# apple/ml-4m

Hardware: AMD Instinct MI355X
Metric: multimodal tokens/sec (4M-B train step, whole job) (higher is better)
Workload: dtype bf16; 1 GPU; 4M-B mod7 (fm_base_12e_12d_swiglu_nobias, 360.8M params, 8 input / 7 target modalities) masked-modeling train step, 224^2 token grids, 128 input + 128 target tokens/sample, AdamW; model=fm_base_12e_12d_swiglu_nobias, per_gpu_batch=256, global_batch=256, seq_len=256, parallelism=dp1

## Files before the change

include/fourm_hip.h:

```cpp
#ifndef FOURM_HIP_H
#define FOURM_HIP_H
#include <stdint.h>

#ifdef __cplusplus
extern "C" {
#endif

#define FM_ABI_VERSION 11
int fm_abi_version(void);
const char* fm_last_error(void);

enum fm_epilogue {
    FM_EPI_BF16 = 0,
    FM_EPI_GELU = 1,
    FM_EPI_RESIDUAL = 2,
    FM_EPI_SWIGLU = 3,
    FM_EPI_F32 = 4,
    FM_EPI_TANH = 5,
    FM_EPI_SWIGLU_BWD = 6,
    FM_EPI_GELU_BWD = 7,
    FM_EPI_QUICK_GELU = 8,
    FM_EPI_RELU = 9,
    FM_EPI_RELU_BWD = 10
};

typedef struct fm_gemm_group {
    const void* W;
    void* out;
    int32_t N, K, ldw, pad_;
} fm_gemm_group;

typedef struct fm_gemm_nt_args {
    const void* W; const void* W2; const void* X;
    void* out; void* out2; const void* res; const void* bias; const void* bias2;
    int32_t M, N, K, ldw, ldx, ldo, ldo2, ldr, Hp, epilogue;
    const fm_gemm_group* groups; const int32_t* tile_group; int32_t max_N;
    int32_t fixed_tiling;
    const int32_t* m_dev; const int32_t* row0_dev;
    void* splitk_ws; int64_t splitk_ws_bytes;
    int32_t conv_C, conv_H, conv_W, conv_Ho, conv_Wo, conv_stride, conv_up, conv_pad_;
} fm_gemm_nt_args;
int fm_gemm_nt(const fm_gemm_nt_args* args, void* stream);
void fm_set_gemm_nt_config(int cfg);
int fm_get_gemm_nt_config(void);
void fm_set_reserved_cus(int n);
int fm_get_reserved_cus(void);

typedef struct fm_gemm_tn_args {
    const void* A; const void* B; void* out;
    int32_t R, N, K, lda, ldb, ldo, a_cols, b_cols, splits, force_tr;
    const fm_gemm_group* groups; const int32_t* seg_start; const int32_t* seg_count;
    int32_t n_groups, max_N, max_R, pad_;
} fm_gemm_tn_args;
int fm_gemm_tn(const fm_gemm_tn_args* args, void* stream);
#define FM_TN_MAX_JOBS 16
typedef struct fm_gemm_tn_job {
    const void* A; const void* B; void* out;
    int32_t R, N, K, lda, ldb, ldo, a_cols, b_cols;
} fm_gemm_tn_job;
int fm_gemm_tn_multi(const fm_gemm_tn_job* jobs, int n_jobs, void* stream);
void fm_set_gemm_tn_config(int cfg);
int fm_get_gemm_tn_config(void);
void fm_set_tn_transpose_read(int on);
int fm_get_tn_transpose_read(void);

int fm_layernorm_fwd(const void* x, int ldx, const void* w, const void* b, void* y, int ldy, int y_is_f32,
                     void* mean, void* rstd, const int32_t* row_map, int R, int D, float eps, void* stream);
int fm_layernorm_fwd_res(const void* x, int ldx, const void* delta, int ldd, void* x_out, int ldxo, const void* w, const void* b,
                         void* y, int ldy, int y_is_f32, void* mean, void* rstd, const int32_t* row_map, int R, int D, float eps,
                         void* stream);
int fm_layernorm_bwd(const void* dy, int lddy, const int32_t* dy_row_map, const void* x, int ldx, const void* w,
                     const void* mean, const void* rstd, const void* dres, void* dx, int lddx, void* dx_bf16,
                     int lddxbf, void* dw, void* db, int R, int D, void* stream);
int fm_layernorm_bwd_h(const void* dy, int lddy, const void* h, int ldh, const void* x, int ldx, const void* w,
                       const void* mean, const void* rstd, const void* dres, void* dx, int lddx, void* dx_bf16,
                       int lddxbf, void* dw, int R, int D, void* stream);

int fm_headnorm_fwd(const void* x, int ldx, const void* w, const void* b, void* y, int ldy, void* stats, int R, int H, float eps,
                    void* stream);
int fm_headnorm_bwd(const void* dy, int lddy, const void* x, int ldx, const void* w, const void* stats, void* dx, int lddx, void* dw,
                    void* db, int R, int H, void* stream);

enum fm_mask_kind {
    FM_MASK_NONE = 0,
    FM_MASK_KEYPAD = 1,
    FM_MASK_DECODER = 2,
    FM_MASK_DENSE = 3
};
typedef struct fm_attn_args {
    const void* Q; const void* K; const void* V; void* O;
    void* stat_m; void* stat_l;
    int32_t ldq, ldk, ldv, ldo;
    int32_t B, H, Nq, Nk, head_dim, mask_kind;
    float scale; int32_t causal;
    const void* kpad; const int32_t* cs; const int16_t* modq; const int16_t* modk; const void* dense;
    const void* dO; void* dQ; void* dK; void* dV;
    int32_t lddo, lddq, lddk, lddv;
    int32_t force_tr;
    int32_t kv_batch_rows;
    int32_t zero_attn;
} fm_attn_args;
int fm_attn_fwd(const fm_attn_args* args, void* stream);
int fm_attn_bwd(const fm_attn_args* args, void* stream);
void fm_set_attn_transpose_read(int on);
int fm_get_attn_transpose_read(void);

#define FM_ATTN_DECODE_MAX_NK 8192
typedef struct fm_attn_decode_args {
    const void* q; void* k; const void* v; void* o;
    const void* q_w; const void* q_b; const void* k_w; const void* k_b;
    const void* kpad;
    int32_t ldq, ldk, ldv, ldo;
    int32_t B, H, Nk, kv_batch_rows, k_new_row, is_f32, zero_attn, pad_;
    float scale, eps;
} fm_attn_decode_args;
int fm_attn_decode(const fm_attn_decode_args* args, void* stream);

#define FM_MAX_MODS 24
enum fm_mod_kind {
    FM_KIND_TOK = 0,
    FM_KIND_PATCH = 1,
    FM_KIND_SEQ = 2,
    FM_KIND_SEQ_EMB = 3
};
typedef struct fm_mod_desc {
    const void* ids;
    const void* mask;
    const void* dam;
    const void* table;
    const void* pos;
    const void* mod_emb;
    const void* proj_bias;
    int32_t L;
    int32_t kind, ids_are_i64, mod_id;
    int32_t max_len;
    int32_t shifted;
    int32_t mask_stride, id_stride;
    int32_t patch, channels, grid_w, orig_dim;
    int32_t head_index;
    int32_t pad_;
} fm_mod_desc;
// ... 267 lines not shown
```

ml-4m_amd/csrc/gemm.hip:

```cpp
#include <type_traits>
#include <cstdlib>
#include <algorithm>
#include "common.h"
#include "fourm_hip.h"
#include "gemm_args.h"

namespace {
using namespace fmk;

constexpr int BK = 64;

__device__ __attribute__((aligned(16))) const uint32_t g_zero16[4] = {0u, 0u, 0u, 0u};

template <int TW, int TX, int WW, int WX, int KB, int STAGES, int EPI, bool GROUPED, bool PP = false, bool PERSIST = false, bool CONV = false>
__global__ __launch_bounds__(WW * WX * 64) void gemm_nt_kernel(NTArgs a) {
    constexpr int NWAVES = WW * WX;
    constexpr int RB = KB * 2;
    constexpr int CPR = RB / 16;
    constexpr int RPP = 1024 / RB;
    constexpr int SWSH = (RB == 128) ? 1 : 2;
    constexpr int LOADS = (TW + TX) / (RPP * NWAVES);
    constexpr int FW = TW / WW / 32, FX = TX / WX / 32;
    constexpr int STAGE = (TW + TX) * RB;
    static_assert(TW % (RPP * NWAVES) == 0 && TX % (RPP * NWAVES) == 0, "tile rows must split evenly over the DMA pieces");
// ... 633 lines not shown
#pragma unroll
                for (int i = 0; i < 2; ++i)
#pragma unroll
                    for (int j = 0; j < 2; ++j)
                        acc[i][j] = __builtin_amdgcn_mfma_f32_32x32x16_bf16(af[kk][i].v, bfr[kk][j].v, acc[i][j], 0, 0, 0);
                if (lead && more) stage_part(t_begin + it + 2, nbuf, kk, KS);
            }
            __builtin_amdgcn_s_setprio(0);
            if (lead) { if (more) wait_vmcnt<LOADS>(); else wait_vmcnt<0>(); }
            __builtin_amdgcn_sched_barrier(0);
            if (lead || it + 1 < NT_) block_barrier();
            buf = buf + 1 == STAGES ? 0 : buf + 1;
        }
    } else {
    int buf = 0;
    for (int it = 0; it < NT_; ++it) {
        const int younger = NT_ - 1 - it;
        if (STAGES >= 4 && younger >= 2) wait_vmcnt<2 * LOADS>();
        else if (STAGES >= 3 && younger >= 1) wait_vmcnt<LOADS>();
        else wait_vmcnt<0>();
        block_barrier();
        if (it + STAGES - 1 < NT_) stage(t_begin + it + STAGES - 1, (buf + STAGES - 1) % STAGES);
        const char* at = smem + buf * STAGE;
        const char* bt = at + KB * RBA;
        if constexpr (TR) {
            bf16x8_t af[2][2], bfr[2][2];
            auto load = [&](int kk, int par) {
                const int rA = kk * 16 + fhi * 8, rB = rA + 4;
#pragma unroll
                for (int i = 0; i < 2; ++i)
                    af[par][i] = lds_col_frag_tr_async([&](int r, int c) { return tn_addr<RBA>(at, r, c); }, rA, rB, wa * 64 + i * 32);
#pragma unroll
                for (int j = 0; j < 2; ++j)
                    bfr[par][j] = lds_col_frag_tr_async([&](int r, int c) { return tn_addr<RBB>(bt, r, c); }, rA, rB, wb * 64 + j * 32);
            };
            load(0, 0);
#pragma unroll
            for (int kk = 0; kk < KB / 16; ++kk) {
                if (kk + 1 < KB / 16) { load(kk + 1, (kk + 1) & 1); wait_lgkmcnt<8>(); }
                else wait_lgkmcnt<0>();
                __builtin_amdgcn_sched_barrier(0);
#pragma unroll
                for (int i = 0; i < 2; ++i)
#pragma unroll
                    for (int j = 0; j < 2; ++j)
                        acc[i][j] = __builtin_amdgcn_mfma_f32_32x32x16_bf16(af[kk & 1][i], bfr[kk & 1][j], acc[i][j], 0, 0, 0);
            }
        } else {
#pragma unroll
            for (int kk = 0; kk < KB / 16; ++kk) {
                const int rA = kk * 16 + fhi * 8, rB = rA + 4;
                bf16x8_t af[2], bfr[2];
#pragma unroll
                for (int i = 0; i < 2; ++i)
                    af[i] = lds_col_frag<false>([&](int r, int c) { return tn_addr<RBA>(at, r, c); }, rA, rB, wa * 64 + i * 32);
#pragma unroll
                for (int j = 0; j < 2; ++j)
                    bfr[j] = lds_col_frag<false>([&](int r, int c) { return tn_addr<RBB>(bt, r, c); }, rA, rB, wb * 64 + j * 32);
#pragma unroll
                for (int i = 0; i < 2; ++i)
#pragma unroll
                    for (int j = 0; j < 2; ++j)
                        acc[i][j] = __builtin_amdgcn_mfma_f32_32x32x16_bf16(af[i], bfr[j], acc[i][j], 0, 0, 0);
            }
        }
        buf = buf + 1 == STAGES ? 0 : buf + 1;
    }
    }
#pragma unroll
    for (int j = 0; j < 2; ++j) {
        const int k = k0 + wb * 64 + j * 32 + (lane & 31);
        if (k >= a.K) continue;
#pragma unroll
        for (int i = 0; i < 2; ++i)
#pragma unroll
            for (int r = 0; r < 16; ++r) {
                const int n = n0 + wa * 64 + i * 32 + (r & 3) + 8 * (r >> 2) + 4 * fhi;
                if (n < N) unsafeAtomicAdd(out + (size_t)n * a.ldo + k, acc[i][j][r]);
            }
    }
}


template <bool MASKED, int TA = 128, int KB = 64, bool LS = false>
__global__ __launch_bounds__(512) void gemm_tn_multi_kernel(TNMultiArgs a) {
    constexpr int TB = 256, WB = 4, STAGES = LS ? 2 : 3, NWAVES = 8;
    constexpr int FWA = TA / 2 / 32;
    constexpr int RBA = TA * 2, RBB = TB * 2;
    constexpr int PA = KB * RBA / 1024, PB = KB * RBB / 1024;
    constexpr int LOADS = (PA + PB) / NWAVES;
    constexpr int STAGE = KB * (RBA + RBB);
    constexpr int KS = KB / 16;
    extern __shared__ __attribute__((aligned(16))) char smem[];
    const int lane = threadIdx.x & 63;
    const int wave = __builtin_amdgcn_readfirstlane(threadIdx.x >> 6);
    const int wa = wave / WB, wb = wave % WB;
    const bool lead = wa == 0;
    const int fhi = lane >> 5;
    const bf16_t* zsrc = (const bf16_t*)g_zero16;
    const int G = gridDim.x;
    const int w = (blockIdx.x % 8) * (G / 8) + blockIdx.x / 8;

    const int li = lane & 15;
    const int frow0 = fhi * 8 + (li >> 2), fcol = ((lane >> 4) & 1) * 16 + (li & 3) * 4;
    const uint32_t smem_lds = (uint32_t)(uintptr_t)(__attribute__((address_space(3))) const char*)smem;
    uint32_t baseA[FWA], baseB[2];
#pragma unroll
    for (int i = 0; i < FWA; ++i) baseA[i] = (uint32_t)tn_off<RBA>(frow0, wa * (TA / 2) + i * 32 + fcol);
#pragma unroll
    for (int i = 0; i < 2; ++i) baseB[i] = (uint32_t)tn_off<RBB>(frow0, wb * 64 + i * 32 + fcol) + KB * RBA;

    auto run = [&](int tile, int t_begin, int t_end) {
        if (t_begin >= t_end) return;
        int j = 0;
        while (j + 1 < a.n_jobs && tile >= a.job[j + 1].tile_start) ++j;
        const TNJob& jb = a.job[j];
        const int local = tile - jb.tile_start;
        const int n0 = (local / jb.n_tiles_b) * TA, k0 = (local % jb.n_tiles_b) * TB;
        const bf16_t* A = jb.A; const bf16_t* B = jb.B;
        const int lda = jb.lda, ldb = jb.ldb, a_cols = jb.a_cols, b_cols = jb.b_cols, r_lim = jb.R;

#if defined(__HIP_DEVICE_COMPILE__)
        if constexpr (LS) {
            static_assert(!LS || (TA == 256 && KB == 64), "lock-step form: 256 x 256 tiles, K-step 64");
            constexpr int NPA = PA / NWAVES, NPB = PB / NWAVES, NP = NPA + NPB;
            const __amdgpu_buffer_rsrc_t rs_a = __builtin_amdgcn_make_buffer_rsrc(const_cast<bf16_t*>(A), 0, (int)min((size_t)r_lim * lda * 2, (size_t)0x7fffffff), 0x00020000);
            const __amdgpu_buffer_rsrc_t rs_b = __builtin_amdgcn_make_buffer_rsrc(const_cast<bf16_t*>(B), 0, (int)min((size_t)r_lim * ldb * 2, (size_t)0x7fffffff), 0x00020000);
            uint32_t offp[NP];
#pragma unroll
            for (int q = 0; q < NP; ++q) {
                const bool isa = q < NPA;
                const int piece = (isa ? q : q - NPA) * NWAVES + wave;
                const int row = piece * 2 + lane / 32;
                const int lc = (lane % 32) ^ ((row & 3) << 2);
                int c = (isa ? n0 : k0) + lc * 8;
                const int cols = isa ? a_cols : b_cols;
                c = c <= cols - 8 ? c : cols - 8;
                offp[q] = (uint32_t)row * (uint32_t)(isa ? lda : ldb) * 2u + (uint32_t)c * 2u;
            }
            auto dma = [&](int t, int buf, int q) __attribute__((always_inline)) {
                char* base = smem + buf * STAGE;
                if (q < NPA) __builtin_amdgcn_raw_ptr_buffer_load_lds(rs_a, LDS_PTR(base + (q * NWAVES + wave) * 1024), 16, offp[q], t * (KB * lda * 2), 0, 0);
                else __builtin_amdgcn_raw_ptr_buffer_load_lds(rs_b, LDS_PTR(base + KB * RBA + ((q - NPA) * NWAVES + wave) * 1024), 16, offp[q], t * (KB * ldb * 2), 0, 0);
            };
            f32x16_t acc[FWA][2];
#pragma unroll
            for (int i = 0; i < FWA; ++i)
#pragma unroll
                for (int jj = 0; jj < 2; ++jj)
#pragma unroll
                    for (int r = 0; r < 16; ++r) acc[i][jj][r] = 0.f;
            const int NT_ = t_end - t_begin;
#pragma unroll
            for (int q = 0; q < NP; ++q) dma(t_begin, 0, q);
            if (NT_ > 1) {
#pragma unroll
                for (int q = 0; q < NP; ++q) dma(t_begin + 1, 1, q);
                wait_vmcnt<NP>();
            } else wait_vmcnt<0>();
            block_barrier();
            union Frag { bf16x8_t v; s16x4_t h[2]; };
            Frag af[2][FWA], bfr[2][2];
            auto rd = [&](uint32_t st, auto kk_c, auto f_c, auto h_c, auto par_c) __attribute__((always_inline)) {
                constexpr int kk = decltype(kk_c)::value, f = decltype(f_c)::value, h = decltype(h_c)::value, PAR = decltype(par_c)::value;
                if constexpr (f < FWA) af[PAR][f].h[h] = tr_read<kk * 16 * RBA + h * 4 * RBA>(st + baseA[f]);
                else bfr[PAR][f - FWA].h[h] = tr_read<kk * 16 * RBB + h * 4 * RBB>(st + baseB[f - FWA]);
            };
            constexpr int NF = FWA + 2, NMF = FWA * 2;
            static_assert(!LS || NMF == 8, "k-step of the lock-step form: 8 MFMAs");
            using I0 = std::integral_constant<int, 0>; using I1 = std::integral_constant<int, 1>; using I2 = std::integral_constant<int, 2>;
            using I3 = std::integral_constant<int, 3>; using I4 = std::integral_constant<int, 4>; using I5 = std::integral_constant<int, 5>;
            auto k_step = [&](uint32_t st_next, auto kn_c, auto par_c, int t_dma, int buf_dma, auto d0_c, auto dn_c) __attribute__((always_inline)) {
                constexpr int PAR = decltype(par_c)::value, d0 = decltype(d0_c)::value, dn = decltype(dn_c)::value;
                wait_lgkmcnt<0>();
                __builtin_amdgcn_sched_barrier(0);
                auto one = [&](auto m_c) __attribute__((always_inline)) {
                    constexpr int m = decltype(m_c)::value;
                    constexpr int i = m / 2, jj = m % 2;
                    acc[i][jj] = __builtin_amdgcn_mfma_f32_32x32x16_bf16(af[PAR][i].v, bfr[PAR][jj].v, acc[i][jj], 0, 0, 0);
                    __builtin_amdgcn_sched_barrier(0);
                    if constexpr (m < NF) {
                        rd(st_next, kn_c, std::integral_constant<int, (m < NF ? m : 0)>{}, I0{}, std::integral_constant<int, PAR ^ 1>{});
                        rd(st_next, kn_c, std::integral_constant<int, (m < NF ? m : 0)>{}, I1{}, std::integral_constant<int, PAR ^ 1>{});
                    }
                    if constexpr (m < dn) { if (t_dma >= 0) dma(t_dma, buf_dma, d0 + m); }
                    __builtin_amdgcn_sched_barrier(0);
                };
                one(I0{}); one(I1{}); one(I2{}); one(I3{}); one(I4{}); one(I5{}); one(std::integral_constant<int, 6>{}); one(std::integral_constant<int, 7>{});
            };
            {
                const uint32_t st0 = smem_lds;
                rd(st0, I0{}, I0{}, I0{}, I0{}); rd(st0, I0{}, I0{}, I1{}, I0{}); rd(st0, I0{}, I1{}, I0{}, I0{}); rd(st0, I0{}, I1{}, I1{}, I0{});
                rd(st0, I0{}, I2{}, I0{}, I0{}); rd(st0, I0{}, I2{}, I1{}, I0{}); rd(st0, I0{}, I3{}, I0{}, I0{}); rd(st0, I0{}, I3{}, I1{}, I0{});
                rd(st0, I0{}, I4{}, I0{}, I0{}); rd(st0, I0{}, I4{}, I1{}, I0{}); rd(st0, I0{}, I5{}, I0{}, I0{}); rd(st0, I0{}, I5{}, I1{}, I0{});
            }
            int buf = 0;
            using NA = std::integral_constant<int, NPA>; using NB = std::integral_constant<int, NPB>;
            for (int it = 0; it < NT_; ++it) {
                const uint32_t st = smem_lds + buf * STAGE, stn = smem_lds + (buf ^ 1) * STAGE;
                const bool next = it + 1 < NT_, more = it + 2 < NT_;
                k_step(st, I1{}, I0{}, (it > 0 && next) ? t_begin + it + 1 : -1, buf ^ 1, NA{}, NB{});
                k_step(st, I2{}, I1{}, 0, 0, I0{}, I0{});
                k_step(st, I3{}, I0{}, 0, 0, I0{}, I0{});
// ... 53 lines not shown
        auto stage_part = [&](int t, int buf, int part, int nparts) {
#pragma unroll
            for (int q = 0; q < NP; ++q)
                if (q >= part * NP / nparts && q < (part + 1) * NP / nparts) stage_piece(t, buf, q);
        };

        f32x16_t acc[FWA][2];
#pragma unroll
        for (int i = 0; i < FWA; ++i)
#pragma unroll
            for (int jj = 0; jj < 2; ++jj)
#pragma unroll
                for (int r = 0; r < 16; ++r) acc[i][jj][r] = 0.f;

        const int NT_ = t_end - t_begin;
#pragma unroll
        for (int p = 0; p < STAGES - 1; ++p)
            if (p < NT_) stage(t_begin + p, p);
        if (NT_ > 1) wait_vmcnt<LOADS>(); else wait_vmcnt<0>();
        block_barrier();
        if (!lead) block_barrier();
        int buf = 0;
        for (int it = 0; it < NT_; ++it) {
            const bool more = it + 2 < NT_;
            const int nbuf = buf >= 1 ? buf - 1 : 2;
            const uint32_t st = smem_lds + buf * STAGE;
            union Frag { bf16x8_t v; s16x4_t h[2]; };
            Frag af[KS][FWA], bfr[KS][2];
            auto read_k = [&](auto kk_c) {
                constexpr int kk = decltype(kk_c)::value;
#pragma unroll
                for (int i = 0; i < FWA; ++i) {
                    af[kk][i].h[0] = tr_read<kk * 16 * RBA>(st + baseA[i]);
                    af[kk][i].h[1] = tr_read<kk * 16 * RBA + 4 * RBA>(st + baseA[i]);
                }
#pragma unroll
                for (int jj = 0; jj < 2; ++jj) {
                    bfr[kk][jj].h[0] = tr_read<kk * 16 * RBB>(st + baseB[jj]);
                    bfr[kk][jj].h[1] = tr_read<kk * 16 * RBB + 4 * RBB>(st + baseB[jj]);
                }
            };
            read_k(std::integral_constant<int, 0>{});
            read_k(std::integral_constant<int, 1>{});
            if constexpr (KS > 2) read_k(std::integral_constant<int, 2>{});
            if constexpr (KS > 3) read_k(std::integral_constant<int, 3>{});
            if (!lead) {
                if (more) { stage(t_begin + it + 2, nbuf); wait_vmcnt<LOADS>(); } else wait_vmcnt<0>();
            }
            wait_lgkmcnt<0>();
            block_barrier();
            __builtin_amdgcn_sched_barrier(0);
            __builtin_amdgcn_s_setprio(1);
#pragma unroll
            for (int kk = 0; kk < KS; ++kk) {
#pragma unroll
                for (int i = 0; i < FWA; ++i)
#pragma unroll
                    for (int jj = 0; jj < 2; ++jj)
                        acc[i][jj] = __builtin_amdgcn_mfma_f32_32x32x16_bf16(af[kk][i].v, bfr[kk][jj].v, acc[i][jj], 0, 0, 0);
                if (lead && more) stage_part(t_begin + it + 2, nbuf, kk, KS);
            }
            __builtin_amdgcn_s_setprio(0);
            if (lead) { if (more) wait_vmcnt<LOADS>(); else wait_vmcnt<0>(); }
            __builtin_amdgcn_sched_barrier(0);
            if (lead || it + 1 < NT_) block_barrier();
            buf = buf + 1 == STAGES ? 0 : buf + 1;
        }
        float* out = jb.out;
        const int N = jb.N, K = jb.K, ldo = jb.ldo;
        if (a.lab & 1) return;
#pragma unroll
        for (int jj = 0; jj < 2; ++jj) {
            const int k = k0 + wb * 64 + jj * 32 + (lane & 31);
            if (k >= K) continue;
#pragma unroll
            for (int i = 0; i < FWA; ++i)
#pragma unroll
                for (int r = 0; r < 16; ++r) {
                    const int n = n0 + wa * (TA / 2) + i * 32 + (r & 3) + 8 * (r >> 2) + 4 * fhi;
                    if (n < N) unsafeAtomicAdd(out + (size_t)n * ldo + k, acc[i][jj][r]);
                }
        }
    };
    tn_multi_walk(a, w, G, run);
}

int g_nt_config = 9, g_nt_prio = 1;
int g_lab[16] = {0, 0, [] { const char* e = getenv("FOURM_NT3"); return e ? atoi(e) : 3; }(), [] { const char* e = getenv("FOURM_NT3_LAB"); return e ? atoi(e) : 0; }(),
                 [] { const char* e = getenv("FOURM_NT4"); return e ? atoi(e) : 1; }(),
                 [] { const char* e = getenv("FOURM_TN4"); return e ? atoi(e) : 0; }(), 0, 0, 0,
                 [] { const char* e = getenv("FOURM_NT_SMALL"); return e ? atoi(e) : 1; }(),
                 [] { const char* e = getenv("FOURM_CONV_K32"); return e ? atoi(e) : 1; }()};
int g_nt_swiglu = 12;
int g_nt_auto[2] = {11, 10};

int g_reserved_cus = [] { const char* e = getenv("FOURM_RESERVED_CUS"); return e ? atoi(e) : 0; }();
static int n_compute_units() {
    static int n = [] {
        int dev = 0, cus = 0;
        if (hipGetDevice(&dev) != hipSuccess || hipDeviceGetAttribute(&cus, hipDeviceAttributeMultiprocessorCount, dev) != hipSuccess || cus <= 0) cus = 256;
        return cus;
    }();
    const int avail = n - g_reserved_cus;
    return avail >= 64 ? avail / 8 * 8 : n;
}

}
int fm_grid_cus() { return n_compute_units(); }
namespace {

template <int TW, int TX, int WW, int WX, int KB, int STAGES, int EPI, bool GROUPED, bool PP = false, bool PERSIST = false, bool CONV = false>
int launch_nt_cfg(NTArgs a, int max_n, hipStream_t s) {
    constexpr int NPT = (EPI == EPI_SWIGLU) ? TW / 2 : TW;
    a.n_tiles_w = (max_n + NPT - 1) / NPT;
    a.n_tiles_x = (a.M + TX - 1) / TX;
    int grid = a.n_tiles_w * a.n_tiles_x;
    if (GROUPED) {
        const int gw_max = TW > 128 ? 8 : 16;
        a.group_w = a.n_tiles_w < gw_max ? a.n_tiles_w : gw_max;
        const int chunks = ((a.n_tiles_w + a.group_w - 1) / a.group_w) * ((a.n_tiles_x + 3) / 4);
        grid = (chunks + 7) / 8 * 8 * a.group_w * 4;
    }
    const size_t lds = (size_t)STAGES * (TW + TX) * KB * 2;
    if (PERSIST) {
        const int slots = n_compute_units() * (int)(160 * 1024 / lds) / 8 * 8;
        if (grid > slots) grid = slots;
    }
    auto k = gemm_nt_kernel<TW, TX, WW, WX, KB, STAGES, EPI, GROUPED, PP, PERSIST, CONV>;
    static bool once = (hipFuncSetAttribute((const void*)k, hipFuncAttributeMaxDynamicSharedMemorySize, (int)lds), true);
    (void)once;
    hipLaunchKernelGGL(k, dim3(grid, a.split_k > 1 ? a.split_k : 1), dim3(WW * WX * 64), lds, s, a);
    FM_CHECK_LAUNCH("fm_gemm_nt");
    return 0;
}

__global__ __launch_bounds__(256) void splitk_reduce_kernel(const float* __restrict__ ws, int S, long long stride, int M, int N4, int ldp, const float* __restrict__ bias,
                                                            bf16_t* __restrict__ out, int ldo) {
    const long long total = (long long)M * N4;
    for (long long e = (long long)blockIdx.x * 256 + threadIdx.x; e < total; e += (long long)gridDim.x * 256) {
        const int m = (int)(e / N4), n = (int)(e % N4) * 4;
        float4 acc = *(const float4*)(ws + (size_t)m * ldp + n);
        for (int z = 1; z < S; ++z) {
            const float4 t = *(const float4*)(ws + (size_t)z * stride + (size_t)m * ldp + n);
            acc.x += t.x; acc.y += t.y; acc.z += t.z; acc.w += t.w;
        }
        if (bias) { const float4 b = *(const float4*)(bias + n); acc.x += bfround(b.x); acc.y += bfround(b.y); acc.z += bfround(b.z); acc.w += bfround(b.w); }
        *(uint2*)(out + (size_t)m * ldo + n) = make_uint2(pack2bf(acc.x, acc.y), pack2bf(acc.z, acc.w));
    }
}

template <int EPI, bool GROUPED>
int launch_nt(const NTArgs& a, int max_n, hipStream_t s) {
    if constexpr (GROUPED) {
        static_assert(FM_SEG_ROWS == 256, "the grouped configurations use a 256-row X tile");
        if constexpr (EPI == EPI_BF16) {
            static const int heads_cfg_k = [] { const char* e = getenv("FOURM_HEADS_NT_CFG"); return e ? atoi(e) : 0; }();
            if (a.K >= 1536 && heads_cfg_k == 3) return launch_nt_cfg<256, 256, 2, 4, 32, 3, EPI, true, true>(a, max_n, s);
            if (a.K >= 1536 && heads_cfg_k == 4) return launch_nt_cfg<256, 256, 2, 4, 64, 2, EPI, true>(a, max_n, s);
        }
        if (a.K >= 1536) return launch_nt_cfg<128, 256, 2, 4, 64, 3, EPI, true, true>(a, max_n, s);
        if constexpr (EPI == EPI_BF16) {
            static const int heads_cfg = [] { const char* e = getenv("FOURM_HEADS_NT_CFG"); return e ? atoi(e) : 0; }();
            if (heads_cfg == 1) return launch_nt_cfg<256, 256, 2, 4, 32, 3, EPI, true, true>(a, max_n, s);
            if (heads_cfg == 2) return launch_nt_cfg<128, 256, 2, 4, 32, 3, EPI, true, true>(a, max_n, s);
        }
        return launch_nt_cfg<128, 256, 2, 4, 32, 3, EPI, true>(a, max_n, s);
    }
    if (a.M <= 128 || a.fixed_tiling) return launch_nt_cfg<128, 128, 2, 2, 32, 3, EPI, GROUPED>(a, max_n, s);
    if constexpr (!GROUPED) {
        int cfg = g_nt_config;
        if (cfg == 9) {
            cfg = EPI == EPI_SWIGLU ? g_nt_swiglu : g_nt_auto[(a.K >= 1536 || EPI == EPI_RES || EPI == EPI_SWIGLU_BWD || EPI == EPI_GELU_BWD) ? 1 : 0];
            const long t256 = (long)((max_n + 255) / 256) * ((a.M + 255) / 256);
            if (cfg == g_nt_auto[0] && g_nt_auto[0] == 11 && max_n % 256 == 0 && t256 % n_compute_units() == 0) cfg = 12;
        }
        switch (cfg) {
            case 0: return launch_nt_cfg<128, 128, 2, 2, 64, 3, EPI, false>(a, max_n, s);
            case 1: return launch_nt_cfg<128, 256, 2, 4, 64, 3, EPI, false>(a, max_n, s);
            case 3: return launch_nt_cfg<256, 256, 2, 4, 32, 3, EPI, false, true>(a, max_n, s);
            case 4: return launch_nt_cfg<256, 256, 2, 4, 32, 3, EPI, false>(a, max_n, s);
            case 5: return launch_nt_cfg<256, 256, 2, 4, 64, 2, EPI, false>(a, max_n, s);
            case 6: return launch_nt_cfg<128, 128, 2, 2, 32, 3, EPI, false>(a, max_n, s);
            case 7: return launch_nt_cfg<128, 256, 2, 4, 64, 3, EPI, false, true>(a, max_n, s);
            case 8: return launch_nt_cfg<128, 256, 2, 4, 32, 3, EPI, false, true>(a, max_n, s);
            case 10: return launch_nt_cfg<128, 256, 2, 4, 64, 3, EPI, false, true, true>(a, max_n, s);
            case 11: return launch_nt_cfg<128, 256, 2, 4, 32, 3, EPI, false, true, true>(a, max_n, s);
            case 12: return launch_nt_cfg<256, 256, 2, 4, 32, 3, EPI, false, true, true>(a, max_n, s);
            case 13: if constexpr (EPI == EPI_BF16) return launch_nt_cfg<256, 256, 2, 2, 64, 2, EPI, false>(a, max_n, s); else break;
            case 14: if constexpr (EPI == EPI_BF16) return launch_nt_cfg<256, 256, 2, 2, 32, 3, EPI, false>(a, max_n, s); else break;
            default: return launch_nt_cfg<128, 256, 2, 4, 32, 3, EPI, false>(a, max_n, s);
        }
    }
    return -1;
}

}

extern "C" int fm_gemm_nt(const fm_gemm_nt_args* p, void* stream) {
    FM_CHECK_ARG(p && p->X && p->out, "fm_gemm_nt: null pointer");
    const bool grouped = p->groups != nullptr;
    FM_CHECK_ARG(grouped || p->W, "fm_gemm_nt: W is null");
    FM_CHECK_ARG(p->M > 0 && (grouped || (p->N > 0 && p->K > 0)), "fm_gemm_nt: bad shape M=%d N=%d K=%d", p->M, p->N, p->K);
    FM_CHECK_ARG(grouped || p->K % BK == 0, "fm_gemm_nt: K=%d must be a multiple of %d (zero padded)", p->K, BK);
    FM_CHECK_ARG(p->ldx % 8 == 0 && (grouped || p->ldw % 8 == 0), "fm_gemm_nt: leading dims must be multiples of 8");
    FM_CHECK_ARG(grouped || p->epilogue == FM_EPI_SWIGLU || p->ldo >= (p->N + 3) / 4 * 4, "fm_gemm_nt: ldo=%d too small for N=%d", p->ldo, p->N);
    FM_CHECK_ARG(!p->bias || (((uintptr_t)p->bias) & 15) == 0, "fm_gemm_nt: bias must be 16-byte aligned");
    FM_CHECK_ARG(p->ldo % 4 == 0, "fm_gemm_nt: ldo must be a multiple of 4");
    NTArgs a{};
    a.W = (const bf16_t*)p->W; a.W2 = (const bf16_t*)p->W2; a.X = (const bf16_t*)p->X;
    a.out = p->out; a.out2 = p->out2; a.res = (const float*)p->res; a.bias = (const float*)p->bias; a.bias2 = (const float*)p->bias2;
    a.M = p->M; a.N = p->N; a.K = p->K; a.ldw = p->ldw; a.ldx = p->ldx; a.ldo = p->ldo; a.ldo2 = p->ldo2; a.ldr = p->ldr; a.Hp = p->Hp;
    a.groups = p->groups; a.tile_group = p->tile_group;
    a.prio = g_nt_prio;
    a.dephase_groups = g_lab[0]; a.dephase_step = g_lab[1]; a.lab = g_lab[3];
    hipStream_t s = (hipStream_t)stream;
    a.m_dev = p->m_dev; a.row0_dev = p->row0_dev;
    const bool fixed = p->fixed_tiling != 0;
    FM_CHECK_ARG(!fixed || (!grouped && !p->m_dev && !p->row0_dev && p->conv_C == 0), "fm_gemm_nt: fixed_tiling is for dense launches (no groups, device-side rows or conv_*)");
    a.fixed_tiling = fixed ? 1 : 0;
    FM_CHECK_ARG(!(p->epilogue == FM_EPI_RELU || p->epilogue == FM_EPI_RELU_BWD) || (p->conv_C > 0 && !grouped && !p->m_dev && !p->row0_dev),
                 "fm_gemm_nt: FM_EPI_RELU / FM_EPI_RELU_BWD belong to the implicit convolution (conv_*), not to dense launches");
    if (p->m_dev || p->row0_dev) {
        FM_CHECK_ARG(p->m_dev && p->row0_dev && !grouped, "fm_gemm_nt: m_dev and row0_dev go together (dense launches only)");
        const int r = fm_launch_nt3(a, p->epilogue, g_lab[2] ? g_lab[2] : 3, s);
        if (r < 0) { fm_set_error("fm_gemm_nt (nt3, device-side rows): launch failed"); return -2; }
        if (r > 0) return 0;
        fm_set_error("fm_gemm_nt: a device-side row range needs FM_EPI_BF16 without bias, N %% 8 == 0, K %% 64 == 0, ldo %% 64 == 0 and a 128-byte aligned out "
                     "(N=%d K=%d ldo=%d epilogue=%d)", p->N, p->K, p->ldo, p->epilogue);
        return -1;
    }
    const int max_n = grouped ? p->max_N : p->N;
    if (!grouped && p->M <= 32 && p->conv_C == 0 && !fixed) {
        const int r = fm_launch_nt_skinny(a, p->epilogue, s);
        if (r < 0) { fm_set_error("fm_gemm_nt (skinny): launch failed"); return -2; }
        if (r > 0) return 0;
    }
    a.conv_C = p->conv_C; a.conv_H = p->conv_H; a.conv_W = p->conv_W; a.conv_Ho = p->conv_Ho; a.conv_Wo = p->conv_Wo; a.conv_stride = p->conv_stride; a.conv_up = p->conv_up;
    if (p->conv_C > 0) {
        const bool relu_bwd = p->epilogue == FM_EPI_RELU_BWD;
        FM_CHECK_ARG(!grouped && !p->m_dev && !p->out2 && (relu_bwd || !p->res) &&
                     (p->epilogue == FM_EPI_BF16 || p->epilogue == FM_EPI_F32 || p->epilogue == FM_EPI_RELU || relu_bwd),
                     "fm_gemm_nt (conv): dense FM_EPI_BF16 / FM_EPI_F32 / FM_EPI_RELU / FM_EPI_RELU_BWD only, no second output, res with FM_EPI_RELU_BWD only");
        FM_CHECK_ARG(!relu_bwd || (p->res && !p->bias && p->ldr % 4 == 0 && p->ldr >= (p->N + 3) / 4 * 4 && (((uintptr_t)p->res | (uintptr_t)p->out) & 7) == 0),
                     "fm_gemm_nt (conv): FM_EPI_RELU_BWD needs res = the saved bf16 activation (ldr %% 4 == 0, ldr >= roundup4(N), 8-byte aligned res / out) and no bias");
        FM_CHECK_ARG(p->conv_C % 64 == 0 && p->K == 9 * p->conv_C && (p->conv_stride == 1 || p->conv_stride == 2) && (p->conv_up == 0 || p->conv_up == 1) &&
                     p->conv_H > 0 && p->conv_W > 0 && p->conv_Ho > 0 && p->conv_Wo > 0 && p->M % (p->conv_Ho * p->conv_Wo) == 0,
                     "fm_gemm_nt (conv): C=%d K=%d stride=%d up=%d grid %dx%d -> %dx%d M=%d", p->conv_C, p->K, p->conv_stride, p->conv_up, p->conv_H, p->conv_W, p->conv_Ho, p->conv_Wo, p->M);
        FM_CHECK_ARG(p->conv_Ho == (p->conv_H + 2 - 3) / p->conv_stride + 1 && p->conv_Wo == (p->conv_W + 2 - 3) / p->conv_stride + 1, "fm_gemm_nt (conv): output grid does not match the input grid");
        if (p->epilogue == FM_EPI_F32) return launch_nt_cfg<128, 128, 2, 2, 64, 3, EPI_F32, false, false, false, true>(a, max_n, s);
        if (p->epilogue == FM_EPI_RELU) {
            if (g_lab[10]) return launch_nt_cfg<128, 128, 2, 2, 32, 3, EPI_RELU, false, false, false, true>(a, max_n, s);
            return launch_nt_cfg<128, 128, 2, 2, 64, 3, EPI_RELU, false, false, false, true>(a, max_n, s);
        }
        if (relu_bwd) {
            if (g_lab[10]) return launch_nt_cfg<128, 128, 2, 2, 32, 3, EPI_RELU_BWD, false, false, false, true>(a, max_n, s);
            return launch_nt_cfg<128, 128, 2, 2, 64, 3, EPI_RELU_BWD, false, false, false, true>(a, max_n, s);
        }
        const int cus = n_compute_units();
        const long t128 = (long)((p->M + 127) / 128) * ((p->N + 127) / 128);
        const int kt = p->K / 64;
        const long ldp = (p->N + 3) / 4 * 4;
        int S = 1;
        if (g_lab[9] && p->splitk_ws && t128 * 2 <= cus && p->N % 4 == 0 && (((uintptr_t)p->splitk_ws) & 15) == 0 && (((uintptr_t)p->out) & 7) == 0)
            S = (int)std::min<long>({cus / t128, (long)kt / 4, 16L, (long)(p->splitk_ws_bytes / ((long long)p->M * ldp * 4))});
        if (S >= 2) {
            const int ks = (kt + S - 1) / S * 64;
            S = (p->K + ks - 1) / ks;
            NTArgs b = a;
            b.out = p->splitk_ws; b.ldo = (int)ldp; b.bias = nullptr;
            b.split_k = S; b.k_slice = ks; b.split_stride = (long long)p->M * ldp;
            const int r = launch_nt_cfg<128, 128, 2, 2, 64, 3, EPI_F32, false, false, false, true>(b, max_n, s);
            if (r != 0) return r;
            const long long quads = (long long)p->M * (ldp / 4);
            const int rgrid = (int)std::min<long long>((quads + 255) / 256, 2048);
            hipLaunchKernelGGL(splitk_reduce_kernel, dim3(rgrid), dim3(256), 0, s, (const float*)p->splitk_ws, S, b.split_stride, p->M, (int)(ldp / 4), (int)ldp,
                               (const float*)p->bias, (bf16_t*)p->out, p->ldo);
            FM_CHECK_LAUNCH("fm_gemm_nt (conv, split-K reduction)");
            return 0;
        }
// ... 72 lines not shown
    }
    fm_set_error("fm_gemm_nt: unknown epilogue %d", p->epilogue);
    return -1;
}

extern int g_nt_flat;
extern "C" void fm_set_gemm_nt_config(int cfg) {
    g_nt_config = cfg & 0xff; g_nt_prio = (cfg >> 8) & 1;
    g_nt_flat = (cfg >> 29) & 1;
    if ((cfg >> 16) & 0xff) { g_nt_auto[0] = (cfg >> 16) & 0xf; g_nt_auto[1] = (cfg >> 20) & 0xf; }
    if ((cfg >> 24) & 0xf) g_nt_swiglu = (cfg >> 24) & 0xf;
}
extern "C" int fm_get_gemm_nt_config(void) { return g_nt_config; }
extern "C" void fm_lab_set(int key, int value) { if (key >= 0 && key < 16) g_lab[key] = value; }
extern "C" void fm_set_reserved_cus(int n) { g_reserved_cus = n < 0 ? 0 : n; }
extern "C" int fm_get_reserved_cus(void) { return g_reserved_cus; }
static int g_tn_config = [] { const char* e = getenv("FOURM_TN_CONFIG"); return e ? atoi(e) : 1; }();
extern "C" void fm_set_gemm_tn_config(int cfg) { g_tn_config = cfg; }
extern "C" int fm_get_gemm_tn_config(void) { return g_tn_config; }
static int g_tn_use_tr = 1;
extern "C" void fm_set_tn_transpose_read(int on) { g_tn_use_tr = on; }
extern "C" int fm_get_tn_transpose_read(void) { return g_tn_use_tr; }

extern "C" int fm_gemm_tn(const fm_gemm_tn_args* p, void* stream) {
    FM_CHECK_ARG(p && p->A && p->B, "fm_gemm_tn: null pointer");
    const bool grouped = p->groups != nullptr;
    FM_CHECK_ARG(grouped || p->out, "fm_gemm_tn: out is null");
    FM_CHECK_ARG(p->K > 0 && (grouped || (p->N > 0 && p->R > 0)), "fm_gemm_tn: bad shape");
    FM_CHECK_ARG(p->lda % 8 == 0 && p->ldb % 8 == 0, "fm_gemm_tn: leading dims must be multiples of 8");
    TNArgs a{};
    a.A = (const bf16_t*)p->A; a.B = (const bf16_t*)p->B; a.out = (float*)p->out;
    a.R = p->R; a.N = p->N; a.K = p->K; a.lda = p->lda; a.ldb = p->ldb; a.ldo = p->ldo;
    a.a_cols = p->a_cols > 0 ? p->a_cols : p->lda; a.b_cols = p->b_cols > 0 ? p->b_cols : p->ldb;
    FM_CHECK_ARG(a.a_cols >= 8 && a.b_cols >= 8, "fm_gemm_tn: operands need at least 8 readable columns");
    a.groups = p->groups; a.seg_start = p->seg_start; a.seg_count = p->seg_count;
    const int max_n = grouped ? p->max_N : p->N;
    constexpr int TN_TA = 128, TN_TB = 256, TN_STAGES = 3;
    const bool pp = (g_tn_config == 1 || g_tn_config == 3 || g_tn_config == 4) && !grouped && p->force_tr != 0;
    const int kb = pp ? 64 : 32, slots = (pp ? 1 : 2) * n_compute_units();
    a.n_tiles_a = (max_n + TN_TA - 1) / TN_TA; a.n_tiles_b = (p->K + TN_TB - 1) / TN_TB;
    int splits = p->splits;
    if (splits <= 0) {
        const int tiles = a.n_tiles_a * a.n_tiles_b;
        const int nt = grouped ? (p->max_R + kb - 1) / kb : (p->R + kb - 1) / kb;
        splits = tiles >= slots ? 1 : slots / tiles;
        while (splits > 1 && nt / splits < 8) --splits;
        if (splits > 64) splits = 64;
        if (nt < 16) splits = 1;
    }
    a.splits = splits;
    const size_t lds = (size_t)TN_STAGES * kb * (TN_TA + TN_TB) * 2;
    const int total_items = a.n_tiles_a * a.n_tiles_b * splits;
    const int deal = grouped ? 8 * 4 * a.n_tiles_b : 8;
    dim3 grid((total_items + deal - 1) / deal * deal, 1, grouped ? p->n_groups : 1);
    hipStream_t s = (hipStream_t)stream;
    const bool masked = grouped || p->R % kb != 0;
#define LAUNCH_TN(TR, G, KBV, PPV)                                                                  \
    if (masked) LAUNCH_TN2(TR, G, KBV, PPV, true) else LAUNCH_TN2(TR, G, KBV, PPV, false)
#define LAUNCH_TN2(TR, G, KBV, PPV, MK)                                                             \
    {                                                                                               \
        auto k = gemm_tn_kernel<TR, G, TN_TA, TN_TB, 2, 4, KBV, TN_STAGES, PPV, MK>;                \
        static bool once = (hipFuncSetAttribute((const void*)k, hipFuncAttributeMaxDynamicSharedMemorySize, (int)lds), true); \
        (void)once;                                                                                 \
        hipLaunchKernelGGL(k, grid, dim3(512), lds, s, a);                                          \
    }
    const int tr = p->force_tr >= 0 ? p->force_tr : g_tn_use_tr;
    if (pp) { if (grouped) { LAUNCH_TN(true, true, 64, true); } else { LAUNCH_TN(true, false, 64, true); } }
    else if (tr) { if (grouped) { LAUNCH_TN(true, true, 32, false); } else { LAUNCH_TN(true, false, 32, false); } }
    else { if (grouped) { LAUNCH_TN(false, true, 32, false); } else { LAUNCH_TN(false, false, 32, false); } }
#undef LAUNCH_TN
#undef LAUNCH_TN2
    FM_CHECK_LAUNCH("fm_gemm_tn");
    return 0;
}

extern "C" int fm_gemm_tn_multi(const fm_gemm_tn_job* jobs, int n_jobs, void* stream) {
    FM_CHECK_ARG(jobs && n_jobs > 0 && n_jobs <= FM_TN_MAX_JOBS, "fm_gemm_tn_multi: 1..FM_TN_MAX_JOBS jobs");
    TNMultiArgs a{};
    bool masked = false;
    int tiles = 0;
    long long units = 0;
    static const bool small_env = [] { const char* e = getenv("FOURM_TN_MULTI_TILE"); return e && atoi(e) == 128; }();
    const bool big = !(small_env || g_tn_config == 3);
    bool t4 = big && g_lab[5] != 0 && (g_tn_config == 1 || g_tn_config == 4);
    if (t4) {
        double useful = 0, padded = 0;
        for (int i = 0; i < n_jobs && t4; ++i) {
            const fm_gemm_tn_job& p = jobs[i];
            const int ac = p.a_cols > 0 ? p.a_cols : p.lda, bc = p.b_cols > 0 ? p.b_cols : p.ldb;
            t4 = p.R % 64 == 0 && p.R >= 256 && p.N % 128 == 0 && p.K % 128 == 0 && ac >= 128 && bc >= 128 && ac % 8 == 0 && bc % 8 == 0 &&
                 (((uintptr_t)p.A | (uintptr_t)p.B) & 15) == 0 && ((size_t)p.R * p.lda + ac) * 2 < 0x7fffffffull && ((size_t)p.R * p.ldb + bc) * 2 < 0x7fffffffull;
            useful += (double)p.N * p.K * p.R;
            padded += (double)((p.N + 255) / 256 * 256) * ((p.K + 383) / 384 * 384) * p.R;
        }
        t4 = t4 && useful >= 0.92 * padded;
    }
    const bool ls = big && (g_tn_config == 4 || t4);
    const int ta = big ? 256 : 128, kb = (big && !ls) ? 32 : 64, tb = t4 ? 384 : 256;
    for (int i = 0; i < n_jobs; ++i) {
        const fm_gemm_tn_job& p = jobs[i];
        FM_CHECK_ARG(p.A && p.B && p.out, "fm_gemm_tn_multi: null pointer");
        FM_CHECK_ARG(p.K > 0 && p.N > 0 && p.R > 0, "fm_gemm_tn_multi: bad shape");
        FM_CHECK_ARG(p.lda % 8 == 0 && p.ldb % 8 == 0, "fm_gemm_tn_multi: leading dims must be multiples of 8");
        TNJob& j = a.job[i];
        j.A = (const bf16_t*)p.A; j.B = (const bf16_t*)p.B; j.out = (float*)p.out;
        j.R = p.R; j.N = p.N; j.K = p.K; j.lda = p.lda; j.ldb = p.ldb; j.ldo = p.ldo;
        j.a_cols = p.a_cols > 0 ? p.a_cols : p.lda; j.b_cols = p.b_cols > 0 ? p.b_cols : p.ldb;
        FM_CHECK_ARG(j.a_cols >= 8 && j.b_cols >= 8, "fm_gemm_tn_multi: operands need at least 8 readable columns");
        j.n_tiles_b = (p.K + tb - 1) / tb;
        j.tiles = ((p.N + ta - 1) / ta) * j.n_tiles_b;
        j.tile_start = tiles;
        j.kt = (p.R + kb - 1) / kb;
        tiles += j.tiles;
        units += (long long)j.tiles * j.kt;
        masked = masked || p.R % kb != 0;
    }
    a.n_jobs = n_jobs; a.tiles = tiles; a.lab = g_lab[6];
    int grid = n_compute_units();
    if (units / 8 < grid) grid = (int)((units / 8 + 7) / 8 * 8);
    if (grid < 8) grid = 8;
    {
        const int rem = tiles % grid, ntail = grid - rem;
        a.tail_rr = rem >= ntail;
        double c = ls ? (a.tail_rr ? 12.0 : 64.0) : big ? (a.tail_rr ? 24.0 : 128.0) : 8.0;
        if (t4 && g_lab[7] > 0) c = g_lab[7];
        double cb = ls ? 16.0 : 32.0;
        if (t4 && g_lab[8] > 0) cb = g_lab[8];
        static const bool band_off = [] { const char* e = getenv("FOURM_TN_BANDS"); return e && atoi(e) == 0; }();
        a.banded = !a.tail_rr && rem > 0 && ntail > rem && !band_off;
        static const bool hybrid_off = [] { const char* e = getenv("FOURM_TN_HYBRID"); return e && atoi(e) == 0; }();
        a.hybrid = a.tail_rr && rem > ntail && ntail > 0 && !hybrid_off;
        for (int i = 0; i < n_jobs; ++i) {
            TNJob& j = a.job[i];
            j.lb = 0;
            if (rem == 0) { j.q = j.kt; continue; }
            if (a.banded) {
                const double rw = (double)rem / (ntail - rem);
                double q = (rw * j.kt + rw * cb) / (1.0 + 2.0 * rw);
                if (q < 0) q = 0;
                if (2 * q > j.kt) q = j.kt / 2;
                j.q = j.lb = (int)q;
                continue;
            }
            if (a.hybrid) {
                const double r = (double)rem / ntail;
                j.q = (int)((j.kt * r + c) / (1.0 + r));
            } else if (a.tail_rr) {
                const int n = (rem + ntail - 1) / ntail;
                double left = (j.kt - (n - 1) * c) / (n + 1.0);
                j.q = j.kt - (left > 0 ? (int)left : 0);
            } else {
                const double r = (double)rem / ntail;
                j.q = (int)((j.kt * r + r * c) / (1.0 + r));
            }
            if (j.q > j.kt) j.q = j.kt;
            if (j.q < 0) j.q = 0;
        }
    }
    hipStream_t s = (hipStream_t)stream;
#define LAUNCH_TNM(MK, TAV, KBV, ...)                                                                                         \
    {                                                                                                                         \
        constexpr bool lsv = sizeof(#__VA_ARGS__) > 1;                                                                        \
        constexpr size_t lds = (size_t)(lsv ? 2 : 3) * KBV * (TAV + 256) * 2;                                                 \
        auto k = gemm_tn_multi_kernel<MK, TAV, KBV, lsv>;                                                                     \
        static bool once = (hipFuncSetAttribute((const void*)k, hipFuncAttributeMaxDynamicSharedMemorySize, (int)lds), true); \
        (void)once;                                                                                                           \
        hipLaunchKernelGGL(k, dim3(grid), dim3(512), lds, s, a);                                                              \
    }
    if (t4) fm_launch_tn4_multi(a, grid, s);
    else if (ls) LAUNCH_TNM(false, 256, 64, ls)
    else if (big) { if (masked) LAUNCH_TNM(true, 256, 32) else LAUNCH_TNM(false, 256, 32) }
    else { if (masked) LAUNCH_TNM(true, 128, 64) else LAUNCH_TNM(false, 128, 64) }
#undef LAUNCH_TNM
    FM_CHECK_LAUNCH("fm_gemm_tn_multi");
    return 0;
}
```

ml-4m_amd/csrc/gemm_args.h:

```cpp
#pragma once
#include "common.h"
#include "fourm_hip.h"

namespace fmk {

enum { EPI_BF16 = FM_EPI_BF16, EPI_GELU = FM_EPI_GELU, EPI_RES = FM_EPI_RESIDUAL, EPI_SWIGLU = FM_EPI_SWIGLU,
       EPI_F32 = FM_EPI_F32, EPI_TANH = FM_EPI_TANH, EPI_SWIGLU_BWD = FM_EPI_SWIGLU_BWD, EPI_GELU_BWD = FM_EPI_GELU_BWD, EPI_QGELU = FM_EPI_QUICK_GELU,
       EPI_RELU = FM_EPI_RELU, EPI_RELU_BWD = FM_EPI_RELU_BWD };

struct NTArgs {
    const bf16_t* W; const bf16_t* W2; const bf16_t* X;
    void* out; void* out2; const float* res; const float* bias; const float* bias2;
    int M, N, K, ldw, ldx, ldo, ldo2, ldr, Hp;
    const fm_gemm_group* groups; const int* tile_group;
    const int* m_dev; const int* row0_dev;
    int n_tiles_w, n_tiles_x;
    int group_w;
    int prio;
    int dephase_groups, dephase_step;
    int reverse;
    int conv_C, conv_H, conv_W, conv_Ho, conv_Wo, conv_stride, conv_up;
    int split_k, k_slice; long long split_stride;
    int fixed_tiling;
    int lab;
};

__device__ __forceinline__ float gelu_f(float x) { return 0.5f * x * (1.0f + erf_fast(x * 0.70710678118654752f)); }
__device__ __forceinline__ float quick_gelu_f(float x) { return x * __builtin_amdgcn_rcpf(1.0f + __expf(-1.702f * x)); }
template <int EPI> constexpr bool is_gelu_like = EPI == EPI_GELU || EPI == EPI_QGELU;
template <int EPI> __device__ __forceinline__ float gelu_like_f(float x) { if constexpr (EPI == EPI_QGELU) return quick_gelu_f(x); else return gelu_f(x); }
__device__ __forceinline__ float silu_f(float x) { return x * __builtin_amdgcn_rcpf(1.0f + __expf(-x)); }


struct TNJob {
    const bf16_t* A; const bf16_t* B; float* out;
    int R, N, K, lda, ldb, ldo, a_cols, b_cols;
    int n_tiles_b, tiles, tile_start, kt;
    int q;
    int lb;
};
struct TNMultiArgs {
    TNJob job[FM_TN_MAX_JOBS];
    int n_jobs, tiles, tail_rr, banded;
    int hybrid;
    int lab;
};


template <typename Run>
__device__ __forceinline__ void tn_multi_walk(const TNMultiArgs& a, int w, int G, Run&& run) {
    auto job_of = [&](int tile) {
        int j = 0;
        while (j + 1 < a.n_jobs && tile >= a.job[j + 1].tile_start) ++j;
        return j;
    };

    const int full = a.tiles / G, T0 = full * G, rem = a.tiles - T0, ntail = G - rem;
    auto q_of = [&](int j) { return a.job[j].q; };
    const int nband = a.hybrid ? 0 : (a.banded ? rem : 0), nwalk = ntail - nband;
    const int walk_T0 = a.hybrid ? T0 + ntail : T0;
    auto q2_of = [&](int j) { return a.job[j].q + ((a.banded && !a.hybrid) ? a.job[j].lb : 0); };
    long long u0 = 0, u1 = 0;
    if (rem > 0 && w >= rem + nband && (!a.tail_rr || a.hybrid)) {
        long long Lsum = 0;
        for (int j = 0; j < a.n_jobs; ++j) {
            const int lo = max(a.job[j].tile_start, walk_T0), hi = a.job[j].tile_start + a.job[j].tiles;
            if (hi > lo) Lsum += (long long)(hi - lo) * (a.job[j].kt - q2_of(j));
        }
        u0 = Lsum * (w - rem - nband) / nwalk; u1 = Lsum * (w - rem - nband + 1) / nwalk;
    }
    int phase = 0, f = 0, tj = 0, ci = -1;
    long long P = 0;
    for (;;) {
        int tile = 0, t0 = 0, t1 = 0;
        bool have = false;
        if (phase == 0) {
            if (f < full) { tile = f * G + w; t1 = a.job[job_of(tile)].kt; ++f; have = true; }
            else { phase = rem == 0 ? 3 : (w < rem ? 1 : ((!a.tail_rr && w < rem + nband) ? 4 : 2)); f = 0; }
        } else if (phase == 1) {
            tile = T0 + w; t1 = q_of(job_of(tile)); phase = 3; have = true;
        } else if (phase == 4) {
            tile = T0 + (w - rem); const int j = job_of(tile); t0 = q_of(j); t1 = t0 + a.job[j].lb; phase = 3; have = true;
        } else if (phase == 2 && a.tail_rr && !(a.hybrid && f > 0)) {
            const int sgm = (w - rem) + f * ntail;
            if (sgm >= rem) phase = 3;
            else { tile = T0 + sgm; const int j = job_of(tile); t0 = q_of(j); t1 = a.job[j].kt; ++f; have = true; }
        } else if (phase == 2) {
            if (tj >= a.n_jobs) phase = 3;
            else {
                const int lo = max(a.job[tj].tile_start, walk_T0), hi = a.job[tj].tile_start + a.job[tj].tiles;
                const int q = q2_of(tj), left = a.job[tj].kt - q;
                bool advance = true;
                if (hi > lo && left > 0) {
                    const long long Pn = P + (long long)(hi - lo) * left;
                    if (u1 > P && u0 < Pn) {
                        const long long s0 = max(u0, P) - P, s1 = min(u1, Pn) - P;
                        if (ci < 0) ci = (int)(s0 / left);
                        const long long base = (long long)ci * left;
                        if (base < s1) {
                            tile = lo + ci; t0 = q + (int)(max(s0, base) - base); t1 = q + (int)(min(s1, base + left) - base);
                            ++ci; have = true; advance = false;
                        }
                    }
                    if (advance) P = Pn;
                }
                if (advance) { ++tj; ci = -1; }
            }
        } else break;
        if (have) run(tile, t0, t1);
    }
}

}

int fm_launch_nt_flat(const fmk::NTArgs& a, int epilogue, hipStream_t s);
int fm_launch_nt3(const fmk::NTArgs& a, int epilogue, int mode, hipStream_t s);
int fm_launch_nt4(const fmk::NTArgs& a, int epilogue, int mode, hipStream_t s);
int fm_launch_nt_skinny(const fmk::NTArgs& a, int epilogue, hipStream_t s);
int fm_grid_cus();
int fm_launch_tn4_multi(const fmk::TNMultiArgs& a, int grid, hipStream_t s);
```

ml-4m_amd/csrc/gemm_nt3.hip:

```cpp
#include <type_traits>
#include "common.h"
#include "fourm_hip.h"
#include "gemm_args.h"

namespace {
using namespace fmk;

typedef __attribute__((ext_vector_type(4))) unsigned int u32x4_t;
typedef __attribute__((ext_vector_type(4))) float f32x4v_t;

__device__ __forceinline__ __amdgpu_buffer_rsrc_t rsrc_of(const void* base) {
    return __builtin_amdgcn_make_buffer_rsrc(const_cast<void*>(base), 0, 0x7fffffff, 0x00020000);
}
constexpr uint32_t OOB = 0x80000000u;

template <int TW, int EPI, bool SPLIT = false, bool STG = false, bool BIAS = false, bool DEVM = false>
__global__ __launch_bounds__(512) void gemm_nt3_kernel(NTArgs a) {
#if defined(__HIP_DEVICE_COMPILE__)
    if constexpr (DEVM) {
        static_assert(EPI == EPI_BF16, "device-side row ranges: bf16 outputs only");
        const int m = (a.m_dev[0] + 255) & ~255;
        const size_t r0 = (size_t)a.row0_dev[0];
        a.M = m; a.n_tiles_x = m >> 8;
        a.X += r0 * a.ldx;
        a.out = (char*)a.out + r0 * a.ldo * 2;
        if (a.n_tiles_w * a.n_tiles_x <= (int)blockIdx.x) return;
    }
    constexpr int TX = 256, KB = 64, WW = 2, WX = 4, NWAVES = 8, KS = 4;
    constexpr int RB = 128, CPR = 8, RPP = 8;
    constexpr int FW = TW / WW / 32, FX = TX / WX / 32;
    constexpr int PW = TW / (RPP * NWAVES), PX = TX / (RPP * NWAVES), LOADS = PW + PX;
    constexpr int STAGE = (TW + TX) * RB;
    constexpr int NPT = (EPI == EPI_SWIGLU) ? TW / 2 : TW;
    constexpr int NMF = FW * FX;
    constexpr int NST = (EPI == EPI_BF16 || is_gelu_like<EPI>) ? FW * FX * 2 : EPI == EPI_SWIGLU ? FX * (FW / 2) * 2 * 3 : EPI == EPI_SWIGLU_BWD ? 60 : FW * FX * 4;
    static_assert(TW % (RPP * NWAVES) == 0, "tile rows must split evenly over the DMA pieces");
    static_assert(EPI != EPI_SWIGLU || FW % 2 == 0, "SwiGLU needs (g,u) fragment pairs per wave");
    extern __shared__ __attribute__((aligned(16))) char smem[];

    const int lane = threadIdx.x & 63;
    const int wave = __builtin_amdgcn_readfirstlane(threadIdx.x >> 6);
    const int ww = wave / WX, wx = wave % WX;
    const int frow = lane & 31, fhi = lane >> 5;
    const int fswz = (frow >> 1) & (CPR - 1);

    const int total = a.n_tiles_w * a.n_tiles_x;
    if (a.dephase_groups > 1) {
        const int ph = ((int)blockIdx.x / 8) % a.dephase_groups;
        for (int i = 0; i < ph * a.dephase_step; ++i) __builtin_amdgcn_s_sleep(32);
    }
    const int n_my = (total - (int)blockIdx.x + (int)gridDim.x - 1) / (int)gridDim.x;
    const int KT = a.K / KB;
    const int G = n_my * KT;
    const int N = a.N;

    uint32_t woff[PW], xoff[PX];
    __amdgpu_buffer_rsrc_t rs_w = rsrc_of(a.W), rs_w2 = rsrc_of(a.W2 ? a.W2 : a.W), rs_x = rsrc_of(a.X);
    (void)rs_w2;
    const int gw = a.group_w;
    const bool grouped_order = gw > 0 && total % 8 == 0 && a.n_tiles_x % 8 == 0 && a.n_tiles_w % gw == 0;
    auto tile_origin = [&](int j, int& n0, int& m0) {
        int tile = xcd_remap((int)blockIdx.x + j * (int)gridDim.x, total);
        if (a.reverse) tile = total - 1 - tile;
        int tw = tile % a.n_tiles_w, tx = tile / a.n_tiles_w;
        if (grouped_order) {
            const int per_xcd = total / 8, xr = a.n_tiles_x / 8;
            const int xcd = tile / per_xcd, l = tile % per_xcd;
            const int grp = l / (xr * gw), rem = l % (xr * gw);
            tx = xcd * xr + rem / gw; tw = grp * gw + rem % gw;
        }
        n0 = tw * NPT; m0 = tx * TX;
    };
    auto set_sources = [&](int j) __attribute__((always_inline)) {
        int n0, m0;
        tile_origin(j, n0, m0);
        rs_w = rsrc_of(a.W + (size_t)n0 * a.ldw);
        if constexpr (EPI == EPI_SWIGLU) rs_w2 = rsrc_of(a.W2 + (size_t)n0 * a.ldw);
        rs_x = rsrc_of(a.X + (size_t)m0 * a.ldx);
#pragma unroll
        for (int p = 0; p < PW; ++p) {
            const int t = (p * NWAVES + wave) * RPP + lane / CPR;
            const int lc = (lane % CPR) ^ ((t >> 1) & (CPR - 1));
            int r;
            if constexpr (EPI == EPI_SWIGLU) r = (t >> 6) * 32 + (t & 31);
            else r = t;
            r = n0 + r < N ? r : N - 1 - n0;
            woff[p] = (uint32_t)r * (uint32_t)a.ldw * 2u + (uint32_t)lc * 16u;
        }
#pragma unroll
        for (int p = 0; p < PX; ++p) {
            const int t = (p * NWAVES + wave) * RPP + lane / CPR;
            const int lc = (lane % CPR) ^ ((t >> 1) & (CPR - 1));
            const int r = m0 + t < a.M ? t : a.M - 1 - m0;
            xoff[p] = (uint32_t)r * (uint32_t)a.ldx * 2u + (uint32_t)lc * 16u;
        }
    };
    int s_kt = 0, s_j = 0, s_buf = 0;
    auto stage_piece = [&](int q) __attribute__((always_inline)) {
        const int soff = s_kt * (KB * 2);
        if (q < PW) {
            const int pi = q < PW ? q : 0;
            const int t0 = (pi * NWAVES + wave) * RPP;
            if (EPI == EPI_SWIGLU && ((t0 >> 5) & 1))
                __builtin_amdgcn_raw_ptr_buffer_load_lds(rs_w2, LDS_PTR(smem + s_buf * STAGE + (pi * NWAVES + wave) * 1024), 16, woff[pi], soff, 0, 0);
            else
                __builtin_amdgcn_raw_ptr_buffer_load_lds(rs_w, LDS_PTR(smem + s_buf * STAGE + (pi * NWAVES + wave) * 1024), 16, woff[pi], soff, 0, 0);
        } else {
            const int pi = q >= PW ? q - PW : 0;
            __builtin_amdgcn_raw_ptr_buffer_load_lds(rs_x, LDS_PTR(smem + s_buf * STAGE + TW * RB + (pi * NWAVES + wave) * 1024), 16, xoff[pi], soff, 0, 0);
        }
    };
    auto stage_advance = [&]() __attribute__((always_inline)) {
        ++s_kt; s_buf ^= 1;
        if (s_kt == KT) { s_kt = 0; ++s_j; if (s_j < n_my) set_sources(s_j); }
    };

    f32x16_t acc[FW][FX];
#pragma unroll
    for (int i = 0; i < FW; ++i)
#pragma unroll
        for (int j = 0; j < FX; ++j)
#pragma unroll
            for (int r = 0; r < 16; ++r) acc[i][j][r] = 0.f;

    auto finish_tile = [&](int j_done) __attribute__((always_inline)) {
        int n0, m0;
        tile_origin(j_done, n0, m0);
        if constexpr ((EPI == EPI_BF16 || is_gelu_like<EPI>) && STG) {
            const __amdgpu_buffer_rsrc_t rs_out = rsrc_of((const char*)a.out + (size_t)m0 * a.ldo * 2);
            const __amdgpu_buffer_rsrc_t rs_pre = rsrc_of((const char*)(a.out2 ? a.out2 : a.out) + (size_t)m0 * (a.out2 ? a.ldo2 : a.ldo) * 2);
            (void)rs_pre;
            constexpr int CW = (TW / WW) / 8;
            constexpr int RCH = CW == 16 ? 8 : 12, ROWB = RCH * 16, NRND = CW / RCH, SPR = 32 * RCH / 64;
            char* sc = smem + 2 * STAGE + wave * (32 * ROWB);
            constexpr int NWHICH = is_gelu_like<EPI> ? 2 : 1;
#pragma unroll
            for (int j = 0; j < FX; ++j)
#pragma unroll
                for (int rnd = 0; rnd < NRND; ++rnd)
#pragma unroll
                for (int which = 0; which < NWHICH; ++which) {
                    if (is_gelu_like<EPI> && which == 0 && !a.out2) continue;
#pragma unroll
                    for (int ii = 0; ii < RCH / 4; ++ii)
#pragma unroll
                        for (int g = 0; g < 4; ++g) {
                            const int i = rnd * (RCH / 4) + ii, ch = ii * 4 + g;
                            float v[4] = {acc[i][j][4 * g], acc[i][j][4 * g + 1], acc[i][j][4 * g + 2], acc[i][j][4 * g + 3]};
                            if constexpr (BIAS) {
                                const int cb = n0 + ww * (TW / WW) + i * 32 + 8 * g + 4 * fhi;
                                if (cb < N) {
                                    const float4 t = *(const float4*)(a.bias + cb);
                                    v[0] += bfround(t.x); v[1] += bfround(t.y); v[2] += bfround(t.z); v[3] += bfround(t.w);
                                }
                            }
                            if (is_gelu_like<EPI> && which == 1) {
#pragma unroll
                                for (int e = 0; e < 4; ++e) v[e] = gelu_like_f<EPI>(bfround(v[e]));
                            }
                            const uint2 pv = make_uint2(pack2bf(v[0], v[1]), pack2bf(v[2], v[3]));
                            int pos;
                            if constexpr (RCH == 8) pos = ch ^ (frow & 7);
                            else { pos = ch + (frow & 7); pos = pos >= 12 ? pos - 12 : pos; }
                            *(uint2*)(sc + frow * ROWB + pos * 16 + fhi * 8) = pv;
                        }
                    wait_lgkmcnt<0>();
                    __builtin_amdgcn_sched_barrier(0);
                    u32x4_t rv[SPR];
                    int rr[SPR], cc[SPR];
#pragma unroll
                    for (int q = 0; q < SPR; ++q) {
                        const int t = q * 64 + lane;
                        rr[q] = t / RCH; cc[q] = t % RCH;
                        int pos;
                        if constexpr (RCH == 8) pos = cc[q] ^ (rr[q] & 7);
                        else { pos = cc[q] + (rr[q] & 7); pos = pos >= 12 ? pos - 12 : pos; }
                        rv[q] = *(const u32x4_t*)(sc + rr[q] * ROWB + pos * 16);
                    }
                    wait_lgkmcnt<0>();
                    __builtin_amdgcn_sched_barrier(0);
#pragma unroll
                    for (int q = 0; q < SPR; ++q) {
                        const int rl = wx * (TX / WX) + j * 32 + rr[q];
                        const int c = n0 + ww * (TW / WW) + rnd * (RCH * 8) + cc[q] * 8;
                        if (is_gelu_like<EPI> && which == 0) {
                            const uint32_t so = ((m0 + rl < a.M && c < N) ? 0u : OOB) | ((uint32_t)(rl * a.ldo2) * 2u + (uint32_t)c * 2u);
                            __builtin_amdgcn_raw_buffer_store_b128(rv[q], rs_pre, so, 0, 0);
                        } else {
                            const uint32_t so = ((m0 + rl < a.M && c < N) ? 0u : OOB) | ((uint32_t)(rl * a.ldo) * 2u + (uint32_t)c * 2u);
                            __builtin_amdgcn_raw_buffer_store_b128(rv[q], rs_out, so, 0, 0);
                        }
                    }
                }
        } else if constexpr (EPI == EPI_BF16) {
            const __amdgpu_buffer_rsrc_t rs_out = rsrc_of((const char*)a.out + (size_t)m0 * a.ldo * 2);
            const int c0 = n0 + ww * (TW / WW) + 8 * fhi;
#pragma unroll
            for (int j = 0; j < FX; ++j) {
                const int rl = wx * (TX / WX) + j * 32 + frow;
                const uint32_t rowoff = (m0 + rl < a.M ? 0u : OOB) | ((uint32_t)(rl * a.ldo) * 2u);
#pragma unroll
                for (int i = 0; i < FW; ++i)
#pragma unroll
                    for (int gp = 0; gp < 2; ++gp) {
                        const int g = 2 * gp;
                        const uint2 p0 = make_uint2(pack2bf(acc[i][j][4 * g], acc[i][j][4 * g + 1]), pack2bf(acc[i][j][4 * g + 2], acc[i][j][4 * g + 3]));
                        const uint2 p1 = make_uint2(pack2bf(acc[i][j][4 * g + 4], acc[i][j][4 * g + 5]), pack2bf(acc[i][j][4 * g + 6], acc[i][j][4 * g + 7]));
                        const auto x = __builtin_amdgcn_permlane32_swap(p0.x, p1.x, false, false);
                        const auto y = __builtin_amdgcn_permlane32_swap(p0.y, p1.y, false, false);
                        const u32x4_t v = {x[0], y[0], x[1], y[1]};
                        const int c = c0 + i * 32 + 16 * gp;
                        const uint32_t so = (c < N ? rowoff : OOB) + (uint32_t)c * 2u;
                        if (a.lab & 32) __builtin_amdgcn_raw_buffer_store_b128(v, rs_out, so, 0, 2);
                        else if (a.lab & 64) __builtin_amdgcn_raw_buffer_store_b128(v, rs_out, so, 0, 17);
                        else if (a.lab & 128) __builtin_amdgcn_raw_buffer_store_b128(v, rs_out, so, 0, 3);
                        else __builtin_amdgcn_raw_buffer_store_b128(v, rs_out, so, 0, 0);
                    }
            }
        } else if constexpr (EPI == EPI_RES) {
            const __amdgpu_buffer_rsrc_t rs_out = rsrc_of((const char*)a.out + (size_t)m0 * a.ldo * 4);
            const __amdgpu_buffer_rsrc_t rs_res = rsrc_of((const char*)a.res + (size_t)m0 * a.ldr * 4);
            const int c0 = n0 + ww * (TW / WW) + 4 * fhi;
            f32x4v_t rv[2][4];
            auto req = [&](int f, int par) __attribute__((always_inline)) {
                const int j = f / FW, i = f % FW;
                const int rl = wx * (TX / WX) + j * 32 + frow;
                const uint32_t rowoff = (m0 + rl < a.M ? 0u : OOB) | ((uint32_t)(rl * a.ldr) * 4u);
#pragma unroll
                for (int g = 0; g < 4; ++g) {
                    const int c = c0 + i * 32 + 8 * g;
                    rv[par][g] = __builtin_bit_cast(f32x4v_t, __builtin_amdgcn_raw_buffer_load_b128(rs_res, (c < N ? rowoff : OOB) + (uint32_t)c * 4u, 0, 0));
                }
            };
            req(0, 0);
#pragma unroll
            for (int f = 0; f < FW * FX; ++f) {
                if (f + 1 < FW * FX) req(f + 1, (f + 1) & 1);
                const int j = f / FW, i = f % FW;
                const int rl = wx * (TX / WX) + j * 32 + frow;
                const uint32_t rowoff = (m0 + rl < a.M ? 0u : OOB) | ((uint32_t)(rl * a.ldo) * 4u);
#pragma unroll
                for (int g = 0; g < 4; ++g) {
                    const int c = c0 + i * 32 + 8 * g;
                    f32x4v_t o = rv[f & 1][g];
#pragma unroll
                    for (int e = 0; e < 4; ++e) o[e] += bfround(acc[i][j][4 * g + e]);
                    __builtin_amdgcn_raw_buffer_store_b128(__builtin_bit_cast(u32x4_t, o), rs_out, (c < N ? rowoff : OOB) + (uint32_t)c * 4u, 0, 0);
                }
            }
        } else if constexpr (EPI == EPI_SWIGLU_BWD) {
            const __amdgpu_buffer_rsrc_t rs_out = rsrc_of((const char*)a.out + (size_t)m0 * a.ldo * 2);
            const __amdgpu_buffer_rsrc_t rs_gu = rsrc_of((const char*)a.res + (size_t)m0 * a.ldr * 2);
            const int c0 = n0 + ww * (TW / WW) + 8 * fhi;
            u32x4_t sv[2][2];
            constexpr int NU = FW * FX * 2;
            auto src_off = [&](int unit, int ld) __attribute__((always_inline)) {
                const int f = unit / 2, gp = unit % 2, j = f / FW, i = f % FW;
                const int rl = wx * (TX / WX) + j * 32 + frow;
                const int c = c0 + i * 32 + 16 * gp;
                return ((m0 + rl < a.M && c < N) ? 0u : OOB) | ((uint32_t)(rl * ld) * 2u + (uint32_t)c * 2u);
            };
            auto req = [&](int unit, int par) __attribute__((always_inline)) {
                const uint32_t off = src_off(unit, a.ldr);
                sv[par][0] = __builtin_amdgcn_raw_buffer_load_b128(rs_gu, off, 0, 0);
                sv[par][1] = __builtin_amdgcn_raw_buffer_load_b128(rs_gu, off + (uint32_t)a.Hp * 2u, 0, 0);
            };
            req(0, 0);
#pragma unroll
            for (int unit = 0; unit < NU; ++unit) {
                if (unit + 1 < NU) req(unit + 1, (unit + 1) & 1);
                const int f = unit / 2, gp = unit % 2, j = f / FW, i = f % FW;
                uint2 g2[2], u2[2], dg2[2], du2[2];
                {
                    const u32x4_t tg = sv[unit & 1][0], tu = sv[unit & 1][1];
                    const auto gx = __builtin_amdgcn_permlane32_swap(tg[0], tg[2], false, false);
                    const auto gy = __builtin_amdgcn_permlane32_swap(tg[1], tg[3], false, false);
                    const auto ux = __builtin_amdgcn_permlane32_swap(tu[0], tu[2], false, false);
                    const auto uy = __builtin_amdgcn_permlane32_swap(tu[1], tu[3], false, false);
                    g2[0] = make_uint2(gx[0], gy[0]); g2[1] = make_uint2(gx[1], gy[1]);
                    u2[0] = make_uint2(ux[0], uy[0]); u2[1] = make_uint2(ux[1], uy[1]);
                }
#pragma unroll
                for (int u = 0; u < 2; ++u) {
                    const int g = 2 * gp + u;
                    float xv[4], uv[4], r1[4], r2[4];
                    unpack_bf4(g2[u], xv); unpack_bf4(u2[u], uv);
#pragma unroll
                    for (int e = 0; e < 4; ++e) {
                        const float d = bfround(acc[i][j][4 * g + e]);
                        const float sg = 1.0f / (1.0f + __expf(-xv[e]));
                        const float sl = bfround(xv[e] * sg);
                        const float ds = bfround(d * uv[e]);
                        r2[e] = d * sl;
                        r1[e] = ds * (sg * (1.0f + xv[e] * (1.0f - sg)));
                    }
                    dg2[u] = make_uint2(pack2bf(r1[0], r1[1]), pack2bf(r1[2], r1[3]));
                    du2[u] = make_uint2(pack2bf(r2[0], r2[1]), pack2bf(r2[2], r2[3]));
                }
                const auto ax = __builtin_amdgcn_permlane32_swap(dg2[0].x, dg2[1].x, false, false);
                const auto ay = __builtin_amdgcn_permlane32_swap(dg2[0].y, dg2[1].y, false, false);
                const auto bx = __builtin_amdgcn_permlane32_swap(du2[0].x, du2[1].x, false, false);
                const auto by = __builtin_amdgcn_permlane32_swap(du2[0].y, du2[1].y, false, false);
                const u32x4_t vg = {ax[0], ay[0], ax[1], ay[1]}, vu = {bx[0], by[0], bx[1], by[1]};
                const uint32_t off = src_off(unit, a.ldo);
                __builtin_amdgcn_raw_buffer_store_b128(vg, rs_out, off, 0, 0);
                __builtin_amdgcn_raw_buffer_store_b128(vu, rs_out, off + (uint32_t)a.Hp * 2u, 0, 0);
            }
        } else if constexpr (EPI == EPI_SWIGLU && STG) {
            const __amdgpu_buffer_rsrc_t rs_out = rsrc_of((const char*)a.out + (size_t)m0 * a.ldo * 2);
            const __amdgpu_buffer_rsrc_t rs_out2 = rsrc_of((const char*)(a.out2 ? a.out2 : a.out) + (size_t)m0 * (a.out2 ? a.ldo2 : a.ldo) * 2);
            char* sc = smem + 2 * STAGE + wave * 4096;
            const int hw0 = n0 + (ww * (TW / WW) / 64) * 32;
#pragma unroll
            for (int j = 0; j < FX; ++j) {
                uint2 qg[FW / 2][4], qu[FW / 2][4];
#pragma unroll
                for (int ip = 0; ip < FW / 2; ++ip)
#pragma unroll
                    for (int g = 0; g < 4; ++g) {
                        qg[ip][g] = make_uint2(pack2bf(acc[2 * ip][j][4 * g], acc[2 * ip][j][4 * g + 1]), pack2bf(acc[2 * ip][j][4 * g + 2], acc[2 * ip][j][4 * g + 3]));
                        qu[ip][g] = make_uint2(pack2bf(acc[2 * ip + 1][j][4 * g], acc[2 * ip + 1][j][4 * g + 1]), pack2bf(acc[2 * ip + 1][j][4 * g + 2], acc[2 * ip + 1][j][4 * g + 3]));
                        asm volatile("" : "+v"(qg[ip][g].x), "+v"(qg[ip][g].y), "+v"(qu[ip][g].x), "+v"(qu[ip][g].y));
                    }
#pragma unroll
                for (int which = 0; which < 3; ++which) {
                    if (which < 2 && !a.out2) continue;
#pragma unroll
                    for (int ip = 0; ip < FW / 2; ++ip)
#pragma unroll
                        for (int g = 0; g < 4; ++g) {
                            uint2 pv = which == 0 ? qg[ip][g] : qu[ip][g];
                            if (which == 2) {
                                float gv[4], uv[4];
                                unpack_bf4(qg[ip][g], gv); unpack_bf4(qu[ip][g], uv);
                                pv = make_uint2(pack2bf(bfround(silu_f(gv[0])) * uv[0], bfround(silu_f(gv[1])) * uv[1]),
                                                pack2bf(bfround(silu_f(gv[2])) * uv[2], bfround(silu_f(gv[3])) * uv[3]));
                            }
                            const int ch = ip * 4 + g;
                            *(uint2*)(sc + frow * 128 + ((ch ^ (frow & 7)) * 16) + fhi * 8) = pv;
                        }
                    wait_lgkmcnt<0>();
                    __builtin_amdgcn_sched_barrier(0);
                    u32x4_t rv[4];
#pragma unroll
                    for (int q = 0; q < 4; ++q) {
                        const int r = q * 8 + (lane >> 3), c = lane & 7;
                        rv[q] = *(const u32x4_t*)(sc + r * 128 + ((c ^ (r & 7)) * 16));
                    }
                    wait_lgkmcnt<0>();
                    __builtin_amdgcn_sched_barrier(0);
#pragma unroll
                    for (int q = 0; q < 4; ++q) {
                        const int rl = wx * (TX / WX) + j * 32 + q * 8 + (lane >> 3);
                        const int h = hw0 + (lane & 7) * 8;
                        const uint32_t ok = (m0 + rl < a.M && h < N) ? 0u : OOB;
                        if (which == 2) __builtin_amdgcn_raw_buffer_store_b128(rv[q], rs_out, ok | ((uint32_t)(rl * a.ldo) * 2u + (uint32_t)h * 2u), 0, 0);
                        else if (a.lab & 32) __builtin_amdgcn_raw_buffer_store_b128(rv[q], rs_out2, ok | ((uint32_t)(rl * a.ldo2) * 2u + (uint32_t)(h + (which == 1 ? a.Hp : 0)) * 2u), 0, 0);
                        else if (a.lab & 64) __builtin_amdgcn_raw_buffer_store_b128(rv[q], rs_out2, ok | ((uint32_t)(rl * a.ldo2) * 2u + (uint32_t)(h + (which == 1 ? a.Hp : 0)) * 2u), 0, 17);
                        else if (a.lab & 128) __builtin_amdgcn_raw_buffer_store_b128(rv[q], rs_out2, ok | ((uint32_t)(rl * a.ldo2) * 2u + (uint32_t)(h + (which == 1 ? a.Hp : 0)) * 2u), 0, 3);
                        else __builtin_amdgcn_raw_buffer_store_b128(rv[q], rs_out2, ok | ((uint32_t)(rl * a.ldo2) * 2u + (uint32_t)(h + (which == 1 ? a.Hp : 0)) * 2u), 0, 2);
                    }
                }
            }
        } else if constexpr (EPI == EPI_SWIGLU) {
            const __amdgpu_buffer_rsrc_t rs_out = rsrc_of((const char*)a.out + (size_t)m0 * a.ldo * 2);
            const __amdgpu_buffer_rsrc_t rs_out2 = rsrc_of((const char*)(a.out2 ? a.out2 : a.out) + (size_t)m0 * (a.out2 ? a.ldo2 : a.ldo) * 2);
            const int h0 = n0 + (ww * (TW / WW) / 64) * 32 + 8 * fhi;
#pragma unroll
            for (int j = 0; j < FX; ++j) {
                const int rl = wx * (TX / WX) + j * 32 + frow;
                const uint32_t ok = m0 + rl < a.M ? 0u : OOB;
                const uint32_t ro = ok | ((uint32_t)(rl * a.ldo) * 2u), ro2 = ok | ((uint32_t)(rl * a.ldo2) * 2u);
                u32x4_t pg[FW / 2][2], pu[FW / 2][2], pa[FW / 2][2];
#pragma unroll
                for (int ip = 0; ip < FW / 2; ++ip)
#pragma unroll
                    for (int gp = 0; gp < 2; ++gp) {
                        uint2 qg[2], qu[2], qa[2];
#pragma unroll
                        for (int u = 0; u < 2; ++u) {
                            const int g = 2 * gp + u;
                            float gv[4], uv[4], av[4];
#pragma unroll
                            for (int e = 0; e < 4; ++e) {
                                gv[e] = bfround(acc[2 * ip][j][4 * g + e]);
                                uv[e] = bfround(acc[2 * ip + 1][j][4 * g + e]);
                                av[e] = bfround(silu_f(gv[e])) * uv[e];
                            }
                            qg[u] = make_uint2(pack2bf(gv[0], gv[1]), pack2bf(gv[2], gv[3]));
                            qu[u] = make_uint2(pack2bf(uv[0], uv[1]), pack2bf(uv[2], uv[3]));
                            qa[u] = make_uint2(pack2bf(av[0], av[1]), pack2bf(av[2], av[3]));
                        }
                        auto swz = [&](const uint2 (&p)[2]) {
                            const auto x = __builtin_amdgcn_permlane32_swap(p[0].x, p[1].x, false, false);
                            const auto y = __builtin_amdgcn_permlane32_swap(p[0].y, p[1].y, false, false);
                            const u32x4_t v = {x[0], y[0], x[1], y[1]};
                            return v;
                        };
                        pg[ip][gp] = swz(qg); pu[ip][gp] = swz(qu); pa[ip][gp] = swz(qa);
                    }
#pragma unroll
                for (int which = 0; which < 3; ++which)
#pragma unroll
                    for (int ip = 0; ip < FW / 2; ++ip)
#pragma unroll
                        for (int gp = 0; gp < 2; ++gp) {
                            const int h = h0 + ip * 32 + 16 * gp;
                            const uint32_t col = (uint32_t)h * 2u;
                            if (which == 2) __builtin_amdgcn_raw_buffer_store_b128(pa[ip][gp], rs_out, (h < N ? ro : OOB) + col, 0, 0);
                            else __builtin_amdgcn_raw_buffer_store_b128(which == 0 ? pg[ip][gp] : pu[ip][gp], rs_out2,
                                                                        ((h < N && a.out2) ? ro2 : OOB) + col + (which == 1 ? (uint32_t)a.Hp * 2u : 0u), 0, 0);
                        }
            }
        }
#pragma unroll
        for (int i = 0; i < FW; ++i)
#pragma unroll
            for (int j = 0; j < FX; ++j)
#pragma unroll
                for (int r = 0; r < 16; ++r) acc[i][j][r] = 0.f;
    };

    set_sources(0);
#pragma unroll
    for (int q = 0; q < LOADS; ++q) stage_piece(q);
    stage_advance();
    if (G > 1) {
#pragma unroll
        for (int q = 0; q < LOADS; ++q) stage_piece(q);
        stage_advance();
        wait_vmcnt<LOADS>();
    } else wait_vmcnt<0>();
    block_barrier();

    bf16x8_t wf[2][FW], xf[2][FX];
    auto read_frags = [&](int buf, int kk, int par) __attribute__((always_inline)) {
        const char* wt = smem + buf * STAGE + (ww * (TW / WW) + frow) * RB;
        const char* xt = smem + buf * STAGE + TW * RB + (wx * (TX / WX) + frow) * RB;
        const int off = ((kk * 2 + fhi) ^ fswz) * 16;
#pragma unroll
        for (int i = 0; i < FW; ++i) wf[par][i] = *(const bf16x8_t*)(wt + i * 32 * RB + off);
#pragma unroll
        for (int j = 0; j < FX; ++j) xf[par][j] = *(const bf16x8_t*)(xt + j * 32 * RB + off);
    };
    auto mfmas = [&](int par) __attribute__((always_inline)) {
#pragma unroll
        for (int i = 0; i < FW; ++i)
#pragma unroll
            for (int j = 0; j < FX; ++j)
                acc[i][j] = __builtin_amdgcn_mfma_f32_32x32x16_bf16(wf[par][i], xf[par][j], acc[i][j], 0, 0, 0);
    };
    read_frags(0, 0, 0);

    int buf = 0, c_kt = 0, c_j = 0;
// ... 8 lines not shown
#pragma unroll
                for (int q = 0; q < PW; ++q) stage_piece(q);
            }
            mfmas(kk & 1);
#pragma unroll
            for (int q = 0; q < FW + FX; ++q) {
                __builtin_amdgcn_sched_group_barrier(0x008, 1, 0);
                __builtin_amdgcn_sched_group_barrier(0x100, 1, 0);
                if (HALF && kk == 0 && q < PW) __builtin_amdgcn_sched_group_barrier(0x020, 1, 0);
            }
            __builtin_amdgcn_sched_barrier(0);
            if (HALF && kk == 0) stage_advance();
        }
        if constexpr (NEXT) {
            if (!(a.lab & 1)) { if (stores_behind && !SPLIT) wait_vmcnt<NST>(); else wait_vmcnt<0>(); }
        }
        wait_lgkmcnt<0>();
        block_barrier();
        __builtin_amdgcn_sched_barrier(0);
        if constexpr (NEXT) read_frags(buf ^ 1, 0, 0);
        constexpr int NOW = SPLIT ? PX : LOADS;
        if constexpr (MORE) {
            if (!(a.lab & 2)) {
#pragma unroll
                for (int q = SPLIT ? PW : 0; q < LOADS; ++q) stage_piece(q);
            }
        }
        mfmas(1);
        constexpr int RD = NEXT ? FW + FX : 0, RSTEPS = (RD + 1) / 2;
#pragma unroll
        for (int q = 0; q < RSTEPS; ++q) {
            __builtin_amdgcn_sched_group_barrier(0x008, 1, 0);
            __builtin_amdgcn_sched_group_barrier(0x100, 2, 0);
        }
        if constexpr (MORE) {
            constexpr int LEFT = NMF - RSTEPS - 1;
            constexpr int PER = (NOW + LEFT - 1) / LEFT;
#pragma unroll
            for (int q = 0; q < LEFT; ++q) {
                __builtin_amdgcn_sched_group_barrier(0x008, 1, 0);
                __builtin_amdgcn_sched_group_barrier(0x020, PER, 0);
            }
        }
        __builtin_amdgcn_sched_barrier(0);
        if constexpr (MORE && !SPLIT) stage_advance();
        buf ^= 1;
        stores_behind = false;
        if (++c_kt == KT) {
            if (!(a.lab & 4)) finish_tile(c_j);
            c_kt = 0; ++c_j; stores_behind = true;
        }
    };
    using T = std::true_type; using F = std::false_type;
    if (G > 2) k_tile(T{}, T{}, T{}); else k_tile(T{}, T{}, F{});
    for (int g = 1; g + 2 < G; ++g) k_tile(F{}, T{}, T{});
    if (G > 2) k_tile(F{}, T{}, F{});
    k_tile(F{}, F{}, F{});
#endif
}

template <int TW, int EPI, bool SPLIT = false, bool STG = false, bool BIAS = false, bool DEVM = false>
int launch_nt3(NTArgs a, hipStream_t s) {
    constexpr int NPT = (EPI == EPI_SWIGLU) ? TW / 2 : TW;
    a.n_tiles_w = (a.N + NPT - 1) / NPT;
    a.n_tiles_x = (a.M + 255) / 256;
    a.group_w = (a.lab >> 12) & 15;
    if (a.group_w == 0 && EPI == EPI_SWIGLU && STG) a.group_w = 4;
    if (a.group_w == 15) a.group_w = 0;
    int grid = a.n_tiles_w * a.n_tiles_x;
    const int cus = fm_grid_cus();
    if (grid > cus || DEVM) grid = cus;
    a.reverse = (a.lab & 2048) ? 0 : 1;
    const size_t lds = (size_t)2 * (TW + 256) * 128 + (STG ? (TW == 256 ? 32768 : 49152) : 0);
    auto k = gemm_nt3_kernel<TW, EPI, SPLIT, STG, BIAS, DEVM>;
    static bool once = (hipFuncSetAttribute((const void*)k, hipFuncAttributeMaxDynamicSharedMemorySize, (int)lds), true);
    (void)once;
    hipLaunchKernelGGL(k, dim3(grid), dim3(512), lds, s, a);
    if (hipGetLastError() != hipSuccess) return -2;
    return 1;
}

}

int fm_launch_nt3(const fmk::NTArgs& a, int epilogue, int mode, hipStream_t s) {
    using namespace fmk;
    if (!mode || a.groups || a.bias2) return 0;
    if (a.m_dev) {
        if (!a.row0_dev || epilogue != FM_EPI_BF16 || a.bias || a.K % 64 != 0 || a.K < 128 || a.N % 8 != 0 || a.ldo % 64 != 0 ||
            (((uintptr_t)a.out) & 127) != 0 || (a.lab & (16 | 1024)))
            return 0;
        if ((size_t)256 * (size_t)a.ldo * 4 >= 0x7fffffffull || (size_t)256 * (size_t)a.ldx * 2 >= 0x7fffffffull || (size_t)256 * (size_t)a.ldw * 2 >= 0x7fffffffull) return 0;
        return (a.N % 192 == 0 && a.N % 256 != 0) ? launch_nt3<192, EPI_BF16, true, true, false, true>(a, s) : launch_nt3<256, EPI_BF16, true, true, false, true>(a, s);
    }
    if (a.bias && !(epilogue == FM_EPI_BF16 || epilogue == FM_EPI_GELU || epilogue == FM_EPI_QUICK_GELU)) return 0;
    if (a.bias && ((((uintptr_t)a.bias) & 15) != 0 || (a.lab & (16 | 1024)))) return 0;
    if (a.M < 2048 || a.K % 64 != 0 || a.K < 128 || a.N % 8 != 0) return 0;
    if ((size_t)256 * (size_t)a.ldo * 4 >= 0x7fffffffull || (size_t)256 * (size_t)a.ldx * 2 >= 0x7fffffffull || (size_t)256 * (size_t)a.ldw * 2 >= 0x7fffffffull) return 0;
    const bool al16 = (((uintptr_t)a.out | (uintptr_t)a.out2 | (uintptr_t)a.res) & 15) == 0;
    if (!al16) return 0;
    const int cus = fm_grid_cus();
    const long xt = (a.M + 255) / 256;
    const long t256 = (long)((a.N + 255) / 256) * xt, t192 = (long)((a.N + 191) / 192) * xt;
    const bool fits192 = a.N % 192 == 0;
    const long c256 = (t256 + cus - 1) / cus * 256, c192 = (t192 + cus - 1) / cus * 192;
    const bool use192 = mode == 2 ? fits192 : mode == 3 ? (fits192 && c192 < c256) : false;
    if (epilogue == FM_EPI_GELU) {
        if (!(a.lab & 131072)) return 0;
        if (a.ldo % 64 != 0 || (((uintptr_t)a.out) & 127) != 0 || (a.out2 && (a.ldo2 % 64 != 0 || (((uintptr_t)a.out2) & 127) != 0)) || (a.lab & (16 | 1024))) return 0;
        if (a.bias) return use192 ? launch_nt3<192, EPI_GELU, true, true, true>(a, s) : launch_nt3<256, EPI_GELU, true, true, true>(a, s);
        return use192 ? launch_nt3<192, EPI_GELU, true, true, false>(a, s) : launch_nt3<256, EPI_GELU, true, true, false>(a, s);
    }
    if (epilogue == FM_EPI_QUICK_GELU) {
        if (!(a.lab & 131072)) return 0;
        if (a.ldo % 64 != 0 || (((uintptr_t)a.out) & 127) != 0 || (a.out2 && (a.ldo2 % 64 != 0 || (((uintptr_t)a.out2) & 127) != 0)) || (a.lab & (16 | 1024))) return 0;
        if (a.bias) return use192 ? launch_nt3<192, EPI_QGELU, true, true, true>(a, s) : launch_nt3<256, EPI_QGELU, true, true, true>(a, s);
        return use192 ? launch_nt3<192, EPI_QGELU, true, true, false>(a, s) : launch_nt3<256, EPI_QGELU, true, true, false>(a, s);
    }
    if (epilogue == FM_EPI_BF16) {
        if (a.ldo % 8 != 0) return 0;
        if (a.bias) {
            if (a.ldo % 64 != 0 || (((uintptr_t)a.out) & 127) != 0) return 0;
            return use192 ? launch_nt3<192, EPI_BF16, true, true, true>(a, s) : launch_nt3<256, EPI_BF16, true, true, true>(a, s);
        }
        if (!(a.lab & 1024) && !(a.lab & 16) && a.ldo % 64 == 0 && (((uintptr_t)a.out) & 127) == 0)
            return use192 ? launch_nt3<192, EPI_BF16, true, true>(a, s) : launch_nt3<256, EPI_BF16, true, true>(a, s);
        if (!(a.lab & 16)) return use192 ? launch_nt3<192, EPI_BF16, true>(a, s) : launch_nt3<256, EPI_BF16, true>(a, s);
        return use192 ? launch_nt3<192, EPI_BF16>(a, s) : launch_nt3<256, EPI_BF16>(a, s);
    }
    if (epilogue == FM_EPI_RESIDUAL) {
        if (!(a.lab & 256)) return 0;
        if (a.ldo % 4 != 0 || a.ldr % 4 != 0 || !a.res) return 0;
        if (!(a.lab & 16)) return use192 ? launch_nt3<192, EPI_RES, true>(a, s) : launch_nt3<256, EPI_RES, true>(a, s);
        return use192 ? launch_nt3<192, EPI_RES>(a, s) : launch_nt3<256, EPI_RES>(a, s);
    }
    if (epilogue == FM_EPI_SWIGLU_BWD) {
        if (a.N % 16 != 0 || a.Hp % 8 != 0 || a.ldo % 8 != 0 || a.ldr % 8 != 0 || !a.res || a.Hp < a.N) return 0;
        if ((size_t)256 * (size_t)a.ldr * 2 >= 0x7fffffffull) return 0;
        return launch_nt3<256, EPI_SWIGLU_BWD, true>(a, s);
    }
    if (epilogue == FM_EPI_SWIGLU) {
        if (a.N % 64 != 0 || a.Hp % 8 != 0 || a.ldo % 8 != 0 || (a.out2 && a.ldo2 % 8 != 0) || !a.W2) return 0;
        if (!(a.lab & 1024) && !(a.lab & 16) && a.ldo % 64 == 0 && (!a.out2 || a.ldo2 % 64 == 0) && a.Hp % 64 == 0 && a.N % 64 == 0)
            return launch_nt3<256, EPI_SWIGLU, true, true>(a, s);
        if (!(a.lab & 16)) return launch_nt3<256, EPI_SWIGLU, true>(a, s);
        return launch_nt3<256, EPI_SWIGLU>(a, s);
    }
    return 0;
}
```

ml-4m_amd/fourm/hip/_lib.py:

```python
import ctypes as C
import os

FM_MAX_MODS = 24
_LIB_PATH = os.environ.get("FOURM_HIP_LIB") or os.path.join(os.path.dirname(os.path.dirname(os.path.abspath(__file__))), "_lib", "libfourm_hip.so")


class FourmHipUnavailable(ImportError):
    pass


def _load():
    if not os.path.exists(_LIB_PATH):
        raise FourmHipUnavailable(
            f"{_LIB_PATH} is missing - build the gfx950 kernels first: python ml-4m_amd/build_ext.py "
            "(the 4M hot path has no fallback implementation)")
    return C.CDLL(_LIB_PATH)


lib = _load()
lib.fm_last_error.restype = C.c_char_p
lib.fm_abi_version.restype = C.c_int
ABI_VERSION = 11
if lib.fm_abi_version() != ABI_VERSION:
    raise FourmHipUnavailable(f"libfourm_hip.so ABI {lib.fm_abi_version()} != expected {ABI_VERSION}; rebuild")

vp, i32, i64, f32 = C.c_void_p, C.c_int32, C.c_int64, C.c_float

EPI_BF16, EPI_GELU, EPI_RESIDUAL, EPI_SWIGLU, EPI_F32, EPI_TANH, EPI_SWIGLU_BWD, EPI_GELU_BWD, EPI_QUICK_GELU = 0, 1, 2, 3, 4, 5, 6, 7, 8
EPI_RELU, EPI_RELU_BWD = 9, 10
MASK_NONE, MASK_KEYPAD, MASK_DECODER, MASK_DENSE = 0, 1, 2, 3
KIND_TOK, KIND_PATCH, KIND_SEQ, KIND_SEQ_EMB = 0, 1, 2, 3
LOSS_MOD, LOSS_TOKEN = 0, 1


class GemmGroup(C.Structure):
    _fields_ = [("W", vp), ("out", vp), ("N", i32), ("K", i32), ("ldw", i32), ("pad_", i32)]


class GemmNTArgs(C.Structure):
    _fields_ = [("W", vp), ("W2", vp), ("X", vp), ("out", vp), ("out2", vp), ("res", vp), ("bias", vp), ("bias2", vp),
                ("M", i32), ("N", i32), ("K", i32), ("ldw", i32), ("ldx", i32), ("ldo", i32), ("ldo2", i32), ("ldr", i32),
                ("Hp", i32), ("epilogue", i32), ("groups", vp), ("tile_group", vp), ("max_N", i32), ("fixed_tiling", i32),
                ("m_dev", vp), ("row0_dev", vp), ("splitk_ws", vp), ("splitk_ws_bytes", i64),
                ("conv_C", i32), ("conv_H", i32), ("conv_W", i32), ("conv_Ho", i32), ("conv_Wo", i32), ("conv_stride", i32), ("conv_up", i32), ("conv_pad_", i32)]


class GemmTNArgs(C.Structure):
    _fields_ = [("A", vp), ("B", vp), ("out", vp), ("R", i32), ("N", i32), ("K", i32), ("lda", i32), ("ldb", i32),
                ("ldo", i32), ("a_cols", i32), ("b_cols", i32), ("splits", i32), ("force_tr", i32), ("groups", vp),
                ("seg_start", vp), ("seg_count", vp), ("n_groups", i32), ("max_N", i32), ("max_R", i32), ("pad_", i32)]


class GemmTNJob(C.Structure):
    _fields_ = [("A", vp), ("B", vp), ("out", vp), ("R", i32), ("N", i32), ("K", i32), ("lda", i32), ("ldb", i32),
                ("ldo", i32), ("a_cols", i32), ("b_cols", i32)]


TN_MAX_JOBS = 16


class AttnArgs(C.Structure):
    _fields_ = [("Q", vp), ("K", vp), ("V", vp), ("O", vp), ("stat_m", vp), ("stat_l", vp),
                ("ldq", i32), ("ldk", i32), ("ldv", i32), ("ldo", i32),
                ("B", i32), ("H", i32), ("Nq", i32), ("Nk", i32), ("head_dim", i32), ("mask_kind", i32),
                ("scale", f32), ("causal", i32),
                ("kpad", vp), ("cs", vp), ("modq", vp), ("modk", vp), ("dense", vp),
                ("dO", vp), ("dQ", vp), ("dK", vp), ("dV", vp),
                ("lddo", i32), ("lddq", i32), ("lddk", i32), ("lddv", i32), ("force_tr", i32), ("kv_batch_rows", i32), ("zero_attn", i32)]


class AttnDecodeArgs(C.Structure):
    _fields_ = [("q", vp), ("k", vp), ("v", vp), ("o", vp), ("q_w", vp), ("q_b", vp), ("k_w", vp), ("k_b", vp), ("kpad", vp),
                ("ldq", i32), ("ldk", i32), ("ldv", i32), ("ldo", i32),
                ("B", i32), ("H", i32), ("Nk", i32), ("kv_batch_rows", i32), ("k_new_row", i32), ("is_f32", i32), ("zero_attn", i32), ("pad_", i32),
                ("scale", f32), ("eps", f32)]


class ModDesc(C.Structure):
    _fields_ = [("ids", vp), ("mask", vp), ("dam", vp), ("table", vp), ("pos", vp), ("mod_emb", vp), ("proj_bias", vp),
                ("L", i32), ("kind", i32), ("ids_are_i64", i32), ("mod_id", i32), ("max_len", i32), ("shifted", i32),
                ("mask_stride", i32), ("id_stride", i32), ("patch", i32), ("channels", i32), ("grid_w", i32),
                ("orig_dim", i32), ("head_index", i32), ("pad_", i32)]


class ShadowDesc(C.Structure):
    _fields_ = [("src", vp), ("dst", vp), ("ld_src", i32), ("ld_dst", i32), ("rows", i32), ("cols", i32),
                ("transpose", i32), ("tile_start", i32), ("col_scale", vp), ("dst_f32", i32), ("reserved", i32)]


FOLD_MAX_JOBS = 48


class FoldGradJob(C.Structure):
    _fields_ = [("dWp", vp), ("W", vp), ("gamma", vp), ("gW", vp), ("ggamma", vp), ("rows", i32), ("cols", i32), ("ld_dwp", i32), ("reserved", i32)]


class GemmF32Args(C.Structure):
    _fields_ = [("X", vp), ("W", vp), ("W2", vp), ("out", vp), ("out2", vp), ("res", vp), ("bias", vp), ("bias2", vp),
                ("sxm", i64), ("sxk", i64), ("swn", i64), ("swk", i64),
                ("M", i32), ("N", i32), ("K", i32), ("ldo", i32), ("ldo2", i32), ("ldr", i32), ("Hp", i32), ("epilogue", i32),
                ("accumulate", i32), ("max_N", i32), ("seg_rows", i32), ("n_groups", i32),
                ("groups", vp), ("tile_group", vp), ("seg_start", vp), ("seg_count", vp)]


class SpanMaskArgs(C.Structure):
    _fields_ = [("ids", vp), ("len", vp), ("unit", vp), ("noise", vp), ("keep_prob", vp), ("r_choice", vp), ("input_budget", vp), ("target_budget", vp),
                ("sentinel_ids", vp), ("emb", vp), ("emb_out", vp), ("src", vp), ("tensor", vp), ("input_mask", vp), ("target_mask", vp),
                ("decoder_attention_mask", vp), ("tries", vp),
                ("B", i32), ("ld_ids", i32), ("T", i32), ("ld_noise", i32), ("n_sentinels", i32), ("max_tokens", i32), ("vocab_offset", i32), ("pad_id", i32),
                ("emb_rows", i32), ("emb_dim", i32)]


class AdamWJob(C.Structure):
    _fields_ = [("p", vp), ("g", vp), ("m", vp), ("v", vp), ("dst_plain", vp), ("dst_t", vp),
                ("rows", i32), ("cols", i32), ("ld_plain", i32), ("ld_t", i32), ("tile_start", i32), ("pad_", i32)]


class SelectDesc(C.Structure):
    _fields_ = [("mods", ModDesc * FM_MAX_MODS),
                ("n_mods", i32), ("batch", i32), ("dim", i32), ("n_keep", i32), ("n_reg", i32), ("total_len", i32),
                ("is_decoder", i32), ("raw", i32),
                ("reg_tokens", vp), ("mask_token", vp),
                ("tokens", vp), ("emb", vp), ("x0", vp), ("out_mask", vp), ("out_mod", vp), ("slot_mod", vp),
                ("slot_src", vp), ("slot_pos", vp), ("target_ids", vp), ("out_cs", vp), ("out_mod_pre", vp),
                ("out_mod_index", vp), ("patch_rows", vp), ("seqemb_rows", vp), ("patch_ld", i32), ("seqemb_ld", i32),
                ("rows_f32", i32), ("pad2_", i32)]


class EmbedBwdMod(C.Structure):
    _fields_ = [("d_table", vp), ("d_pos", vp), ("d_mod_emb", vp), ("d_proj_bias", vp),
                ("kind", i32), ("has_padding_idx", i32), ("padding_idx", i32), ("pad_", i32)]


class EmbedBwdDesc(C.Structure):
    _fields_ = [("mods", EmbedBwdMod * FM_MAX_MODS), ("dx", vp), ("slot_mod", vp), ("slot_src", vp), ("slot_pos", vp),
                ("d_mask_token", vp), ("d_reg_tokens", vp),
                ("n_mods", i32), ("batch", i32), ("dim", i32), ("Nt", i32), ("lddx", i32), ("is_decoder", i32)]


class EmaJob(C.Structure):
    _fields_ = [("ema", vp), ("model", vp), ("n", i64), ("first_chunk", i64)]


def _sig(name, *argtypes):
    fn = getattr(lib, name)
    fn.argtypes = list(argtypes)
    fn.restype = C.c_int
    return fn


P = C.POINTER
gemm_nt = _sig("fm_gemm_nt", P(GemmNTArgs), vp)
gemm_tn = _sig("fm_gemm_tn", P(GemmTNArgs), vp)
gemm_tn_multi = _sig("fm_gemm_tn_multi", P(GemmTNJob), C.c_int, vp)
layernorm_fwd = _sig("fm_layernorm_fwd", vp, i32, vp, vp, vp, i32, i32, vp, vp, vp, i32, i32, f32, vp)
layernorm_fwd_res = _sig("fm_layernorm_fwd_res", vp, i32, vp, i32, vp, i32, vp, vp, vp, i32, i32, vp, vp, vp, i32, i32, f32, vp)
layernorm_bwd = _sig("fm_layernorm_bwd", vp, i32, vp, vp, i32, vp, vp, vp, vp, vp, i32, vp, i32, vp, vp, i32, i32, vp)
layernorm_bwd_h = _sig("fm_layernorm_bwd_h", vp, i32, vp, i32, vp, i32, vp, vp, vp, vp, vp, i32, vp, i32, vp, i32, i32, vp)
attn_fwd = _sig("fm_attn_fwd", P(AttnArgs), vp)
attn_bwd = _sig("fm_attn_bwd", P(AttnArgs), vp)
attn_decode = _sig("fm_attn_decode", P(AttnDecodeArgs), vp)
ATTN_DECODE_MAX_NK = 8192
select_embed = _sig("fm_select_embed", P(SelectDesc), vp)
embed_bwd = _sig("fm_embed_bwd", P(EmbedBwdDesc), vp)
dense_decoder_mask = _sig("fm_dense_decoder_mask", vp, vp, vp, i32, i32, i32, i32, i32, vp)
segment_rows = _sig("fm_segment_rows", vp, i32, i32, vp, vp, vp, vp, vp, i32, vp)
gather_rows = _sig("fm_gather_rows", vp, i32, vp, vp, i32, i32, i32, vp)
cross_entropy = _sig("fm_cross_entropy", vp, i32, vp, vp, vp, vp, vp, vp, vp, i32, i32, i32, i32, vp, vp, vp, vp, i32, vp)
swiglu_bwd = _sig("fm_swiglu_bwd", vp, i32, vp, i32, vp, i32, i32, i32, i32, vp)
gelu_bwd = _sig("fm_gelu_bwd", vp, i32, vp, i32, vp, i32, i32, i32, i32, vp)
cast_pad = _sig("fm_cast_pad", vp, i32, vp, i32, i32, i32, vp)
transpose_cast_pad = _sig("fm_transpose_cast_pad", vp, i32, vp, i32, i32, i32, i32, vp)
colsum = _sig("fm_colsum", vp, i32, vp, i32, i32, vp)
shadow_refresh = _sig("fm_shadow_refresh", vp, i32, i32, vp)
fold_colscale_grad = _sig("fm_fold_colscale_grad", vp, i32, vp)
headnorm_fwd = _sig("fm_headnorm_fwd", vp, i32, vp, vp, vp, i32, vp, i32, i32, C.c_float, vp)
headnorm_bwd = _sig("fm_headnorm_bwd", vp, i32, vp, i32, vp, vp, vp, i32, vp, vp, i32, i32, vp)
f32_to_bf16 = _sig("fm_f32_to_bf16", vp, vp, i64, vp)
bf16_to_f32_scaled = _sig("fm_bf16_to_f32_scaled", vp, vp, i64, f32, vp)
add_bf16_f32 = _sig("fm_add_bf16_f32", vp, vp, vp, i64, vp)
lib.fm_set_reserved_cus.argtypes = [C.c_int]
lib.fm_get_reserved_cus.restype = C.c_int
lib.fm_get_reserved_cus.argtypes = []
adamw = _sig("fm_adamw", vp, vp, vp, vp, i64, f32, f32, f32, f32, f32, i64, vp, vp, vp, vp)
adamw_shadow = _sig("fm_adamw_shadow", vp, i32, i32, f32, f32, f32, f32, f32, i64, vp, vp, vp, vp)
sumsq = _sig("fm_sumsq", vp, i64, vp, vp)
clip_coef = _sig("fm_clip_coef", vp, f32, vp, vp, vp)
sample_tokens = _sig("fm_sample_tokens", vp, i32, i32, i32, i32, f32, i32, f32, vp, vp, vp, vp)
maskgit_commit = _sig("fm_maskgit_commit", vp, vp, vp, i32, i32, i32, vp, i32, i32, vp, vp, vp, vp)
gemm_f32 = _sig("fm_gemm_f32", P(GemmF32Args), vp)
attn_f32_fwd = _sig("fm_attn_f32_fwd", P(AttnArgs), vp)
attn_f32_bwd = _sig("fm_attn_f32_bwd", P(AttnArgs), vp)
layernorm_bwd_f32 = _sig("fm_layernorm_bwd_f32", vp, i32, vp, vp, i32, vp, vp, vp, vp, vp, i32, vp, i32, vp, vp, i32, i32, vp)
headnorm_f32_fwd = _sig("fm_headnorm_f32_fwd", vp, i32, vp, vp, vp, i32, vp, i32, i32, C.c_float, vp)
headnorm_f32_bwd = _sig("fm_headnorm_f32_bwd", vp, i32, vp, i32, vp, vp, vp, i32, vp, vp, i32, i32, vp)
swiglu_bwd_f32 = _sig("fm_swiglu_bwd_f32", vp, i32, vp, i32, vp, i32, i32, i32, i32, vp)
gelu_bwd_f32 = _sig("fm_gelu_bwd_f32", vp, i32, vp, i32, vp, i32, i32, i32, vp)
colsum_f32 = _sig("fm_colsum_f32", vp, i32, vp, i32, i32, vp)
cross_entropy_f32 = _sig("fm_cross_entropy_f32", vp, i32, vp, vp, vp, vp, vp, vp, vp, i32, i32, i32, i32, vp, vp, vp, vp, i32, vp)
vq_patchify = _sig("fm_vq_patchify", vp, vp, i32, i32, i32, i32, i32, i32, vp)
l2norm_rows = _sig("fm_l2norm_rows", vp, i32, vp, i32, i32, i32, vp)
vq_assign = _sig("fm_vq_assign", vp, i32, vp, vp, i32, i32, i32, i32, i32, vp, vp, i32, vp, vp, vp)
lib.fm_set_tn_transpose_read.argtypes = [C.c_int]
lib.fm_set_gemm_tn_config.argtypes = [C.c_int]
lib.fm_set_attn_transpose_read.argtypes = [C.c_int]

lib.fm_set_gemm_nt_config.argtypes = [C.c_int]
lib.fm_lab_set.argtypes = [C.c_int, C.c_int]
lib.fm_lab_set.restype = None
vq_code_stats = _sig("fm_vq_code_stats", vp, i32, vp, i32, i32, i32, vp, vp, vp)
vq_ema_update = _sig("fm_vq_ema_update", vp, vp, vp, vp, i32, i32, f32, vp)
vq_code_bias = _sig("fm_vq_code_bias", vp, i32, i32, vp, vp)
vq_assign_bias = _sig("fm_vq_assign_bias", vp, i32, vp, vp, vp, i32, i32, i32, i32, i32, vp, vp, i32, vp, vp, vp)
vq_code_stats_raw = _sig("fm_vq_code_stats_raw", vp, i32, vp, i32, i32, i32, vp, vp, vp)
vq_ema_update_euclid = _sig("fm_vq_ema_update_euclid", vp, vp, vp, vp, vp, vp, i32, i32, f32, f32, vp)
vq_unpatchify = _sig("fm_vq_unpatchify", vp, i32, vp, i32, i32, i32, i32, i32, vp)
VQ_WIDE_TILE, CONVNEXT_MAX_C = 128, 4
vq_assign_wide = _sig("fm_vq_assign_wide", vp, i32, vp, vp, i32, i32, i32, i32, vp, vp, i32, vp, vp, vp)
memcodes_assign = _sig("fm_memcodes_assign", vp, i32, vp, vp, i32, i32, i32, i32, i32, vp, vp, i32, vp, vp, vp)
convnext_block = _sig("fm_convnext_block", vp, vp, vp, vp, vp, vp, vp, vp, vp, vp, vp, i32, i32, i32, i32, f32, vp)
vq_latent_grad = _sig("fm_vq_latent_grad", vp, i32, vp, vp, vp, i32, vp, f32, vp, i32, vp, i32, i32, vp)
tanh_bwd_f32 = _sig("fm_tanh_bwd_f32", vp, vp, vp, i32, i32, i32, vp)
embed_rows_f32 = _sig("fm_embed_rows_f32", vp, vp, vp, i32, i32, i32, vp)
vq_patchify_ex = _sig("fm_vq_patchify_ex", vp, vp, vp, vp, vp, vp, i32, i32, i32, i32, i32, i32, vp)
vq_cls_emb_bwd = _sig("fm_vq_cls_emb_bwd", vp, i32, vp, vp, i32, i32, i32, i32, i32, vp)
vq_latent_grad_normalized = _sig("fm_vq_latent_grad_normalized", vp, i32, vp, vp, vp, i32, vp, f32, vp, i32, vp, i32, i32, vp)
scale_rows_bf16 = _sig("fm_scale_rows_bf16", vp, i32, vp, i32, i32, i32, vp)
image_mask = _sig("fm_image_mask", vp, vp, vp, i32, i32, vp, vp, vp, vp)
token_budgets = _sig("fm_token_budgets", vp, vp, vp, vp, vp, vp, vp, i32, i32, i32, i32, vp, vp, vp)
span_mask = _sig("fm_span_mask", P(SpanMaskArgs), vp)
guidance_combine = _sig("fm_guidance_combine", vp, i32, i32, vp, i32, i32, f32, vp, i32, i32, i32, i32, vp)
unpack_image_u8 = _sig("fm_unpack_image_u8", vp, vp, i32, i32, i32, i32, P(C.c_float), P(C.c_float), vp)
unpack_ids_u16 = _sig("fm_unpack_ids_u16", vp, vp, i64, vp)
unpack_mask_bits = _sig("fm_unpack_mask_bits", vp, vp, i32, i32, vp)
decoder_attention_from_target = _sig("fm_decoder_attention_from_target", vp, vp, i32, i32, vp)
split3_bf16 = _sig("fm_split3_bf16", vp, i32, vp, i32, i32, i32, i32, i32, vp)
unet_im2col = _sig("fm_unet_im2col", vp, i32, i32, vp, i32, i32, i32, i32, vp, i32, i32, i32, i32, i32, i32, i32, i32, vp)
groupnorm_nhwc = _sig("fm_groupnorm_nhwc", vp, i32, vp, i32, vp, vp, vp, i32, vp, i32, i32, i32, i32, f32, i32, vp)
add_bf16 = _sig("fm_add_bf16", vp, i32, vp, i32, vp, i32, i64, i32, vp)
silu_f32_to_bf16 = _sig("fm_silu_f32_to_bf16", vp, vp, i64, vp)
timestep_embedding = _sig("fm_timestep_embedding", vp, vp, i32, i32, i32, f32, vp)
unet_attention = _sig("fm_unet_attention", vp, i32, vp, i32, i32, i32, i32, i32, vp)
unet_im2col_f32 = _sig("fm_unet_im2col_f32", vp, i32, i32, vp, i32, i32, i32, i32, vp, i32, i32, i32, i32, i32, i32, i32, i32, vp)
groupnorm_nhwc_f32 = _sig("fm_groupnorm_nhwc_f32", vp, i32, vp, i32, vp, vp, vp, i32, i32, i32, i32, i32, f32, i32, vp)
unet_attention_f32 = _sig("fm_unet_attention_f32", vp, i32, vp, i32, i32, i32, i32, i32, vp)
add_f32 = _sig("fm_add_f32", vp, i32, vp, i32, vp, i32, i64, i32, vp)
silu_f32 = _sig("fm_silu_f32", vp, vp, i64, vp)
timestep_embedding_f32 = _sig("fm_timestep_embedding_f32", vp, vp, i32, i32, i32, f32, vp)
unet_col2im_f32 = _sig("fm_unet_col2im_f32", vp, i32, vp, i32, i32, i32, i32, i32, i32, i32, i32, i32, vp)
groupnorm_nhwc_bwd_f32 = _sig("fm_groupnorm_nhwc_bwd_f32", vp, i32, vp, i32, vp, i32, vp, vp, vp, i32, vp, vp, vp, i32, vp, i32, i32, i32, i32, f32, i32, vp)
unet_attention_bwd_f32 = _sig("fm_unet_attention_bwd_f32", vp, i32, vp, i32, vp, i32, vp, i32, i32, i32, i32, vp)
silu_bwd_f32 = _sig("fm_silu_bwd_f32", vp, vp, vp, i64, vp)
diffusion_x0 = _sig("fm_diffusion_x0", vp, vp, f32, f32, vp, i64, vp)
quantile_abs = _sig("fm_quantile_abs", vp, i32, i64, f32, vp, vp)
diffusion_step = _sig("fm_diffusion_step", vp, vp, f32, f32, vp, vp, vp, f32, f32, f32, f32, vp, vp, i32, i64, vp)
lora_apply = _sig("fm_lora_apply", vp, i32, vp, i64, i64, vp, i64, i64, vp, i32, f32, vp, i32, i32, i32, i32, i32, i32, vp)
lora_grad = _sig("fm_lora_grad", vp, i32, vp, vp, i64, i64, f32, i32, i32, i32, i32, i32, vp)
vit_patch_rows = _sig("fm_vit_patch_rows", vp, vp, i32, i32, i32, i32, i32, i32, i32, vp)
vit_emb_rows = _sig("fm_vit_emb_rows", vp, vp, vp, i32, i32, i32, i32, vp)
vit_colsum = _sig("fm_vit_colsum", vp, i32, vp, i32, i32, vp, i64, vp)
clip_embed_ln = _sig("fm_clip_embed_ln", vp, i32, i32, vp, vp, vp, vp, vp, i32, i32, i32, i32, f32, vp)
FEAT_COSINE, FEAT_L1 = 0, 1
feat_distance = _sig("fm_feat_distance", vp, i32, vp, i32, i32, i32, i32, i32, vp, vp, i32, vp)
quick_gelu_bwd = _sig("fm_quick_gelu_bwd", vp, i32, vp, i32, vp, i32, i32, i32, i32, vp)
quick_gelu_bwd_f32 = _sig("fm_quick_gelu_bwd_f32", vp, i32, vp, i32, vp, i32, i32, i32, vp)
clip_embed_ln_bwd = _sig("fm_clip_embed_ln_bwd", vp, i32, vp, i32, i32, vp, vp, vp, i32, i32, i32, i32, f32, vp)
tap_add = _sig("fm_tap_add", vp, i32, vp, i32, vp, i32, vp, i32, i32, i32, vp)
LPIPS_CHUNK = 64
lpips_stem = _sig("fm_lpips_stem", vp, vp, vp, vp, vp, vp, i32, i32, i32, i32, i32, vp)
lpips_stem_bwd = _sig("fm_lpips_stem_bwd", vp, i32, i32, vp, vp, vp, vp, i32, i32, i32, vp)
maxpool2x2_nhwc = _sig("fm_maxpool2x2_nhwc", vp, i32, vp, i32, i32, i32, i32, i32, i32, vp)
lpips_distance = _sig("fm_lpips_distance", vp, i32, vp, i32, i32, vp, i32, i32, i32, vp, vp, i32, vp, vp)
lpips_tap_bwd = _sig("fm_lpips_tap_bwd", vp, i32, vp, i32, vp, i32, vp, i32, vp, i32, i32, i32, i32, i32, i32, vp)
LOSS_MSE, LOSS_L1, LOSS_SMOOTH_L1, LOSS_CE_INDEX, LOSS_BCE, LOSS_COSINE, LOSS_COSINE_1D = 0, 1, 2, 3, 4, 5, 6
RECONST_CHUNK, EMA_CHUNK, TOKEN_USAGE_MAX_K = 4096, 4096, 1 << 20
reconst_loss_scratch = _sig("fm_reconst_loss_scratch", i32, i32, i32, i64)
reconst_loss = _sig("fm_reconst_loss", vp, vp, i32, i32, i32, i64, vp, vp, vp, vp)
scale_f32 = _sig("fm_scale_f32", vp, vp, i64, vp)
mask_out_samples = _sig("fm_mask_out_samples", vp, vp, f32, vp, i32, i32, i64, vp)
ema_update = _sig("fm_ema_update", vp, i32, i64, f32, f32, vp)
diffusion_pair = _sig("fm_diffusion_pair", vp, vp, vp, vp, vp, i32, vp, vp, i32, i64, vp)
token_usage = _sig("fm_token_usage", vp, i32, i64, i64, i32, vp, vp, vp)
EXPORTS = ["fm_reconst_loss_scratch", "fm_reconst_loss", "fm_scale_f32", "fm_mask_out_samples", "fm_ema_update", "fm_diffusion_pair", "fm_token_usage", "fm_lpips_stem", "fm_lpips_stem_bwd", "fm_maxpool2x2_nhwc", "fm_lpips_distance", "fm_lpips_tap_bwd", "fm_feat_distance", "fm_quick_gelu_bwd", "fm_quick_gelu_bwd_f32", "fm_clip_embed_ln_bwd", "fm_tap_add", "fm_clip_embed_ln", "fm_attn_decode", "fm_vit_patch_rows", "fm_vit_emb_rows", "fm_vit_colsum", "fm_lora_apply", "fm_lora_grad", "fm_vq_assign_wide", "fm_memcodes_assign", "fm_convnext_block", "fm_split3_bf16", "fm_unet_im2col", "fm_groupnorm_nhwc", "fm_add_bf16", "fm_silu_f32_to_bf16", "fm_timestep_embedding", "fm_unet_attention", "fm_diffusion_x0", "fm_quantile_abs",
           "fm_diffusion_step", "fm_unpack_image_u8", "fm_unpack_ids_u16", "fm_unpack_mask_bits", "fm_decoder_attention_from_target", "fm_guidance_combine", "fm_image_mask", "fm_token_budgets", "fm_span_mask", "fm_vq_code_stats", "fm_vq_ema_update", "fm_vq_code_bias", "fm_vq_assign_bias", "fm_vq_code_stats_raw", "fm_vq_ema_update_euclid", "fm_vq_unpatchify", "fm_vq_latent_grad", "fm_tanh_bwd_f32", "fm_embed_rows_f32", "fm_vq_patchify_ex", "fm_vq_cls_emb_bwd", "fm_vq_latent_grad_normalized", "fm_abi_version", "fm_last_error", "fm_gemm_nt", "fm_set_gemm_nt_config", "fm_get_gemm_nt_config", "fm_set_reserved_cus", "fm_get_reserved_cus", "fm_bf16_to_f32_scaled", "fm_add_bf16_f32", "fm_scale_rows_bf16", "fm_gemm_tn", "fm_gemm_tn_multi", "fm_set_gemm_tn_config", "fm_get_gemm_tn_config", "fm_set_tn_transpose_read",
           "fm_get_tn_transpose_read", "fm_layernorm_fwd", "fm_layernorm_fwd_res", "fm_layernorm_bwd", "fm_layernorm_bwd_h", "fm_headnorm_fwd", "fm_headnorm_bwd", "fm_attn_fwd", "fm_attn_bwd",
           "fm_set_attn_transpose_read", "fm_get_attn_transpose_read", "fm_select_embed", "fm_embed_bwd",
           "fm_dense_decoder_mask", "fm_segment_rows", "fm_gather_rows", "fm_cross_entropy", "fm_swiglu_bwd",
           "fm_gelu_bwd", "fm_cast_pad", "fm_transpose_cast_pad", "fm_shadow_refresh", "fm_fold_colscale_grad", "fm_colsum", "fm_f32_to_bf16", "fm_adamw", "fm_adamw_shadow",
           "fm_sumsq", "fm_clip_coef", "fm_vq_patchify", "fm_l2norm_rows", "fm_vq_assign",
           "fm_sample_tokens", "fm_maskgit_commit", "fm_gemm_f32", "fm_attn_f32_fwd", "fm_attn_f32_bwd", "fm_layernorm_bwd_f32", "fm_headnorm_f32_fwd", "fm_headnorm_f32_bwd",
           "fm_swiglu_bwd_f32", "fm_gelu_bwd_f32", "fm_colsum_f32", "fm_cross_entropy_f32", "fm_lab_set",
           "fm_unet_im2col_f32", "fm_groupnorm_nhwc_f32", "fm_unet_attention_f32", "fm_add_f32", "fm_silu_f32", "fm_timestep_embedding_f32",
           "fm_unet_col2im_f32", "fm_groupnorm_nhwc_bwd_f32", "fm_unet_attention_bwd_f32", "fm_silu_bwd_f32"]


def check(rc: int):
    if rc != 0:
        raise RuntimeError(f"libfourm_hip: {lib.fm_last_error().decode()} (rc={rc})")
```

ml-4m_amd/fourm/hip/engine.py:

```python
import math
import os
import random
import weakref
from typing import Dict, List, Optional

import torch
import torch.nn as nn

from . import _lib as L
from . import ops

_WEIGHT_EPOCH = 0
FUSE_ACT_BWD = os.environ.get("FOURM_FUSE_ACT_BWD", "0") == "1"
HEADS_DENSE = os.environ.get("FOURM_HEADS_DENSE", "1") == "1"
HEADS_DENSE_MAX = int(os.environ.get("FOURM_HEADS_DENSE_MAX", "8"))
DEFER_RESIDUAL = os.environ.get("FOURM_DEFER_RESIDUAL", "1") == "1"
HOIST_CTX = os.environ.get("FOURM_HOIST_CTX", "1") == "1"
LN_BWD_FROM_H = os.environ.get("FOURM_LN_BWD_FROM_H", "1") == "1"
DP_RESERVE_ALWAYS = os.environ.get("FOURM_DP_RESERVE_ALWAYS", "0") == "1"


def bump_weight_epoch():
    global _WEIGHT_EPOCH
    _WEIGHT_EPOCH += 1


def ru(x, m):
    return (x + m - 1) // m * m


def is_lora(lin) -> bool:
    return hasattr(lin, "lora_down")


def check_lora_targets(model):
    from fourm.models.lora_utils import MAX_LORA_WIDTH, LoRAWrapper
    ok = set()
    for blk in model.encoder:
        ok |= {id(blk.attn.qkv), id(blk.attn.proj)}
    for blk in getattr(model, "decoder", ()):
        ok |= {id(blk.self_attn.qkv), id(blk.self_attn.proj), id(blk.cross_attn.q), id(blk.cross_attn.kv), id(blk.cross_attn.proj)}
    for name, mod in model.named_modules():
        if not isinstance(mod, LoRAWrapper):
            continue
        if id(mod) not in ok:
            raise NotImplementedError(f"LoRA wrapper at '{name}': the HIP engine adapts the attention Linears of the encoder / decoder blocks only "
                                      "(the MLP's fc1 / fc3 run as one launch whose SwiGLU epilogue consumes the pre-activation; embeddings and "
                                      "heads have no low-rank path)")
        width = mod.lora_down.weight.shape[0]
        if width > MAX_LORA_WIDTH:
            raise NotImplementedError(f"LoRA wrapper at '{name}': rank x packed Linears = {width} exceeds {MAX_LORA_WIDTH}")


class Shadow:
    __slots__ = ("buf", "params", "jobs", "stamp")

    def __init__(self, buf, params, jobs):
        self.buf, self.params, self.jobs, self.stamp = buf, params, jobs, None


class Workspace:

    def __init__(self, device, per_stream: bool = False):
        self.device = device
        self.per_stream = per_stream
        self.bufs: Dict[tuple, torch.Tensor] = {}

    def get(self, name, shape, dtype):
        key = (name, tuple(shape), dtype, torch.cuda.current_stream(self.device).cuda_stream) if self.per_stream else (name, tuple(shape), dtype)
        t = self.bufs.get(key)
        if t is None:
            t = self.bufs[key] = torch.zeros(shape, dtype=dtype, device=self.device)
        return t

    def nbytes(self):
        return sum(t.numel() * t.element_size() for t in self.bufs.values())


def fill_mod_desc(md, d, emb, is_dec: bool, mod_id: int, head_index: int = 0, raw: int = 0, name: str = "modality"):
    kind = emb.kind
    t = d["tensor"]
    B = t.shape[0]
    mask = d["target_mask" if is_dec else "input_mask"]
    mask = mask.reshape(B, -1)
    if mask.dtype != torch.bool:
        mask = mask.bool()
    mask = mask.contiguous()
    keep = [mask]
    md.mask, md.mask_stride = mask.data_ptr(), mask.shape[1]
    md.kind, md.mod_id, md.head_index = kind, mod_id, head_index
    md.pos = emb.pos_emb.data_ptr()
    md.mod_emb = emb.mod_emb.data_ptr()
    md.shifted = 1 if (is_dec and kind == L.KIND_SEQ and raw != 2) else 0
    md.max_len = getattr(emb, "max_length", 0) or 0
    if kind in (L.KIND_TOK, L.KIND_SEQ):
        ids = t.reshape(B, -1)
        if ids.dtype not in (torch.int32, torch.int64):
            ids = ids.long()
# ... 582 lines not shown
        ckpt = save and self.checkpointing
        for i, blk in enumerate(m.encoder):
            if ckpt:
                st["enc_layers"].append(dict(ckpt_in=x))
                x = self.encoder_block_fwd(blk, x, B, N, emask, None, f"enc{i % 2}", defer_out=True, out_name=f"enc{i}.x_out")
                st["enc_layers"][-1]["dp"] = self._last_dp
                continue
            sv = {} if save else None
            x = self.encoder_block_fwd(blk, x, B, N, emask, sv, f"enc{i}" if save else f"enc{i % 2}", defer_out=True)
            if save:
                st["enc_layers"].append(sv)
        R, Rp, D = B * N, x.shape[0], self.D
        sv_top = {} if save else None
        xn = self._ln(m.encoder_norm, x, self._buf(sv_top, "top", "xn", (Rp, D), self.adt), R, sv_top, "en", "top")
        ctx = self._buf(sv_top, "top", "ctx", (Rp, D), torch.float32)
        pc = m.decoder_proj_context
        ops.gemm_nt(xn, self.w(pc.weight), ctx, epilogue=L.EPI_RESIDUAL, res=enc["emb"], bias=pc.bias, M=R, N=D, K=D)
        return x, ctx, emask, sv_top

    def trunk_forward(self, enc, dec, save: bool):
        m = self.model
        B, N, Mt = enc["B"], enc["Nt"], dec["Nt"]
        st = dict(enc_layers=[], dec_layers=[]) if save else None
        x, ctx, emask, sv_top = self.encode_context(enc, st)
        y = dec["x0"]
        smask = self.decoder_mask(dec["cs"], dec["mod_pre"]) if "cs" in dec else dec["sa_mask"]
        ctx_hat, sv_hat = None, None
        if self.hoist_ctx:
            sv_hat = {} if save else None
            ctx_hat = self._ln(self._unit_norm(), ctx, self._buf(sv_hat, "top", "ctx_hat", (ctx.shape[0], self.D), self.adt), B * N, sv_hat, "ch", "top")
        for i, blk in enumerate(m.decoder):
            if save and self.checkpointing:
                st["dec_layers"].append(dict(ckpt_in=y))
                y = self.decoder_block_fwd(blk, y, ctx, B, Mt, N, smask, emask, None, f"dec{i % 2}", defer_out=i + 1 < len(m.decoder),
                                           out_name=f"dec{i}.y_out", ctx_hat=ctx_hat)
                st["dec_layers"][-1]["dp"] = self._last_dp
                continue
            sv = {} if save else None
            y = self.decoder_block_fwd(blk, y, ctx, B, Mt, N, smask, emask, sv, f"dec{i}" if save else f"dec{i % 2}",
                                       defer_out=i + 1 < len(m.decoder), ctx_hat=ctx_hat)
            if save:
                st["dec_layers"].append(sv)
        if save:
            st.update(top=sv_top, x_final=x, y_final=y, ctx=ctx, emask=emask, smask=smask, ctx_hat=ctx_hat, sv_hat=sv_hat)
        return y, st

    def heads_setup(self, dec, y_final, save):
        m = self.model
        heads = dec["heads"]
        nH = len(heads)
        B, Mt, D = dec["B"], dec["Nt"], self.D
        R = B * Mt
        Rp = ops.padded_rows(R, nH)
        ws, dev, i32 = self.ws, self.device, torch.int32
        hs = dict(n=nH, Rp=Rp, heads=heads)
        hs["seg_start"], hs["seg_count"] = ws.get("heads.seg_start", (nH,), i32), ws.get("heads.seg_count", (nH,), i32)
        hs["perm"], hs["r2p"] = ws.get("heads.perm", (Rp,), i32), ws.get("heads.r2p", (R,), i32)
        hs["tile_group"] = ws.get("heads.tile_group", (Rp // ops.SEG,), i32)
        ops.segment_rows(dec["head_of_row"].view(-1), nH, hs["seg_start"], hs["seg_count"], hs["perm"], hs["r2p"], hs["tile_group"])
        sv = {} if save else None
        yp = ws.get("heads.yp", (Rp, D), self.adt)
        with ops._prof("fills"):
            yp.zero_()
        self._ln(m.decoder_norm, y_final, yp, R, sv, "dn", "heads", row_map=hs["r2p"])
        vocabs = [m.decoder_embeddings[h].vocab_size for h in heads]
        hs["vocabs"], hs["maxV"] = vocabs, max(vocabs)
        ldl = ru(hs["maxV"], 64)
        w_fwd = [self.w(m.decoder_embeddings[h].to_logits.weight) for h in heads]
        w_bwd = [self.wt(m.decoder_embeddings[h].to_logits.weight) for h in heads] if save else None
        key = tuple(t.data_ptr() for t in w_fwd) + (tuple(t.data_ptr() for t in w_bwd) if save else ())
        cache = getattr(self, "_head_groups", None)
        if cache is None or cache[0] != key:
            fwd = ops.make_groups([dict(W=t, N=v, K=D, ldw=D) for t, v in zip(w_fwd, vocabs)], dev)
            if self.fp32:
                bwd = ops.make_groups([dict(W=m.decoder_embeddings[h].to_logits.weight, N=D, K=v, ldw=D, transposed=1)
                                       for h, v in zip(heads, vocabs)], dev) if save else None
            else:
                bwd = ops.make_groups([dict(W=t, N=D, K=ru(v, 64), ldw=ru(v, 64)) for t, v in zip(w_bwd, vocabs)], dev) if save else None
            vt = torch.tensor(vocabs, dtype=i32, device=dev)
            self._head_groups = cache = (key, fwd, bwd, vt)
        hs["g_fwd"], hs["g_bwd"], hs["vocab_t"] = cache[1], cache[2], cache[3]
        logits = ws.get("heads.logits", (Rp, ldl), self.adt)
        if HEADS_DENSE and not self.fp32 and nH <= HEADS_DENSE_MAX and ops.heads_dense_ok(w_fwd, vocabs, logits):
            ops.gemm_nt_heads(yp, w_fwd, vocabs, hs["seg_start"], hs["seg_count"], logits, D)
        else:
            ops.gemm_nt_grouped(yp, hs["g_fwd"], hs["tile_group"], logits, hs["maxV"], max_K=D)
        hs.update(yp=yp, logits=logits, sv=sv)
        hs["row_loss"] = ws.get("heads.row_loss", (Rp,), torch.float32)
        hs["row_lse"] = ws.get("heads.row_lse", (Rp,), torch.float32)
        hs["head_loss"] = ws.get("heads.head_loss", (nH,), torch.float32)
        hs["total"] = ws.get("heads.total", (1,), torch.float32)
        return hs

    def loss_forward(self, dec, hs, loss_type):
        lt = L.LOSS_MOD if loss_type in ("mod", "modality") else L.LOSS_TOKEN
        hs["loss_type"] = lt
        ops.cross_entropy(hs["logits"], hs["perm"], hs["tile_group"], dec["target_ids"].view(-1), hs["vocab_t"], hs["seg_start"],
                          hs["seg_count"], hs["n"], hs["maxV"], hs["row_loss"], hs["row_lse"], hs["head_loss"], hs["total"], loss_type=lt)
        return hs["total"], hs["head_loss"]

    def dec_order(self, mod_dict):
        names = [n for n in mod_dict if n in self.model.decoder_embeddings]
        return random.sample(names, len(names))

    def train_forward(self, mod_dict, n_enc, n_dec, loss_type, save=True):
        if loss_type not in ("mod", "modality", "token"):
            raise ValueError("Invalid loss type")
        self.prepare()
        if save:
            self._ensure_flat()
        enc_names = [n for n in mod_dict if n in self.model.encoder_embeddings]
        enc = self.select(mod_dict, n_enc, False, enc_names, "enc.")
        dec = self.select(mod_dict, n_dec, True, self.dec_order(mod_dict), "dec.")
        y, st = self.trunk_forward(enc, dec, save)
        hs = self.heads_setup(dec, y, save)
        total, head_loss = self.loss_forward(dec, hs, loss_type)
        if save:
            self._ctx = dict(enc=enc, dec=dec, st=st, hs=hs)
        return total, head_loss, hs["heads"], hs["seg_count"]

    def _g(self, p):
        return self.grad_view(p) if p.requires_grad else None

    def _dW(self, dy, x, lin, R64, n_cols=None, dy_cols=None):
        g = self._g(lin.weight)
        N = lin.weight.shape[0] if n_cols is None else n_cols
        if g is not None:
            if self._dw_jobs is not None:
                self._dw_jobs.append((dy, x, g.view(g.shape[0], -1), N, lin.weight[0].numel(), R64))
            else:
                ops.gemm_tn(dy, x, g.view(g.shape[0], -1), N=N, K=lin.weight[0].numel(), R=R64)
        if lin.bias is not None and lin.bias.requires_grad:
            ops.colsum(dy, self.grad_view(lin.bias), N, R=R64)

    def _flush_dW(self):
        jobs, self._dw_jobs = self._dw_jobs, None
        if jobs:
            ops.gemm_tn_multi(jobs)

    def _ln_bwd(self, norm, dy, x, sv, key, g, g_bf, R, dres, dy_row_map=None):
        dw = self._g(norm.weight)
        db = self._g(norm.bias) if isinstance(norm.bias, nn.Parameter) else None
        ops.layernorm_bwd(dy, x, norm.weight, sv[key + ".mu"], sv[key + ".rs"], g, dres=dres, dx_bf16=g_bf, dw=dw, db=db,
                          dy_row_map=dy_row_map, R=R, h=sv.get(key + ".h"))

    def _mlp_bwd(self, mlp, sv, g_bf, R, Rp):
        bf, D, Hp, Hd = self.adt, self.D, self.Hp, self.Hd
        R64 = R
        ws = self.ws
        self._dW(g_bf, sv["act"], mlp.fc2, R64)
        dh = ws.get("bwd.dh", (Rp, D), bf)
        fuse = FUSE_ACT_BWD and self.act != "quick_gelu"
        if not fuse:
            da = ws.get("bwd.da", (Rp, Hp), bf)
            padN = not self.fp32 and Hp != Hd
            ops.gemm_nt(g_bf, self.wt(mlp.fc2.weight, padN), da, M=R, N=Hp if padN else Hd, K=D)
        if self.gated:
            dgu = ws.get("bwd.dgu", (Rp, 2 * Hp), bf)
            if fuse:
                ops.gemm_nt(g_bf, self.wt(mlp.fc2.weight), dgu, M=R, N=Hd, K=D, epilogue=L.EPI_SWIGLU_BWD, res=sv["gu"], Hp=Hp)
            else:
                ops.swiglu_bwd(da, sv["gu"], dgu, Hd, Hp, R=R)
            self._dW(dgu[:, :Hp], sv["h2"], mlp.fc1, R64, n_cols=Hd)
            self._dW(dgu[:, Hp:], sv["h2"], mlp.fc3, R64, n_cols=Hd)
            if self.fp32:
                ops.gemm_nt(dgu[:, :Hp], self.wt(mlp.fc1.weight), dh, M=R, N=D, K=Hd)
                ops.gemm_nt(dgu[:, Hp:], self.wt(mlp.fc3.weight), dh, M=R, N=D, K=Hd, epilogue=L.EPI_F32, res=dh)
# ... 81 lines not shown
            ops.attn_bwd(sv["q"], kv[:, :D], kv[:, D:], sv["o2"], do, dq, dkv[:, :D], dkv[:, D:], B, self.H, M, N, self.scale,
                         sv["sm2"], sv["sl2"], zero_attn=getattr(xa, "allow_zero_attn", False), **xa_mask)
        self._dW(dq, sv["hq"], xa.q, Rq)
        dhq = ws.get("bwd.dh", (Rqp, D), bf)
        ops.gemm_nt(dq, self.wt(xa.q.weight), dhq, M=Rq, N=D, K=D)
        self._lora_bwd(xa.q, dq, sv["hq"], dhq, sv.get("lora.q"), Rq)
        g_bf = ws.get("bwd.dec.gbf2", tuple(g_in.shape), g_in.dtype)
        self._ln_bwd(blk.query_norm, dhq, sv["y1"], sv, "nq", g, g_bf, Rq, dres=g)
        if dp:
            ops.scale_rows_bf16(g_bf, dp[0], M, Rq)
        if hoist is None:
            self._dW(dkv, sv["hc"], xa.kv, Rc)
            dhc = ws.get("bwd.dhc", (Rcp, D), bf)
            ops.gemm_nt(dkv, self.wt(xa.kv.weight), dhc, M=Rc, N=D, K=2 * D)
            self._lora_bwd(xa.kv, dkv, sv["hc"], dhc, sv.get("lora.kv"), Rc)
            self._ln_bwd(blk.context_norm, dhc, ctx, sv, "nc", dctx, dctx_bf, Rc, dres=dctx)
        elif xa.kv.weight.requires_grad or blk.context_norm.weight.requires_grad:
            self._dw_jobs.append((dkv, hoist[1], hoist[2], 2 * D, D, Rc))
        dh = self._self_attn_bwd(blk.self_attn, sv, g_bf, B, M, Rq, Rqp, sa_mask)
        self._flush_dW()
        self._ln_bwd(blk.norm1, dh, sv["y_in"], sv, "n1", g, g_in, Rq, dres=g)

    def _embed_bwd(self, sel, dx, dx_extra, is_dec):
        m = self.model
        embs = m.decoder_embeddings if is_dec else m.encoder_embeddings
        d = L.EmbedBwdDesc()
        for i, n in enumerate(sel["names"]):
            e, md = embs[n], d.mods[i]
            md.kind = e.kind
            if e.kind in (L.KIND_TOK, L.KIND_SEQ) and not (is_dec and e.kind == L.KIND_TOK):
                w = e.token_emb.weight
                md.d_table = self.grad_view(w).data_ptr() if w.requires_grad else None
                pad = e.token_emb.padding_idx
                md.has_padding_idx, md.padding_idx = (1, pad) if pad is not None else (0, 0)
            if isinstance(e.pos_emb, nn.Parameter) and e.pos_emb.requires_grad:
                md.d_pos = self.grad_view(e.pos_emb).data_ptr()
            if e.mod_emb.requires_grad:
                md.d_mod_emb = self.grad_view(e.mod_emb).data_ptr()
            if e.kind == L.KIND_SEQ_EMB and e.emb_proj.bias.requires_grad:
                md.d_proj_bias = self.grad_view(e.emb_proj.bias).data_ptr()
        d.dx, d.lddx = dx.data_ptr(), dx.stride(0)
        d.slot_mod, d.slot_src, d.slot_pos = sel["slot_mod"].data_ptr(), sel["slot_src"].data_ptr(), sel["slot_pos"].data_ptr()
        if is_dec and m.mask_token.requires_grad:
            d.d_mask_token = self.grad_view(m.mask_token).data_ptr()
        if not is_dec and m.num_register_tokens and m.register_tokens.requires_grad:
            d.d_reg_tokens = self.grad_view(m.register_tokens).data_ptr()
        d.n_mods, d.batch, d.dim, d.Nt, d.is_decoder = len(sel["names"]), sel["B"], self.D, sel["Nt"], 1 if is_dec else 0
        with ops._prof("embed_bwd"):
            L.check(L.embed_bwd(ops.C.byref(d), ops._stream()))
        if dx_extra is not None:
            d2 = L.EmbedBwdDesc()
            ops.C.memmove(ops.C.byref(d2), ops.C.byref(d), ops.C.sizeof(d))
            for i in range(d.n_mods):
                d2.mods[i].d_table = None
                d2.mods[i].d_proj_bias = None
            d2.d_reg_tokens = None
            d2.dx, d2.lddx = dx_extra.data_ptr(), dx_extra.stride(0)
            with ops._prof("embed_bwd"):
                L.check(L.embed_bwd(ops.C.byref(d2), ops._stream()))

    def train_backward(self, grad_scale: torch.Tensor):
        c = self._ctx
        if c is None:
            raise RuntimeError("train_backward without a preceding training forward")
        self._ctx, self._dw_jobs = None, None
        if self.reducer is not None:
            self.reducer.begin()
            if getattr(self.reducer, "reserved_cus", 0):
                L.lib.fm_set_reserved_cus(int(self.reducer.reserved_cus))
        m, ws = self.model, self.ws
        enc, dec, st, hs = c["enc"], c["dec"], c["st"], c["hs"]
        B, N, Mt, D = enc["B"], enc["Nt"], dec["Nt"], self.D
        bf, f32 = self.adt, torch.float32
        Rq, Rc = B * Mt, B * N
        Rqp, Rcp = st["y_final"].shape[0], st["x_final"].shape[0]
        ops.cross_entropy(hs["logits"], hs["perm"], hs["tile_group"], dec["target_ids"].view(-1), hs["vocab_t"], hs["seg_start"],
                          hs["seg_count"], hs["n"], hs["maxV"], hs["row_loss"], hs["row_lse"], hs["head_loss"], hs["total"],
                          loss_type=hs["loss_type"], grad_scale=grad_scale, write_grad=True)
        dyp = ws.get("bwd.dyp", (hs["Rp"], D), bf)
        ops.gemm_nt_grouped(hs["logits"], hs["g_bwd"], hs["tile_group"], dyp, D, max_K=ru(hs["maxV"], 64))
        heads = [m.decoder_embeddings[h] for h in hs["heads"]]
        if any(h.to_logits.weight.requires_grad for h in heads):
            outs = [self.grad_view(h.to_logits.weight) if h.to_logits.weight.requires_grad else None for h in heads]
            key = tuple(o.data_ptr() if o is not None else 0 for o in outs)
            cache = getattr(self, "_head_tn_groups", None)
            if cache is None or cache[0] != key:
                cache = self._head_tn_groups = (key, ops.make_groups(
                    [dict(out=o, N=(v if o is not None else 0)) for o, v in zip(outs, hs["vocabs"])], self.device))
            tn = cache[1]
            ops.gemm_tn_grouped(hs["logits"], hs["yp"], tn, hs["seg_start"], hs["seg_count"], hs["n"], hs["maxV"], hs["Rp"], D)
        g = ws.get("bwd.g_dec", (Rqp, D), f32)
        g_bf = ws.get("bwd.g_dec_bf", (Rqp, D), bf)
        self._ln_bwd(m.decoder_norm, dyp, st["y_final"], hs["sv"], "dn", g, g_bf, Rq, dres=None, dy_row_map=hs["r2p"])
        self._stage("heads")
        dctx = ws.get("bwd.dctx", (Rcp, D), f32)
        dctx_bf = ws.get("bwd.dctx_bf", (Rcp, D), bf)
        Ld = len(m.decoder)
        ctx_hat = st.get("ctx_hat")
        if ctx_hat is None:
            with ops._prof("fills"):
                dctx.zero_()
        else:
            dkv_all = ws.get("bwd.dkv_all", (Rcp, Ld * 2 * D), bf)
            dwp = ws.get("bwd.dwp", (Ld, 2 * D, D), f32)
            with ops._prof("fills"):
                dwp.zero_()
        for i in reversed(range(Ld)):
            sv = st["dec_layers"][i]
            if "ckpt_in" in sv:
                y_in, dp, sv = sv["ckpt_in"], sv["dp"], {}
                self.decoder_block_fwd(m.decoder[i], y_in, st["ctx"], B, Mt, N, st["smask"], st["emask"], sv, "ckpt", out_name="ckpt.out", dp=dp,
                                       ctx_hat=ctx_hat)
            hoist = None if ctx_hat is None else (dkv_all[:, i * 2 * D:(i + 1) * 2 * D], ctx_hat, dwp[i])
            self.decoder_block_bwd(m.decoder[i], sv, g, g_bf, dctx, dctx_bf, st["ctx"], B, Mt, N, st["smask"], st["emask"], hoist=hoist)
            self._stage(f"dec{i}")
        if ctx_hat is not None and Ld:
            dxh = ws.get("bwd.dhc", (Rcp, D), bf)
            ops.gemm_nt(dkv_all, self.wt_fold_stack(), dxh, M=Rc, N=D, K=Ld * 2 * D)
            self._ln_bwd(self._unit_norm(), dxh, st["ctx"], st["sv_hat"], "ch", dctx, dctx_bf, Rc, dres=None)
            jobs = [(dwp[i], b.cross_attn.kv.weight.detach(), b.context_norm.weight.detach(), self._g(b.cross_attn.kv.weight), self._g(b.context_norm.weight))
                    for i, b in enumerate(m.decoder) if b.cross_attn.kv.weight.requires_grad or b.context_norm.weight.requires_grad]
            if jobs:
                ops.fold_colscale_grad(jobs)
        self._embed_bwd(dec, g, None, True)
        self._stage("dec_emb")
        top = st["top"]
        if len(m.decoder) == 0:
            ops.f32_to_bf16(dctx, dctx_bf)
        self._dW(dctx_bf, top["xn"], m.decoder_proj_context, Rc)
        dxn = ws.get("bwd.dh", (Rcp, D), bf)
        ops.gemm_nt(dctx_bf, self.wt(m.decoder_proj_context.weight), dxn, M=Rc, N=D, K=D)
        ge = ws.get("bwd.g_enc", (Rcp, D), f32)
        ge_bf = ws.get("bwd.g_enc_bf", (Rcp, D), bf)
        self._ln_bwd(m.encoder_norm, dxn, st["x_final"], top, "en", ge, ge_bf, Rc, dres=None)
        self._stage("ctx")
        for i in reversed(range(len(m.encoder))):
            sv = st["enc_layers"][i]
            if "ckpt_in" in sv:
                x_in, dp, sv = sv["ckpt_in"], sv["dp"], {}
                self.encoder_block_fwd(m.encoder[i], x_in, B, N, st["emask"], sv, "ckpt", out_name="ckpt.out", dp=dp)
            self.encoder_block_bwd(m.encoder[i], sv, ge, ge_bf, B, N, st["emask"])
            self._stage(f"enc{i}")
        for n in enc["names"]:
            e = m.encoder_embeddings[n]
            if e.kind == L.KIND_PATCH and e.proj.weight.requires_grad:
                ops.gemm_tn(ge_bf, enc["patch_rows"], self.grad_view(e.proj.weight), N=D, K=e.proj.weight.shape[1], R=Rc)
            elif e.kind == L.KIND_SEQ_EMB and e.emb_proj.weight.requires_grad:
                ops.gemm_tn(ge_bf, enc["seqemb_rows"], self.grad_view(e.emb_proj.weight), N=D, K=e.emb_proj.weight.shape[1], R=Rc)
        self._embed_bwd(enc, ge, dctx, False)
        if self.reducer is not None:
            self.reducer.finish()
            if getattr(self.reducer, "reserved_cus", 0) and not DP_RESERVE_ALWAYS:
                L.lib.fm_set_reserved_cus(0)
```

ml-4m_amd/fourm/hip/ops.py:

```python
import contextlib
import ctypes as C
import threading
from typing import Optional

import torch

from . import _lib as L

_PROFILER = None


def set_profiler(p):
    global _PROFILER
    _PROFILER = p


class _Null:
    def __enter__(self):
        return self

    def __exit__(self, *a):
        return False


# ... 76 lines not shown
        return _gemm_f32(x, w, out, epilogue=epilogue, bias=bias, res=res, w2=w2, bias2=bias2, out2=out2, Hp=Hp, N=N, K=K, M=M)
    a = L.GemmNTArgs()
    a.W, a.W2, a.X, a.out, a.out2 = _p(w), _p(w2), _p(x), _p(out), _p(out2)
    a.res, a.bias, a.bias2 = _p(res), _p(bias), _p(bias2)
    a.M = x.shape[0] if M is None else M
    a.N = w.shape[0] if N is None else N
    a.K = w.shape[1] if K is None else K
    a.ldw, a.ldx, a.ldo = _ld(w), _ld(x), _ld(out)
    a.ldo2 = _ld(out2) if out2 is not None else 0
    a.ldr = _ld(res) if res is not None else 0
    a.Hp, a.epilogue = Hp, epilogue
    if conv is not None:
        a.conv_C, a.conv_H, a.conv_W, a.conv_Ho, a.conv_Wo = conv["C"], conv["H"], conv["W"], conv["Ho"], conv["Wo"]
        a.conv_stride, a.conv_up = conv.get("stride", 1), conv.get("up", 0)
    if conv is None and getattr(_TILING, "fixed", False):
        a.fixed_tiling = 1
    elif epilogue == L.EPI_BF16 and a.M * a.N <= SPLITK_MAX_OUT and a.K >= 512:
        ws = _splitk_ws(x.device)
        a.splitk_ws, a.splitk_ws_bytes = ws.data_ptr(), ws.numel() * 4
    two = 2 if epilogue == L.EPI_SWIGLU else 1
    nbytes = 2.0 * a.K * (a.M + two * a.N) + a.M * a.N * two * out.element_size()
    nbytes += (a.M * a.N * 4.0 if res is not None and epilogue in (L.EPI_RESIDUAL, L.EPI_F32) else 0.0) + (a.M * a.N * 4.0 if out2 is not None else 0.0)
    with _prof(f"gemm_nt/epi{epilogue}", 2.0 * a.M * a.N * a.K * two, nbytes, tag=f"M{a.M} N{a.N} K{a.K}"):
        L.check(L.gemm_nt(C.byref(a), _stream()))
    return out


def _gemm_f32(x, w, out, *, epilogue=L.EPI_BF16, bias=None, res=None, w2=None, bias2=None, out2=None, Hp=0, N=None, K=None, M=None,
              accumulate=False):
    assert w.dtype == torch.float32 and out.dtype == torch.float32 and x.stride(1) == 1 and out.stride(1) == 1
    a = L.GemmF32Args()
    a.X, a.W, a.W2, a.out, a.out2, a.res, a.bias, a.bias2 = _p(x), _p(w), _p(w2), _p(out), _p(out2), _p(res), _p(bias), _p(bias2)
    a.M = x.shape[0] if M is None else M
    a.N = w.shape[0] if N is None else N
    a.K = min(w.shape[1] if K is None else K, w.shape[1])
    a.sxm, a.sxk, a.swn, a.swk = x.stride(0), 1, w.stride(0), w.stride(1)
    if w2 is not None:
        assert w2.stride() == w.stride()
    a.ldo, a.ldo2, a.ldr = out.stride(0), out2.stride(0) if out2 is not None else 0, res.stride(0) if res is not None else 0
    a.Hp, a.epilogue, a.accumulate = Hp, epilogue, 1 if accumulate else 0
    with _prof("gemm_f32", 2.0 * a.M * a.N * a.K * (2 if epilogue == L.EPI_SWIGLU else 1), 4.0 * (a.K * (a.M + a.N) + a.M * a.N), tag=f"M{a.M} N{a.N} K{a.K}"):
        L.check(L.gemm_f32(C.byref(a), _stream()))
    return out


@_timed("heads_gemm_nt (logits, dY)")
def gemm_nt_grouped(x, groups, tile_group, out, max_N, M=None, max_K=0):
    if x.dtype == torch.float32:
        a = L.GemmF32Args()
        a.X, a.out, a.groups, a.tile_group = _p(x), _p(out), _p(groups), _p(tile_group)
        a.M, a.N, a.max_N, a.seg_rows = (x.shape[0] if M is None else M), max_N, max_N, SEG
        a.sxm, a.sxk, a.ldo, a.epilogue = x.stride(0), 1, out.stride(0), L.EPI_BF16
        L.check(L.gemm_f32(C.byref(a), _stream()))
        return out
    a = L.GemmNTArgs()
    a.X, a.out = _p(x), _p(out)
    a.M = x.shape[0] if M is None else M
    a.K = max_K
    a.ldx, a.ldo = _ld(x), _ld(out)
    a.epilogue = L.EPI_BF16
    a.groups, a.tile_group, a.max_N = _p(groups), _p(tile_group), max_N
    L.check(L.gemm_nt(C.byref(a), _stream()))
    return out


def heads_dense_ok(ws, vocabs, out):
    return (out.dtype == torch.bfloat16 and all(v % 8 == 0 for v in vocabs) and all(w.dtype == torch.bfloat16 and w.shape[1] % 64 == 0 for w in ws)
            and _ld(out) % 64 == 0 and out.data_ptr() % 128 == 0)


@_timed("heads_gemm_nt (logits, dY)")
def gemm_nt_heads(x, ws, vocabs, seg_start, seg_count, out, K):
    for h, (w, v) in enumerate(zip(ws, vocabs)):
        a = L.GemmNTArgs()
        a.W, a.X, a.out = _p(w), _p(x), _p(out)
        a.M, a.N, a.K = x.shape[0], v, K
        a.ldw, a.ldx, a.ldo = _ld(w), _ld(x), _ld(out)
        a.epilogue = L.EPI_BF16
        a.m_dev, a.row0_dev = seg_count.data_ptr() + 4 * h, seg_start.data_ptr() + 4 * h
        L.check(L.gemm_nt(C.byref(a), _stream()))
    return out


def gemm_tn(a_mat, b_mat, out, *, N=None, K=None, R=None, splits=0, force_tr=-1, a_cols=0, b_cols=0):
    if a_mat.dtype == torch.float32:
        g = L.GemmF32Args()
        g.X, g.W, g.out = _p(a_mat), _p(b_mat), _p(out)
        g.M = a_mat.shape[1] if N is None else N
        g.N = b_mat.shape[1] if K is None else K
        g.K = a_mat.shape[0] if R is None else R
        g.sxm, g.sxk, g.swn, g.swk = 1, a_mat.stride(0), 1, b_mat.stride(0)
        g.ldo, g.epilogue, g.accumulate = _ld(out), L.EPI_BF16, 1
        L.check(L.gemm_f32(C.byref(g), _stream()))
        return out
    a = L.GemmTNArgs()
    a.A, a.B, a.out = _p(a_mat), _p(b_mat), _p(out)
    a.R = a_mat.shape[0] if R is None else R
    a.N = a_mat.shape[1] if N is None else N
    a.K = b_mat.shape[1] if K is None else K
    a.lda, a.ldb, a.ldo = _ld(a_mat), _ld(b_mat), _ld(out)
    a.a_cols = a_cols or a_mat.shape[1]
    a.b_cols = b_cols or b_mat.shape[1]
    a.splits, a.force_tr = splits, force_tr
    with _prof("gemm_tn", 2.0 * a.R * a.N * a.K, 2.0 * a.R * (a.N + a.K) + 4.0 * a.N * a.K, tag=f"R{a.R} N{a.N} K{a.K}"):
        L.check(L.gemm_tn(C.byref(a), _stream()))
    return out


def gemm_tn_multi(jobs):
    if not jobs:
        return
    if jobs[0][0].dtype == torch.float32:
        for a_mat, b_mat, out, N, K, R in jobs:
            gemm_tn(a_mat, b_mat, out, N=N, K=K, R=R)
        return
    for lo in range(0, len(jobs), L.TN_MAX_JOBS):
        part = jobs[lo:lo + L.TN_MAX_JOBS]
        arr = (L.GemmTNJob * len(part))()
        flops = 0.0
        for j, (a_mat, b_mat, out, N, K, R) in zip(arr, part):
            j.A, j.B, j.out = _p(a_mat), _p(b_mat), _p(out)
            j.R, j.N, j.K = R, N, K
            j.lda, j.ldb, j.ldo = _ld(a_mat), _ld(b_mat), _ld(out)
            j.a_cols, j.b_cols = a_mat.shape[1], b_mat.shape[1]
            flops += 2.0 * R * N * K
        with _prof("gemm_tn_multi", flops, 0.0, tag=f"jobs{len(part)} R{part[0][5]}"):
            L.check(L.gemm_tn_multi(arr, len(part), _stream()))


@_timed("heads_gemm_tn (dW)")
def gemm_tn_grouped(a_mat, b_mat, groups, seg_start, seg_count, n_groups, max_N, max_R, K, *, splits=0, force_tr=-1):
    if a_mat.dtype == torch.float32:
        g = L.GemmF32Args()
        g.X, g.W, g.groups, g.seg_start, g.seg_count = _p(a_mat), _p(b_mat), _p(groups), _p(seg_start), _p(seg_count)
        g.N, g.max_N, g.n_groups = K, max_N, n_groups
        g.sxm, g.sxk, g.swn, g.swk = 1, a_mat.stride(0), 1, b_mat.stride(0)
        g.ldo, g.epilogue, g.accumulate = K, L.EPI_BF16, 1
        L.check(L.gemm_f32(C.byref(g), _stream()))
        return
    a = L.GemmTNArgs()
    a.A, a.B = _p(a_mat), _p(b_mat)
    a.K = K
    a.lda, a.ldb, a.ldo = _ld(a_mat), _ld(b_mat), K
    a.a_cols, a.b_cols = a_mat.shape[1], b_mat.shape[1]
    a.splits, a.force_tr = splits, force_tr
    a.groups, a.seg_start, a.seg_count = _p(groups), _p(seg_start), _p(seg_count)
    a.n_groups, a.max_N, a.max_R = n_groups, max_N, max_R
    L.check(L.gemm_tn(C.byref(a), _stream()))


def make_groups(entries, device):
    arr = (L.GemmGroup * len(entries))()
    for i, e in enumerate(entries):
        arr[i].W = e["W"].data_ptr() if e.get("W") is not None else None
        arr[i].out = e["out"].data_ptr() if e.get("out") is not None else None
        arr[i].N, arr[i].K, arr[i].ldw = e["N"], e.get("K", 0), e.get("ldw", 0)
        arr[i].pad_ = e.get("transposed", 0)
    host = torch.frombuffer(bytearray(bytes(arr)), dtype=torch.uint8)
    return host.to(device)


def layernorm_fwd(x, w, b, y, mean=None, rstd=None, row_map=None, eps=1e-6, R=None, delta=None, x_out=None):
    R = x.shape[0] if R is None else R
    if delta is not None:
        with _prof("layernorm_fwd", 0.0, R * w.numel() * (10 + y.element_size())):
            L.check(L.layernorm_fwd_res(_p(x), _ld(x), _p(delta), _ld(delta), _p(x_out), _ld(x_out), _p(w), _p(b), _p(y), _ld(y),
# ... 470 lines not shown
```

Before: 1.169 million tokens/s.

## Batch per-head logits and head-weight-gradient GEMMs into single job-list launches

Adds a job-list variant of the nt3 GEMM kernel so all output-head logit GEMMs (one per modality, each with device-side row segments) run in one launch instead of one launch per head. Adds device-side row windows to the TN multi-job kernel so head weight gradients are computed per-head over only that head's segment rows, replacing the padded grouped TN path. The aim is to cut launch count and tail underutilization across the 7 small head GEMMs, and to skip padded rows in the dW reduction. The windowed TN path disables the t4 kernel and the tail split heuristics, which could lose some efficiency.

New measurement: 1.172 million tokens/s (median of 5 runs). No clear change (+0.3%).

```diff
diff --git a/include/fourm_hip.h b/include/fourm_hip.h
--- a/include/fourm_hip.h
+++ b/include/fourm_hip.h
@@ -41,6 +41,12 @@
     int32_t conv_C, conv_H, conv_W, conv_Ho, conv_Wo, conv_stride, conv_up, conv_pad_;
 } fm_gemm_nt_args;
 int fm_gemm_nt(const fm_gemm_nt_args* args, void* stream);
+typedef struct fm_gemm_nt_job {
+    const void* W;
+    int32_t N, ldw;
+} fm_gemm_nt_job;
+int fm_gemm_nt_list(const void* X, int ldx, void* out, int ldo, int K, const fm_gemm_nt_job* jobs, int n_jobs, const int32_t* row0_dev,
+                    const int32_t* m_dev, void* stream);
 void fm_set_gemm_nt_config(int cfg);
 int fm_get_gemm_nt_config(void);
 void fm_set_reserved_cus(int n);
@@ -57,6 +63,7 @@
 typedef struct fm_gemm_tn_job {
     const void* A; const void* B; void* out;
     int32_t R, N, K, lda, ldb, ldo, a_cols, b_cols;
+    const int32_t* row0_dev; const int32_t* rows_dev;
 } fm_gemm_tn_job;
 int fm_gemm_tn_multi(const fm_gemm_tn_job* jobs, int n_jobs, void* stream);
 void fm_set_gemm_tn_config(int cfg);
diff --git a/ml-4m_amd/csrc/gemm.hip b/ml-4m_amd/csrc/gemm.hip
--- a/ml-4m_amd/csrc/gemm.hip
+++ b/ml-4m_amd/csrc/gemm.hip
@@ -739,7 +739,7 @@
 }
 
 
-template <bool MASKED, int TA = 128, int KB = 64, bool LS = false>
+template <bool MASKED, int TA = 128, int KB = 64, bool LS = false, bool WIN = false>
 __global__ __launch_bounds__(512) void gemm_tn_multi_kernel(TNMultiArgs a) {
     constexpr int TB = 256, WB = 4, STAGES = LS ? 2 : 3, NWAVES = 8;
     constexpr int FWA = TA / 2 / 32;
@@ -775,7 +775,16 @@
         const int local = tile - jb.tile_start;
         const int n0 = (local / jb.n_tiles_b) * TA, k0 = (local % jb.n_tiles_b) * TB;
         const bf16_t* A = jb.A; const bf16_t* B = jb.B;
-        const int lda = jb.lda, ldb = jb.ldb, a_cols = jb.a_cols, b_cols = jb.b_cols, r_lim = jb.R;
+        const int lda = jb.lda, ldb = jb.ldb, a_cols = jb.a_cols, b_cols = jb.b_cols;
+        int r_lim = jb.R;
+        if constexpr (WIN) {
+            static_assert(!WIN || MASKED || LS, "row windows: masked reductions");
+            r_lim = min(max(a.win_rows[j][0], 0), jb.R);
+            const size_t r0w = (size_t)a.win_row0[j][0];
+            A += r0w * lda; B += r0w * ldb;
+            t_end = (r_lim + KB - 1) / KB;
+            if (t_end <= 0) return;
+        }
 
 #if defined(__HIP_DEVICE_COMPILE__)
         if constexpr (LS) {
@@ -995,7 +1004,7 @@
                 }
         }
     };
-    tn_multi_walk(a, w, G, run);
+    tn_multi_walk<WIN>(a, w, G, run);
 }
 
 int g_nt_config = 9, g_nt_prio = 1;
@@ -1108,6 +1117,8 @@
 }
 
 }
+
+int fm_nt3_lab() { return g_lab[3]; }
 
 extern "C" int fm_gemm_nt(const fm_gemm_nt_args* p, void* stream) {
     FM_CHECK_ARG(p && p->X && p->out, "fm_gemm_nt: null pointer");
@@ -1346,7 +1357,9 @@
     long long units = 0;
     static const bool small_env = [] { const char* e = getenv("FOURM_TN_MULTI_TILE"); return e && atoi(e) == 128; }();
     const bool big = !(small_env || g_tn_config == 3);
-    bool t4 = big && g_lab[5] != 0 && (g_tn_config == 1 || g_tn_config == 4);
+    bool windowed = false;
+    for (int i = 0; i < n_jobs; ++i) windowed = windowed || jobs[i].rows_dev || jobs[i].row0_dev;
+    bool t4 = big && g_lab[5] != 0 && (g_tn_config == 1 || g_tn_config == 4) && !windowed;
     if (t4) {
         double useful = 0, padded = 0;
         for (int i = 0; i < n_jobs && t4; ++i) {
@@ -1365,11 +1378,14 @@
         const fm_gemm_tn_job& p = jobs[i];
         FM_CHECK_ARG(p.A && p.B && p.out, "fm_gemm_tn_multi: null pointer");
         FM_CHECK_ARG(p.K > 0 && p.N > 0 && p.R > 0, "fm_gemm_tn_multi: bad shape");
+        FM_CHECK_ARG(!p.rows_dev == !p.row0_dev, "fm_gemm_tn_multi: row0_dev and rows_dev go together");
         FM_CHECK_ARG(p.lda % 8 == 0 && p.ldb % 8 == 0, "fm_gemm_tn_multi: leading dims must be multiples of 8");
         TNJob& j = a.job[i];
         j.A = (const bf16_t*)p.A; j.B = (const bf16_t*)p.B; j.out = (float*)p.out;
         j.R = p.R; j.N = p.N; j.K = p.K; j.lda = p.lda; j.ldb = p.ldb; j.ldo = p.ldo;
         j.a_cols = p.a_cols > 0 ? p.a_cols : p.lda; j.b_cols = p.b_cols > 0 ? p.b_cols : p.ldb;
+        FM_CHECK_ARG(!windowed || p.rows_dev, "fm_gemm_tn_multi: either every job of a list has a device row window or none");
+        a.win_row0[i] = p.row0_dev; a.win_rows[i] = p.rows_dev;
         FM_CHECK_ARG(j.a_cols >= 8 && j.b_cols >= 8, "fm_gemm_tn_multi: operands need at least 8 readable columns");
         j.n_tiles_b = (p.K + tb - 1) / tb;
         j.tiles = ((p.N + ta - 1) / ta) * j.n_tiles_b;
@@ -1379,12 +1395,13 @@
         units += (long long)j.tiles * j.kt;
         masked = masked || p.R % kb != 0;
     }
+    masked = masked || windowed;
     a.n_jobs = n_jobs; a.tiles = tiles; a.lab = g_lab[6];
     int grid = n_compute_units();
     if (units / 8 < grid) grid = (int)((units / 8 + 7) / 8 * 8);
     if (grid < 8) grid = 8;
     {
-        const int rem = tiles % grid, ntail = grid - rem;
+        const int rem = windowed ? 0 : tiles % grid, ntail = grid - rem;
         a.tail_rr = rem >= ntail;
         double c = ls ? (a.tail_rr ? 12.0 : 64.0) : big ? (a.tail_rr ? 24.0 : 128.0) : 8.0;
         if (t4 && g_lab[7] > 0) c = g_lab[7];
@@ -1422,20 +1439,27 @@
         }
     }
     hipStream_t s = (hipStream_t)stream;
-#define LAUNCH_TNM(MK, TAV, KBV, ...)                                                                                         \
+#define LAUNCH_TNM(MK, TAV, KBV, ...) LAUNCH_TNM_W(false, MK, TAV, KBV, __VA_ARGS__)
+#define LAUNCH_TNM_W(WINV, MK, TAV, KBV, ...)                                                                                       \
     {                                                                                                                         \
         constexpr bool lsv = sizeof(#__VA_ARGS__) > 1;                                                                        \
         constexpr size_t lds = (size_t)(lsv ? 2 : 3) * KBV * (TAV + 256) * 2;                                                 \
-        auto k = gemm_tn_multi_kernel<MK, TAV, KBV, lsv>;                                                                     \
+        auto k = gemm_tn_multi_kernel<MK, TAV, KBV, lsv, WINV>;                                                                  \
         static bool once = (hipFuncSetAttribute((const void*)k, hipFuncAttributeMaxDynamicSharedMemorySize, (int)lds), true); \
         (void)once;                                                                                                           \
         hipLaunchKernelGGL(k, dim3(grid), dim3(512), lds, s, a);                                                              \
     }
+    if (windowed) {
+        if (ls) LAUNCH_TNM_W(true, false, 256, 64, ls)
+        else if (big) LAUNCH_TNM_W(true, true, 256, 32)
+        else LAUNCH_TNM_W(true, true, 128, 64)
+    } else
     if (t4) fm_launch_tn4_multi(a, grid, s);
     else if (ls) LAUNCH_TNM(false, 256, 64, ls)
     else if (big) { if (masked) LAUNCH_TNM(true, 256, 32) else LAUNCH_TNM(false, 256, 32) }
     else { if (masked) LAUNCH_TNM(true, 128, 64) else LAUNCH_TNM(false, 128, 64) }
 #undef LAUNCH_TNM
+#undef LAUNCH_TNM_W
     FM_CHECK_LAUNCH("fm_gemm_tn_multi");
     return 0;
 }
diff --git a/ml-4m_amd/csrc/gemm_args.h b/ml-4m_amd/csrc/gemm_args.h
--- a/ml-4m_amd/csrc/gemm_args.h
+++ b/ml-4m_amd/csrc/gemm_args.h
@@ -25,6 +25,13 @@
     int lab;
 };
 
+constexpr int NT_LIST_MAX = 16;
+struct NTListJob { const bf16_t* W; int N, ldw, n_tiles_w, pad_; };
+struct NTListArgs : NTArgs {
+    NTListJob job[NT_LIST_MAX];
+    int n_jobs;
+};
+
 __device__ __forceinline__ float gelu_f(float x) { return 0.5f * x * (1.0f + erf_fast(x * 0.70710678118654752f)); }
 __device__ __forceinline__ float quick_gelu_f(float x) { return x * __builtin_amdgcn_rcpf(1.0f + __expf(-1.702f * x)); }
 template <int EPI> constexpr bool is_gelu_like = EPI == EPI_GELU || EPI == EPI_QGELU;
@@ -44,11 +51,20 @@
     int n_jobs, tiles, tail_rr, banded;
     int hybrid;
     int lab;
+    const int* win_row0[FM_TN_MAX_JOBS]; const int* win_rows[FM_TN_MAX_JOBS];
 };
 
 
-template <typename Run>
+template <bool WHOLE = false, typename Run>
 __device__ __forceinline__ void tn_multi_walk(const TNMultiArgs& a, int w, int G, Run&& run) {
+    if constexpr (WHOLE) {
+        for (int tile = w; tile < a.tiles; tile += G) {
+            int j = 0;
+            while (j + 1 < a.n_jobs && tile >= a.job[j + 1].tile_start) ++j;
+            run(tile, 0, a.job[j].kt);
+        }
+        return;
+    }
     auto job_of = [&](int tile) {
         int j = 0;
         while (j + 1 < a.n_jobs && tile >= a.job[j + 1].tile_start) ++j;
@@ -118,4 +134,5 @@
 int fm_launch_nt4(const fmk::NTArgs& a, int epilogue, int mode, hipStream_t s);
 int fm_launch_nt_skinny(const fmk::NTArgs& a, int epilogue, hipStream_t s);
 int fm_grid_cus();
+int fm_nt3_lab();
 int fm_launch_tn4_multi(const fmk::TNMultiArgs& a, int grid, hipStream_t s);
diff --git a/ml-4m_amd/csrc/gemm_nt3.hip b/ml-4m_amd/csrc/gemm_nt3.hip
--- a/ml-4m_amd/csrc/gemm_nt3.hip
+++ b/ml-4m_amd/csrc/gemm_nt3.hip
@@ -14,8 +14,8 @@
 }
 constexpr uint32_t OOB = 0x80000000u;
 
-template <int TW, int EPI, bool SPLIT = false, bool STG = false, bool BIAS = false, bool DEVM = false>
-__global__ __launch_bounds__(512) void gemm_nt3_kernel(NTArgs a) {
+template <int TW, int EPI, bool SPLIT = false, bool STG = false, bool BIAS = false, bool DEVM = false, bool LIST = false>
+__global__ __launch_bounds__(512) void gemm_nt3_kernel(std::conditional_t<LIST, NTListArgs, NTArgs> a) {
 #if defined(__HIP_DEVICE_COMPILE__)
     if constexpr (DEVM) {
         static_assert(EPI == EPI_BF16, "device-side row ranges: bf16 outputs only");
@@ -25,6 +25,18 @@
         a.X += r0 * a.ldx;
         a.out = (char*)a.out + r0 * a.ldo * 2;
         if (a.n_tiles_w * a.n_tiles_x <= (int)blockIdx.x) return;
+    }
+    int list_total = 0;
+    int list_pre[NT_LIST_MAX];
+    (void)list_pre;
+    if constexpr (LIST) {
+        static_assert(EPI == EPI_BF16 && !DEVM, "job lists: bf16 outputs only");
+#pragma unroll
+        for (int h = 0; h < NT_LIST_MAX; ++h) {
+            list_pre[h] = list_total;
+            if (h < a.n_jobs) list_total += a.job[h].n_tiles_w * ((a.m_dev[h] + 255) >> 8);
+        }
+        if (list_total <= (int)blockIdx.x) return;
     }
     constexpr int TX = 256, KB = 64, WW = 2, WX = 4, NWAVES = 8, KS = 4;
     constexpr int RB = 128, CPR = 8, RPP = 8;
@@ -44,7 +56,7 @@
     const int frow = lane & 31, fhi = lane >> 5;
     const int fswz = (frow >> 1) & (CPR - 1);
 
-    const int total = a.n_tiles_w * a.n_tiles_x;
+    const int total = LIST ? list_total : a.n_tiles_w * a.n_tiles_x;
     if (a.dephase_groups > 1) {
         const int ph = ((int)blockIdx.x / 8) % a.dephase_groups;
         for (int i = 0; i < ph * a.dephase_step; ++i) __builtin_amdgcn_s_sleep(32);
@@ -52,14 +64,28 @@
     const int n_my = (total - (int)blockIdx.x + (int)gridDim.x - 1) / (int)gridDim.x;
     const int KT = a.K / KB;
     const int G = n_my * KT;
-    const int N = a.N;
+    int N = a.N;
 
     uint32_t woff[PW], xoff[PX];
     __amdgpu_buffer_rsrc_t rs_w = rsrc_of(a.W), rs_w2 = rsrc_of(a.W2 ? a.W2 : a.W), rs_x = rsrc_of(a.X);
     (void)rs_w2;
-    const int gw = a.group_w;
+    const int gw = LIST ? 0 : a.group_w;
     const bool grouped_order = gw > 0 && total % 8 == 0 && a.n_tiles_x % 8 == 0 && a.n_tiles_w % gw == 0;
-    auto tile_origin = [&](int j, int& n0, int& m0) {
+    struct TileSrc { const bf16_t* W; int N, ldw; };
+    auto tile_origin = [&](int j, int& n0, int& m0, TileSrc& ts) {
+        if constexpr (LIST) {
+            const int id = (int)blockIdx.x + j * (int)gridDim.x;
+            int h = 0, start = 0;
+#pragma unroll
+            for (int i = 1; i < NT_LIST_MAX; ++i)
+                if (i < a.n_jobs && id >= list_pre[i]) { h = i; start = list_pre[i]; }
+            const int ntw = a.job[h].n_tiles_w, cnt = ntw * ((a.m_dev[h] + 255) >> 8);
+            int local = xcd_remap(id - start, cnt);
+            if (a.reverse) local = cnt - 1 - local;
+            ts.W = a.job[h].W; ts.N = a.job[h].N; ts.ldw = a.job[h].ldw;
+            n0 = (local % ntw) * NPT; m0 = a.row0_dev[h] + (local / ntw) * TX;
+            return;
+        }
         int tile = xcd_remap((int)blockIdx.x + j * (int)gridDim.x, total);
         if (a.reverse) tile = total - 1 - tile;
         int tw = tile % a.n_tiles_w, tx = tile / a.n_tiles_w;
@@ -73,9 +99,12 @@
     };
     auto set_sources = [&](int j) __attribute__((always_inline)) {
         int n0, m0;
-        tile_origin(j, n0, m0);
-        rs_w = rsrc_of(a.W + (size_t)n0 * a.ldw);
-        if constexpr (EPI == EPI_SWIGLU) rs_w2 = rsrc_of(a.W2 + (size_t)n0 * a.ldw);
+        TileSrc ts;
+        tile_origin(j, n0, m0, ts);
+        if constexpr (LIST) N = ts.N;
+        const int ldw = LIST ? ts.ldw : a.ldw;
+        rs_w = rsrc_of((LIST ? ts.W : a.W) + (size_t)n0 * ldw);
+        if constexpr (EPI == EPI_SWIGLU) rs_w2 = rsrc_of(a.W2 + (size_t)n0 * ldw);
         rs_x = rsrc_of(a.X + (size_t)m0 * a.ldx);
 #pragma unroll
         for (int p = 0; p < PW; ++p) {
@@ -85,13 +114,13 @@
             if constexpr (EPI == EPI_SWIGLU) r = (t >> 6) * 32 + (t & 31);
             else r = t;
             r = n0 + r < N ? r : N - 1 - n0;
-            woff[p] = (uint32_t)r * (uint32_t)a.ldw * 2u + (uint32_t)lc * 16u;
+            woff[p] = (uint32_t)r * (uint32_t)ldw * 2u + (uint32_t)lc * 16u;
         }
 #pragma unroll
         for (int p = 0; p < PX; ++p) {
             const int t = (p * NWAVES + wave) * RPP + lane / CPR;
             const int lc = (lane % CPR) ^ ((t >> 1) & (CPR - 1));
-            const int r = m0 + t < a.M ? t : a.M - 1 - m0;
+            const int r = m0 + t < (LIST ? 0x7fffffff : a.M) ? t : (LIST ? 0x7fffffff : a.M) - 1 - m0;
             xoff[p] = (uint32_t)r * (uint32_t)a.ldx * 2u + (uint32_t)lc * 16u;
         }
     };
@@ -125,7 +154,9 @@
 
     auto finish_tile = [&](int j_done) __attribute__((always_inline)) {
         int n0, m0;
-        tile_origin(j_done, n0, m0);
+        TileSrc ts;
+        tile_origin(j_done, n0, m0, ts);
+        if constexpr (LIST) N = ts.N;
         if constexpr ((EPI == EPI_BF16 || is_gelu_like<EPI>) && STG) {
             const __amdgpu_buffer_rsrc_t rs_out = rsrc_of((const char*)a.out + (size_t)m0 * a.ldo * 2);
             const __amdgpu_buffer_rsrc_t rs_pre = rsrc_of((const char*)(a.out2 ? a.out2 : a.out) + (size_t)m0 * (a.out2 ? a.ldo2 : a.ldo) * 2);
@@ -184,10 +215,10 @@
                         const int rl = wx * (TX / WX) + j * 32 + rr[q];
                         const int c = n0 + ww * (TW / WW) + rnd * (RCH * 8) + cc[q] * 8;
                         if (is_gelu_like<EPI> && which == 0) {
-                            const uint32_t so = ((m0 + rl < a.M && c < N) ? 0u : OOB) | ((uint32_t)(rl * a.ldo2) * 2u + (uint32_t)c * 2u);
+                            const uint32_t so = ((m0 + rl < (LIST ? 0x7fffffff : a.M) && c < N) ? 0u : OOB) | ((uint32_t)(rl * a.ldo2) * 2u + (uint32_t)c * 2u);
                             __builtin_amdgcn_raw_buffer_store_b128(rv[q], rs_pre, so, 0, 0);
                         } else {
-                            const uint32_t so = ((m0 + rl < a.M && c < N) ? 0u : OOB) | ((uint32_t)(rl * a.ldo) * 2u + (uint32_t)c * 2u);
+                            const uint32_t so = ((m0 + rl < (LIST ? 0x7fffffff : a.M) && c < N) ? 0u : OOB) | ((uint32_t)(rl * a.ldo) * 2u + (uint32_t)c * 2u);
                             __builtin_amdgcn_raw_buffer_store_b128(rv[q], rs_out, so, 0, 0);
                         }
                     }
@@ -198,7 +229,7 @@
 #pragma unroll
             for (int j = 0; j < FX; ++j) {
                 const int rl = wx * (TX / WX) + j * 32 + frow;
-                const uint32_t rowoff = (m0 + rl < a.M ? 0u : OOB) | ((uint32_t)(rl * a.ldo) * 2u);
+                const uint32_t rowoff = (m0 + rl < (LIST ? 0x7fffffff : a.M) ? 0u : OOB) | ((uint32_t)(rl * a.ldo) * 2u);
 #pragma unroll
                 for (int i = 0; i < FW; ++i)
 #pragma unroll
@@ -225,7 +256,7 @@
             auto req = [&](int f, int par) __attribute__((always_inline)) {
                 const int j = f / FW, i = f % FW;
                 const int rl = wx * (TX / WX) + j * 32 + frow;
-                const uint32_t rowoff = (m0 + rl < a.M ? 0u : OOB) | ((uint32_t)(rl * a.ldr) * 4u);
+                const uint32_t rowoff = (m0 + rl < (LIST ? 0x7fffffff : a.M) ? 0u : OOB) | ((uint32_t)(rl * a.ldr) * 4u);
 #pragma unroll
                 for (int g = 0; g < 4; ++g) {
                     const int c = c0 + i * 32 + 8 * g;
@@ -238,7 +269,7 @@
                 if (f + 1 < FW * FX) req(f + 1, (f + 1) & 1);
                 const int j = f / FW, i = f % FW;
                 const int rl = wx * (TX / WX) + j * 32 + frow;
-                const uint32_t rowoff = (m0 + rl < a.M ? 0u : OOB) | ((uint32_t)(rl * a.ldo) * 4u);
+                const uint32_t rowoff = (m0 + rl < (LIST ? 0x7fffffff : a.M) ? 0u : OOB) | ((uint32_t)(rl * a.ldo) * 4u);
 #pragma unroll
                 for (int g = 0; g < 4; ++g) {
                     const int c = c0 + i * 32 + 8 * g;
@@ -258,7 +289,7 @@
                 const int f = unit / 2, gp = unit % 2, j = f / FW, i = f % FW;
                 const int rl = wx * (TX / WX) + j * 32 + frow;
                 const int c = c0 + i * 32 + 16 * gp;
-                return ((m0 + rl < a.M && c < N) ? 0u : OOB) | ((uint32_t)(rl * ld) * 2u + (uint32_t)c * 2u);
+                return ((m0 + rl < (LIST ? 0x7fffffff : a.M) && c < N) ? 0u : OOB) | ((uint32_t)(rl * ld) * 2u + (uint32_t)c * 2u);
             };
             auto req = [&](int unit, int par) __attribute__((always_inline)) {
                 const uint32_t off = src_off(unit, a.ldr);
@@ -353,7 +384,7 @@
                     for (int q = 0; q < 4; ++q) {
                         const int rl = wx * (TX / WX) + j * 32 + q * 8 + (lane >> 3);
                         const int h = hw0 + (lane & 7) * 8;
-                        const uint32_t ok = (m0 + rl < a.M && h < N) ? 0u : OOB;
+                        const uint32_t ok = (m0 + rl < (LIST ? 0x7fffffff : a.M) && h < N) ? 0u : OOB;
                         if (which == 2) __builtin_amdgcn_raw_buffer_store_b128(rv[q], rs_out, ok | ((uint32_t)(rl * a.ldo) * 2u + (uint32_t)h * 2u), 0, 0);
                         else if (a.lab & 32) __builtin_amdgcn_raw_buffer_store_b128(rv[q], rs_out2, ok | ((uint32_t)(rl * a.ldo2) * 2u + (uint32_t)(h + (which == 1 ? a.Hp : 0)) * 2u), 0, 0);
                         else if (a.lab & 64) __builtin_amdgcn_raw_buffer_store_b128(rv[q], rs_out2, ok | ((uint32_t)(rl * a.ldo2) * 2u + (uint32_t)(h + (which == 1 ? a.Hp : 0)) * 2u), 0, 17);
@@ -369,7 +400,7 @@
 #pragma unroll
             for (int j = 0; j < FX; ++j) {
                 const int rl = wx * (TX / WX) + j * 32 + frow;
-                const uint32_t ok = m0 + rl < a.M ? 0u : OOB;
+                const uint32_t ok = m0 + rl < (LIST ? 0x7fffffff : a.M) ? 0u : OOB;
                 const uint32_t ro = ok | ((uint32_t)(rl * a.ldo) * 2u), ro2 = ok | ((uint32_t)(rl * a.ldo2) * 2u);
                 u32x4_t pg[FW / 2][2], pu[FW / 2][2], pa[FW / 2][2];
 #pragma unroll
@@ -544,6 +575,35 @@
 
 }
 
+extern "C" int fm_gemm_nt_list(const void* X, int ldx, void* out, int ldo, int K, const fm_gemm_nt_job* jobs, int n_jobs,
+                               const int32_t* row0_dev, const int32_t* m_dev, void* stream) {
+    using namespace fmk;
+    FM_CHECK_ARG(X && out && jobs && row0_dev && m_dev, "fm_gemm_nt_list: null pointer");
+    FM_CHECK_ARG(n_jobs > 0 && n_jobs <= NT_LIST_MAX, "fm_gemm_nt_list: 1..%d jobs", NT_LIST_MAX);
+    FM_CHECK_ARG(K % 64 == 0 && K >= 128 && ldx % 8 == 0 && ldo % 64 == 0 && (((uintptr_t)out) & 127) == 0,
+                 "fm_gemm_nt_list: K %% 64 == 0, K >= 128, ldx %% 8 == 0, ldo %% 64 == 0 and a 128-byte aligned out (K=%d ldx=%d ldo=%d)", K, ldx, ldo);
+    FM_CHECK_ARG((size_t)256 * (size_t)ldo * 4 < 0x7fffffffull && (size_t)256 * (size_t)ldx * 2 < 0x7fffffffull, "fm_gemm_nt_list: row stride too large");
+    NTListArgs a{};
+    a.X = (const bf16_t*)X; a.out = out; a.K = K; a.ldx = ldx; a.ldo = ldo;
+    a.m_dev = m_dev; a.row0_dev = row0_dev;
+    a.lab = fm_nt3_lab() & ~(16 | 1024);
+    a.reverse = (a.lab & 2048) ? 0 : 1;
+    a.n_jobs = n_jobs;
+    for (int i = 0; i < n_jobs; ++i) {
+        const fm_gemm_nt_job& p = jobs[i];
+        FM_CHECK_ARG(p.W && p.N > 0 && p.N % 8 == 0 && p.N <= ldo && p.ldw % 8 == 0 && p.ldw >= K && (size_t)256 * (size_t)p.ldw * 2 < 0x7fffffffull,
+                     "fm_gemm_nt_list: job %d: N=%d (a multiple of 8, <= ldo) ldw=%d (a multiple of 8, >= K)", i, p.N, p.ldw);
+        a.job[i].W = (const bf16_t*)p.W; a.job[i].N = p.N; a.job[i].ldw = p.ldw; a.job[i].n_tiles_w = (p.N + 255) / 256;
+    }
+    constexpr size_t lds = (size_t)2 * (256 + 256) * 128 + 32768;
+    auto list_kernel = gemm_nt3_kernel<256, EPI_BF16, true, true, false, false, true>;
+    static bool once = (hipFuncSetAttribute((const void*)list_kernel, hipFuncAttributeMaxDynamicSharedMemorySize, (int)lds), true);
+    (void)once;
+    hipLaunchKernelGGL(list_kernel, dim3(fm_grid_cus()), dim3(512), lds, (hipStream_t)stream, a);
+    FM_CHECK_LAUNCH("fm_gemm_nt_list");
+    return 0;
+}
+
 int fm_launch_nt3(const fmk::NTArgs& a, int epilogue, int mode, hipStream_t s) {
     using namespace fmk;
     if (!mode || a.groups || a.bias2) return 0;
diff --git a/ml-4m_amd/fourm/hip/_lib.py b/ml-4m_amd/fourm/hip/_lib.py
--- a/ml-4m_amd/fourm/hip/_lib.py
+++ b/ml-4m_amd/fourm/hip/_lib.py
@@ -53,10 +53,17 @@
 
 class GemmTNJob(C.Structure):
     _fields_ = [("A", vp), ("B", vp), ("out", vp), ("R", i32), ("N", i32), ("K", i32), ("lda", i32), ("ldb", i32),
-                ("ldo", i32), ("a_cols", i32), ("b_cols", i32)]
+                ("ldo", i32), ("a_cols", i32), ("b_cols", i32), ("row0_dev", vp), ("rows_dev", vp)]
 
 
 TN_MAX_JOBS = 16
+
+
+class GemmNTJob(C.Structure):
+    _fields_ = [("W", vp), ("N", i32), ("ldw", i32)]
+
+
+NT_LIST_MAX = 16
 
 
 class AttnArgs(C.Structure):
@@ -151,6 +158,7 @@
 
 P = C.POINTER
 gemm_nt = _sig("fm_gemm_nt", P(GemmNTArgs), vp)
+gemm_nt_list = _sig("fm_gemm_nt_list", vp, i32, vp, i32, i32, P(GemmNTJob), i32, vp, vp, vp)
 gemm_tn = _sig("fm_gemm_tn", P(GemmTNArgs), vp)
 gemm_tn_multi = _sig("fm_gemm_tn_multi", P(GemmTNJob), C.c_int, vp)
 layernorm_fwd = _sig("fm_layernorm_fwd", vp, i32, vp, vp, vp, i32, i32, vp, vp, vp, i32, i32, f32, vp)
@@ -282,7 +290,7 @@
 diffusion_pair = _sig("fm_diffusion_pair", vp, vp, vp, vp, vp, i32, vp, vp, i32, i64, vp)
 token_usage = _sig("fm_token_usage", vp, i32, i64, i64, i32, vp, vp, vp)
 EXPORTS = ["fm_reconst_loss_scratch", "fm_reconst_loss", "fm_scale_f32", "fm_mask_out_samples", "fm_ema_update", "fm_diffusion_pair", "fm_token_usage", "fm_lpips_stem", "fm_lpips_stem_bwd", "fm_maxpool2x2_nhwc", "fm_lpips_distance", "fm_lpips_tap_bwd", "fm_feat_distance", "fm_quick_gelu_bwd", "fm_quick_gelu_bwd_f32", "fm_clip_embed_ln_bwd", "fm_tap_add", "fm_clip_embed_ln", "fm_attn_decode", "fm_vit_patch_rows", "fm_vit_emb_rows", "fm_vit_colsum", "fm_lora_apply", "fm_lora_grad", "fm_vq_assign_wide", "fm_memcodes_assign", "fm_convnext_block", "fm_split3_bf16", "fm_unet_im2col", "fm_groupnorm_nhwc", "fm_add_bf16", "fm_silu_f32_to_bf16", "fm_timestep_embedding", "fm_unet_attention", "fm_diffusion_x0", "fm_quantile_abs",
-           "fm_diffusion_step", "fm_unpack_image_u8", "fm_unpack_ids_u16", "fm_unpack_mask_bits", "fm_decoder_attention_from_target", "fm_guidance_combine", "fm_image_mask", "fm_token_budgets", "fm_span_mask", "fm_vq_code_stats", "fm_vq_ema_update", "fm_vq_code_bias", "fm_vq_assign_bias", "fm_vq_code_stats_raw", "fm_vq_ema_update_euclid", "fm_vq_unpatchify", "fm_vq_latent_grad", "fm_tanh_bwd_f32", "fm_embed_rows_f32", "fm_vq_patchify_ex", "fm_vq_cls_emb_bwd", "fm_vq_latent_grad_normalized", "fm_abi_version", "fm_last_error", "fm_gemm_nt", "fm_set_gemm_nt_config", "fm_get_gemm_nt_config", "fm_set_reserved_cus", "fm_get_reserved_cus", "fm_bf16_to_f32_scaled", "fm_add_bf16_f32", "fm_scale_rows_bf16", "fm_gemm_tn", "fm_gemm_tn_multi", "fm_set_gemm_tn_config", "fm_get_gemm_tn_config", "fm_set_tn_transpose_read",
+           "fm_diffusion_step", "fm_unpack_image_u8", "fm_unpack_ids_u16", "fm_unpack_mask_bits", "fm_decoder_attention_from_target", "fm_guidance_combine", "fm_image_mask", "fm_token_budgets", "fm_span_mask", "fm_vq_code_stats", "fm_vq_ema_update", "fm_vq_code_bias", "fm_vq_assign_bias", "fm_vq_code_stats_raw", "fm_vq_ema_update_euclid", "fm_vq_unpatchify", "fm_vq_latent_grad", "fm_tanh_bwd_f32", "fm_embed_rows_f32", "fm_vq_patchify_ex", "fm_vq_cls_emb_bwd", "fm_vq_latent_grad_normalized", "fm_abi_version", "fm_last_error", "fm_gemm_nt", "fm_gemm_nt_list", "fm_set_gemm_nt_config", "fm_get_gemm_nt_config", "fm_set_reserved_cus", "fm_get_reserved_cus", "fm_bf16_to_f32_scaled", "fm_add_bf16_f32", "fm_scale_rows_bf16", "fm_gemm_tn", "fm_gemm_tn_multi", "fm_set_gemm_tn_config", "fm_get_gemm_tn_config", "fm_set_tn_transpose_read",
            "fm_get_tn_transpose_read", "fm_layernorm_fwd", "fm_layernorm_fwd_res", "fm_layernorm_bwd", "fm_layernorm_bwd_h", "fm_headnorm_fwd", "fm_headnorm_bwd", "fm_attn_fwd", "fm_attn_bwd",
            "fm_set_attn_transpose_read", "fm_get_attn_transpose_read", "fm_select_embed", "fm_embed_bwd",
            "fm_dense_decoder_mask", "fm_segment_rows", "fm_gather_rows", "fm_cross_entropy", "fm_swiglu_bwd",
diff --git a/ml-4m_amd/fourm/hip/engine.py b/ml-4m_amd/fourm/hip/engine.py
--- a/ml-4m_amd/fourm/hip/engine.py
+++ b/ml-4m_amd/fourm/hip/engine.py
@@ -14,6 +14,8 @@
 FUSE_ACT_BWD = os.environ.get("FOURM_FUSE_ACT_BWD", "0") == "1"
 HEADS_DENSE = os.environ.get("FOURM_HEADS_DENSE", "1") == "1"
 HEADS_DENSE_MAX = int(os.environ.get("FOURM_HEADS_DENSE_MAX", "8"))
+HEADS_LIST = os.environ.get("FOURM_HEADS_LIST", "1") == "1"
+HEADS_TN_LIST = os.environ.get("FOURM_HEADS_TN_LIST", "1") == "1"
 DEFER_RESIDUAL = os.environ.get("FOURM_DEFER_RESIDUAL", "1") == "1"
 HOIST_CTX = os.environ.get("FOURM_HOIST_CTX", "1") == "1"
 LN_BWD_FROM_H = os.environ.get("FOURM_LN_BWD_FROM_H", "1") == "1"
@@ -762,7 +764,10 @@
         hs["g_fwd"], hs["g_bwd"], hs["vocab_t"] = cache[1], cache[2], cache[3]
         logits = ws.get("heads.logits", (Rp, ldl), self.adt)
         if HEADS_DENSE and not self.fp32 and nH <= HEADS_DENSE_MAX and ops.heads_dense_ok(w_fwd, vocabs, logits):
-            ops.gemm_nt_heads(yp, w_fwd, vocabs, hs["seg_start"], hs["seg_count"], logits, D)
+            if HEADS_LIST and ops.heads_list_ok(w_fwd, vocabs, logits):
+                ops.gemm_nt_heads_list(yp, w_fwd, vocabs, hs["seg_start"], hs["seg_count"], logits, D)
+            else:
+                ops.gemm_nt_heads(yp, w_fwd, vocabs, hs["seg_start"], hs["seg_count"], logits, D)
         else:
             ops.gemm_nt_grouped(yp, hs["g_fwd"], hs["tile_group"], logits, hs["maxV"], max_K=D)
         hs.update(yp=yp, logits=logits, sv=sv)
@@ -1010,13 +1015,16 @@
         heads = [m.decoder_embeddings[h] for h in hs["heads"]]
         if any(h.to_logits.weight.requires_grad for h in heads):
             outs = [self.grad_view(h.to_logits.weight) if h.to_logits.weight.requires_grad else None for h in heads]
-            key = tuple(o.data_ptr() if o is not None else 0 for o in outs)
-            cache = getattr(self, "_head_tn_groups", None)
-            if cache is None or cache[0] != key:
-                cache = self._head_tn_groups = (key, ops.make_groups(
-                    [dict(out=o, N=(v if o is not None else 0)) for o, v in zip(outs, hs["vocabs"])], self.device))
-            tn = cache[1]
-            ops.gemm_tn_grouped(hs["logits"], hs["yp"], tn, hs["seg_start"], hs["seg_count"], hs["n"], hs["maxV"], hs["Rp"], D)
+            if HEADS_DENSE and HEADS_TN_LIST and not self.fp32 and ops.heads_tn_list_ok(hs["logits"], hs["yp"], hs["vocabs"]):
+                ops.gemm_tn_heads(hs["logits"], hs["yp"], outs, hs["vocabs"], hs["seg_start"], hs["seg_count"], hs["Rp"], D)
+            else:
+                key = tuple(o.data_ptr() if o is not None else 0 for o in outs)
+                cache = getattr(self, "_head_tn_groups", None)
+                if cache is None or cache[0] != key:
+                    cache = self._head_tn_groups = (key, ops.make_groups(
+                        [dict(out=o, N=(v if o is not None else 0)) for o, v in zip(outs, hs["vocabs"])], self.device))
+                tn = cache[1]
+                ops.gemm_tn_grouped(hs["logits"], hs["yp"], tn, hs["seg_start"], hs["seg_count"], hs["n"], hs["maxV"], hs["Rp"], D)
         g = ws.get("bwd.g_dec", (Rqp, D), f32)
         g_bf = ws.get("bwd.g_dec_bf", (Rqp, D), bf)
         self._ln_bwd(m.decoder_norm, dyp, st["y_final"], hs["sv"], "dn", g, g_bf, Rq, dres=None, dy_row_map=hs["r2p"])
diff --git a/ml-4m_amd/fourm/hip/ops.py b/ml-4m_amd/fourm/hip/ops.py
--- a/ml-4m_amd/fourm/hip/ops.py
+++ b/ml-4m_amd/fourm/hip/ops.py
@@ -182,6 +182,38 @@
     return out
 
 
+def heads_list_ok(ws, vocabs, out):
+    return heads_dense_ok(ws, vocabs, out) and 0 < len(ws) <= L.NT_LIST_MAX and all(w.shape[1] >= 128 and _ld(w) % 8 == 0 for w in ws)
+
+
+@_timed("heads_gemm_nt (logits, dY)")
+def gemm_nt_heads_list(x, ws, vocabs, seg_start, seg_count, out, K):
+    arr = (L.GemmNTJob * len(ws))()
+    for j, w, v in zip(arr, ws, vocabs):
+        j.W, j.N, j.ldw = _p(w), v, _ld(w)
+    L.check(L.gemm_nt_list(_p(x), _ld(x), _p(out), _ld(out), K, arr, len(ws), _p(seg_start), _p(seg_count), _stream()))
+    return out
+
+
+@_timed("heads_gemm_tn (dW)")
+def gemm_tn_heads(a_mat, b_mat, outs, vocabs, seg_start, seg_count, max_R, K):
+    todo = [(h, o, v) for h, (o, v) in enumerate(zip(outs, vocabs)) if o is not None]
+    for lo in range(0, len(todo), L.TN_MAX_JOBS):
+        part = todo[lo:lo + L.TN_MAX_JOBS]
+        arr = (L.GemmTNJob * len(part))()
+        for j, (h, o, v) in zip(arr, part):
+            j.A, j.B, j.out = _p(a_mat), _p(b_mat), _p(o)
+            j.R, j.N, j.K = max_R, v, K
+            j.lda, j.ldb, j.ldo = _ld(a_mat), _ld(b_mat), _ld(o)
+            j.a_cols, j.b_cols = a_mat.shape[1], b_mat.shape[1]
+            j.row0_dev, j.rows_dev = seg_start.data_ptr() + 4 * h, seg_count.data_ptr() + 4 * h
+        L.check(L.gemm_tn_multi(arr, len(part), _stream()))
+
+
+def heads_tn_list_ok(a_mat, b_mat, vocabs):
+    return a_mat.dtype == torch.bfloat16 and b_mat.dtype == torch.bfloat16 and all(v >= 8 for v in vocabs) and b_mat.shape[1] >= 8
+
+
 def gemm_tn(a_mat, b_mat, out, *, N=None, K=None, R=None, splits=0, force_tr=-1, a_cols=0, b_cols=0):
     if a_mat.dtype == torch.float32:
         g = L.GemmF32Args()
```
